# megvii-research/AAAI2023-PVD

Measured on AMD Instinct MI355X. Metric: train rays/s (hash->vm chair distillation step), higher is better.
Workload: dtype f16 tables+MLP (AMP, as the reference forces) / f32 marcher+compositor; 1 GPU; distill hash->vm, synthetic chair, synthetic cameras, stage 3 (rgb + feature/sigma/colour losses), 4096 rays/GPU/step, occupancy 128^3 5.0% occupied, max_steps 1024, teacher pre-trained 300 steps; rays_per_gpu=4096, parallelism=ray-dp1, update=AdamW in one launch, capture_fallback=False

## Files before the change

aaai2023-pvd_amd/csrc/raymarching.hip:

```cpp
#include "dda.h"
#include "rays.h"
#include "../../include/pvd_hip_march.h"

#include <float.h>

namespace pvd {

constexpr uint32_t kBlock = 256;
constexpr float kRPi = 0.3183098861837907f;


__global__ void __launch_bounds__(kBlock) k_near_far(const float *__restrict__ rays_o, const float *__restrict__ rays_d,
                                                     const float *__restrict__ aabb, uint32_t N, float min_near,
                                                     float *__restrict__ nears, float *__restrict__ fars) {
    const uint32_t n = blockIdx.x * kBlock + threadIdx.x;
    if (n >= N) return;
    const float o[3] = {rays_o[3 * (size_t)n], rays_o[3 * (size_t)n + 1], rays_o[3 * (size_t)n + 2]};
    const float d[3] = {rays_d[3 * (size_t)n], rays_d[3 * (size_t)n + 1], rays_d[3 * (size_t)n + 2]};
    near_far_of(o, d, aabb, min_near, nears[n], fars[n]);
}

__global__ void __launch_bounds__(kBlock) k_polar(const float *__restrict__ rays_o, const float *__restrict__ rays_d,
                                                  float radius, uint32_t N, float *__restrict__ coords) {
    const uint32_t n = blockIdx.x * kBlock + threadIdx.x;
    if (n >= N) return;
    const float ox = rays_o[3 * (size_t)n], oy = rays_o[3 * (size_t)n + 1], oz = rays_o[3 * (size_t)n + 2];
    const float dx = rays_d[3 * (size_t)n], dy = rays_d[3 * (size_t)n + 1], dz = rays_d[3 * (size_t)n + 2];
    const float A = dx * dx + dy * dy + dz * dz;
    const float Bh = ox * dx + oy * dy + oz * dz;
    const float Cc = ox * ox + oy * oy + oz * oz - radius * radius;
    const float t = (-Bh + sqrtf(Bh * Bh - A * Cc)) / A;
    const float x = ox + t * dx, y = oy + t * dy, z = oz + t * dz;
    const float theta = atan2f(sqrtf(x * x + z * z), y);
    const float phi = atan2f(z, x);
    coords[2 * (size_t)n] = 2 * theta * kRPi - 1;
    coords[2 * (size_t)n + 1] = phi * kRPi;
}

__global__ void __launch_bounds__(kBlock) k_get_rays(const float *__restrict__ pose, float fx, float fy, float cx, float cy,
                                                     const int64_t *__restrict__ inds, uint32_t W, uint32_t N,
                                                     float *__restrict__ rays_o, float *__restrict__ rays_d) {
    const uint32_t n = blockIdx.x * kBlock + threadIdx.x;
    if (n >= N) return;
    float o[3], d[3];
    ray_of_pixel(pose, fx, fy, cx, cy, inds ? inds[n] : (int64_t)n, W, o, d);
#pragma unroll
    for (int r = 0; r < 3; r++) { rays_o[3 * (size_t)n + r] = o[r]; rays_d[3 * (size_t)n + r] = d[r]; }
}

__global__ void __launch_bounds__(kBlock) k_make_ray_batch(const float *__restrict__ poses, uint32_t P, long long *__restrict__ state,
                                                           uint64_t seed, float fx, float fy, float cx, float cy, uint32_t H, uint32_t W,
                                                           uint32_t N, const float *__restrict__ aabb, float min_near,
                                                           int64_t *__restrict__ inds, float *__restrict__ rays_o,
                                                           float *__restrict__ rays_d, float *__restrict__ bg, float *__restrict__ nears,
                                                           float *__restrict__ fars) {
    const uint32_t n = blockIdx.x * kBlock + threadIdx.x;
    const long long pose_idx = state[0], batch = state[1];
    if (n < N) {
        Pcg32 g;
        g.seed(seed + 0x9E3779B97F4A7C15ull * (uint64_t)(batch + 1));
        g.advance(4ull * n);
        const int64_t k = (int64_t)(((uint64_t)g.next() * (uint64_t)(H * W)) >> 32);
        float o[3], d[3];
        ray_of_pixel(poses + 16 * (size_t)pose_idx, fx, fy, cx, cy, k, W, o, d);
        if (inds) inds[n] = k;
#pragma unroll
        for (int r = 0; r < 3; r++) { rays_o[3 * (size_t)n + r] = o[r]; rays_d[3 * (size_t)n + r] = d[r]; }
        if (bg) {
#pragma unroll
            for (int r = 0; r < 3; r++) bg[3 * (size_t)n + r] = g.next_float();
        }
        near_far_of(o, d, aabb, min_near, nears[n], fars[n]);
    }
    __syncthreads();
    if (threadIdx.x == 0) {
        __threadfence();
        const unsigned long long done = atomicAdd(reinterpret_cast<unsigned long long *>(state + 2), 1ull);
        if (done == gridDim.x - 1) {
            state[0] = (pose_idx + 1) % (long long)P;
            state[1] = batch + 1;
            state[2] = 0;
        }
    }
}

__global__ void __launch_bounds__(kBlock) k_morton3D(const int32_t *__restrict__ coords, uint32_t N, int32_t *__restrict__ indices) {
    const uint32_t n = blockIdx.x * kBlock + threadIdx.x;
    if (n >= N) return;
    indices[n] = (int32_t)morton3((uint32_t)coords[3 * (size_t)n], (uint32_t)coords[3 * (size_t)n + 1], (uint32_t)coords[3 * (size_t)n + 2]);
}

__global__ void __launch_bounds__(kBlock) k_morton3D_invert(const int32_t *__restrict__ indices, uint32_t N, int32_t *__restrict__ coords) {
    const uint32_t n = blockIdx.x * kBlock + threadIdx.x;
    if (n >= N) return;
    const int32_t ind = indices[n];
    coords[3 * (size_t)n] = (int32_t)gather3((uint32_t)(ind >> 0));
    coords[3 * (size_t)n + 1] = (int32_t)gather3((uint32_t)(ind >> 1));
    coords[3 * (size_t)n + 2] = (int32_t)gather3((uint32_t)(ind >> 2));
}

__global__ void __launch_bounds__(kBlock) k_packbits(const float *__restrict__ grid, uint32_t N, float thresh, uint8_t *__restrict__ bitfield) {
    const uint32_t n = blockIdx.x * kBlock + threadIdx.x;
    if (n >= N) return;
    const float4 a = reinterpret_cast<const float4 *>(grid)[2 * (size_t)n];
    const float4 b = reinterpret_cast<const float4 *>(grid)[2 * (size_t)n + 1];
    uint32_t bits = 0;
    bits |= (a.x > thresh) ? 1u : 0u;   bits |= (a.y > thresh) ? 2u : 0u;
    bits |= (a.z > thresh) ? 4u : 0u;   bits |= (a.w > thresh) ? 8u : 0u;
    bits |= (b.x > thresh) ? 16u : 0u;  bits |= (b.y > thresh) ? 32u : 0u;
    bits |= (b.z > thresh) ? 64u : 0u;  bits |= (b.w > thresh) ? 128u : 0u;
    bitfield[n] = (uint8_t)bits;
}


constexpr uint32_t kScanBlock = 1024;
__global__ void __launch_bounds__(kScanBlock) k_march_scan(int32_t *__restrict__ rays, uint32_t N, int32_t *__restrict__ counter) {
    __shared__ uint32_t wave_sums[kScanBlock / kWave];
    __shared__ uint32_t carry_s;
    const uint32_t tid = threadIdx.x, lane = tid & 63u, wid = tid >> 6;
    if (tid == 0) carry_s = (uint32_t)counter[0];
    __syncthreads();
    for (uint32_t base = 0; base < N; base += kScanBlock) {
        const uint32_t n = base + tid;
        const uint32_t v = (n < N) ? (uint32_t)rays[3 * (size_t)n + 2] : 0u;
        uint32_t s = v;
#pragma unroll
        for (int off = 1; off < kWave; off <<= 1) {
            const uint32_t up = __shfl_up(s, off, kWave);
            if ((int)lane >= off) s += up;
        }
        if (lane == 63) wave_sums[wid] = s;
        __syncthreads();
        uint32_t wave_prefix = 0, total = 0;
#pragma unroll
        for (uint32_t w = 0; w < kScanBlock / kWave; w++) {
            const uint32_t ws = wave_sums[w];
            if (w < wid) wave_prefix += ws;
            total += ws;
        }
        const uint32_t carry = carry_s;
        if (n < N) {
            rays[3 * (size_t)n] = (int32_t)n;
            rays[3 * (size_t)n + 1] = (int32_t)(carry + wave_prefix + s - v);
        }
        __syncthreads();
        if (tid == 0) carry_s = carry + total;
        __syncthreads();
    }
    if (tid == 0) {
        counter[0] = (int32_t)carry_s;
        counter[1] += (int32_t)N;
    }
}

__device__ __forceinline__ uint32_t logical_budget(uint32_t M, const int32_t *__restrict__ budget) {
    return budget ? min(M, (uint32_t)max(*budget, 0)) : M;
}


__device__ __forceinline__ float lattice_advance(float t, float dt, uint32_t n) {
    while (n > 0) {
        const float t1 = t + dt;
        n--;
        if (n == 0) return t1;
        const float t2 = t1 + dt;
        const uint32_t b1 = __float_as_uint(t1), b2 = __float_as_uint(t2);
        if ((b1 >> 23) != (b2 >> 23)) { t = t1; continue; }
        n--;
        if (n == 0) return t2;
        const float t3 = t2 + dt;
        const uint32_t b3 = __float_as_uint(t3);
        if ((b2 >> 23) != (b3 >> 23)) { t = t2; continue; }
        const uint32_t c = b3 - b2;
        if (c == 0) return t2;
        const uint32_t last = ((b2 >> 23) + 1u) << 23;
        const uint32_t kmax = (last - 1u - b2) / c;
        const uint32_t k = n < kmax ? n : kmax;
        t = __uint_as_float(b2 + k * c);
        n -= k;
    }
    return t;
}

__device__ __forceinline__ float lattice_points_gamma(float t_base, uint32_t lane, float dt_gamma, float dt_min, float dt_max, float far) {
    float cur = t_base, mine = t_base;
    for (uint32_t i = 1; i < 64; i++) {
        cur = cur + clampf(cur * dt_gamma, dt_min, dt_max);
        mine = lane >= i ? cur : mine;
        if (!(cur < far)) break;
    }
    return mine;
}

__device__ __forceinline__ uint64_t lanes_from(uint32_t lane) { return lane >= 64 ? 0ull : (~0ull << lane); }
__device__ __forceinline__ float readlane_f(float v, uint32_t lane) {
    return __uint_as_float((uint32_t)__builtin_amdgcn_readlane((int)__float_as_uint(v), (int)lane));
}

constexpr uint32_t kMarchMaxRecords = 15;
struct MarchChunk { uint64_t mask; float t_base; uint32_t pad; };
struct MarchRayRecords {
    uint32_t n, overflow, pad[2];
    MarchChunk chunk[kMarchMaxRecords];
};
struct MarchRecord {
    MarchChunk *chunk;
    uint32_t n;
    bool overflow;
};
static_assert(sizeof(MarchRayRecords) == 256, "workspace stride");

template <bool WRITE>
__device__ __forceinline__ uint32_t march_ray_wave(const Dda &r, float t0, float far, uint32_t limit, uint32_t lane,
                                                  float *__restrict__ xyzs, float *__restrict__ dirs, float *__restrict__ deltas,
                                                  uint32_t *n_chunks = nullptr, MarchRecord *__restrict__ rec = nullptr) {
    const bool grows = r.dt_gamma != 0.0f;
    float t_base = t0;
    bool pending = false;
    float pending_tt = 0.f;
    uint32_t emitted = 0;
    float last_t = t0;
    if (limit == 0) return 0;
    uint32_t lat_c = 0;
    for (;;) {
        if (n_chunks) (*n_chunks)++;
        const uint32_t bb = __float_as_uint(t_base);
        const bool fast = !grows && lat_c != 0 && bb + 64u * lat_c < (((bb >> 23) + 1u) << 23);
        const float t = grows ? lattice_points_gamma(t_base, lane, r.dt_gamma, r.dt_min, r.dt_max, far)
                              : (fast ? __uint_as_float(bb + lane * lat_c) : lattice_advance(t_base, r.dt_const, lane));
        const float t_after = t + clampf(t * r.dt_gamma, r.dt_min, r.dt_max);
        const bool valid = t < far;
        float x = 0, y = 0, z = 0, dtp = 0, tt = 0;
        bool occ = false;
// ... 1 lines not shown
        const uint64_t valid_mask = __ballot(valid);
        const uint64_t occ_mask = __ballot(valid && occ);
        uint32_t jump = 64;
        {
            uint32_t lo = lane + 1, hi = 64;
#pragma unroll
            for (int s = 0; s < 6; s++) {
                const uint32_t mid = (lo + hi) >> 1;
                const float tm = __shfl(t, (int)(mid & 63u), 64);
                const bool go_right = lo < hi && tm < tt;
                const bool go_left = lo < hi && !(tm < tt);
                lo = go_right ? mid + 1 : lo;
                hi = go_left ? mid : hi;
            }
            jump = lo;
        }

        uint32_t cur = 0;
        bool done = false;
        uint64_t emit_mask = 0;
        if (pending) {
            const uint64_t ge = __ballot(!(t < pending_tt));
            if (ge == 0) {
                cur = 64;
                if (!((valid_mask >> 63) & 1ull)) done = true;
            } else {
                cur = (uint32_t)__ffsll((long long)ge) - 1u;
                pending = false;
            }
        }
        while (cur < 64 && !done) {
            if (!((valid_mask >> cur) & 1ull)) { done = true; break; }
            if ((occ_mask >> cur) & 1ull) {
                const uint64_t stop = ~occ_mask & lanes_from(cur);
                const uint32_t e = stop ? (uint32_t)__ffsll((long long)stop) - 1u : 64u;
                uint32_t run = e - cur;
                const uint32_t room = limit - emitted;
                if (run >= room) { run = room; done = true; }
                emit_mask |= lanes_from(cur) & ~lanes_from(cur + run);
                emitted += run;
                cur = e;
            } else {
                const uint32_t j = (uint32_t)__builtin_amdgcn_readlane((int)jump, (int)cur);
                if (j >= 64) {
                    pending = true;
                    pending_tt = readlane_f(tt, cur);
                    cur = 64;
                    if (!((valid_mask >> 63) & 1ull)) done = true;
                } else {
                    cur = j;
                }
            }
        }
        if (WRITE && emit_mask) {
            const uint64_t below = emit_mask & ((1ull << lane) - 1ull);
            const uint32_t n_before = emitted - (uint32_t)__popcll(emit_mask);
            const int prev_lane = below ? 63 - __clzll((long long)below) : 0;
            const float prev_after = __shfl(t_after, prev_lane, 64);
            if ((emit_mask >> lane) & 1ull) {
                const size_t k = n_before + (uint32_t)__popcll(below);
                xyzs[3 * k] = x; xyzs[3 * k + 1] = y; xyzs[3 * k + 2] = z;
                dirs[3 * k] = r.dx; dirs[3 * k + 1] = r.dy; dirs[3 * k + 2] = r.dz;
                deltas[2 * k] = dtp;
                deltas[2 * k + 1] = t_after - (below ? prev_after : last_t);
            }
            last_t = readlane_f(t_after, 63u - (uint32_t)__clzll((long long)emit_mask));
        }
        if (rec && emit_mask) {
            if (rec->n < kMarchMaxRecords) {
                if (lane == 0) { rec->chunk[rec->n].mask = emit_mask; rec->chunk[rec->n].t_base = t_base; }
                rec->n++;
            } else {
                rec->overflow = true;
            }
        }
        if (done) break;
        t_base = readlane_f(t_after, 63);
        if (!fast && !grows) {
            const uint32_t b61 = __float_as_uint(readlane_f(t_after, 61)), b62 = __float_as_uint(readlane_f(t_after, 62));
            const uint32_t b63 = __float_as_uint(t_base);
            lat_c = ((b61 >> 23) == (b63 >> 23) && (b62 >> 23) == (b63 >> 23)) ? b63 - b62 : 0u;
        }
    }
    return emitted;
}

constexpr uint32_t kRaysPerBlock = kBlock / kWave;

constexpr uint32_t kCoarseShift = 3;
static_assert((1u << kCoarseShift) == PVD_COARSE_BLOCK, "coarse block edge");

__global__ void __launch_bounds__(kBlock) k_occ_coarse_mask(const uint8_t *__restrict__ bitfield, uint32_t C, uint32_t H,
                                                            uint8_t *__restrict__ mask) {
    const uint32_t G = H >> kCoarseShift, G3 = G * G * G;
    const uint32_t i = blockIdx.x * kBlock + threadIdx.x;
    if (i >= C * G3) return;
    const uint32_t c = i / G3, b = i - c * G3;
    const uint32_t bx = b / (G * G), by = (b / G) % G, bz = b % G;
    const uint8_t *cascade = bitfield + (size_t)c * ((size_t)H * H * H / 8);
    uint32_t any = 0;
    for (uint32_t x = max(bx, 1u) - 1u; x <= min(bx + 1u, G - 1u); x++)
        for (uint32_t y = max(by, 1u) - 1u; y <= min(by + 1u, G - 1u); y++)
            for (uint32_t z = max(bz, 1u) - 1u; z <= min(bz + 1u, G - 1u); z++) {
                const uint4 *p = reinterpret_cast<const uint4 *>(cascade + (size_t)morton3(x, y, z) * 64u);
#pragma unroll
                for (int q = 0; q < 4; q++) { const uint4 v = p[q]; any |= v.x | v.y | v.z | v.w; }
            }
    mask[i] = any ? (uint8_t)1 : (uint8_t)0;
}

__device__ __forceinline__ bool coarse_confine(const Dda &r, const uint8_t *__restrict__ mask, float t0, float &far, uint32_t lane,
                                               bool &empty) {
    empty = false;
    if (!mask || r.dt_gamma != 0.0f) return false;
    const float span = far - t0;
    if (!(span >= far * (1.0f / 1024.0f)) || !(span > 1e-6f)) return false;
    const float step = span * (1.0f / 63.0f);
    const float dmax = fmaxf(fabsf(r.dx), fmaxf(fabsf(r.dy), fabsf(r.dz)));
    const float delta = 1.25f * (0.5f * step * dmax) + r.bound * (1.0f / 1048576.0f);
    const float edge0 = (float)(2u << kCoarseShift) * r.mip_bound0 * r.rH;
    if (!(delta <= 0.9f * edge0)) return false;

    const float s = fmaf((float)lane, step, t0);
    const float x = clampf(fmaf(s, r.dx, r.ox), -r.bound, r.bound);
    const float y = clampf(fmaf(s, r.dy, r.oy), -r.bound, r.bound);
    const float z = clampf(fmaf(s, r.dz, r.oz), -r.bound, r.bound);
    int lo = 0, hi = 0;
    if (!r.one_cascade) {
        const float mx = fmaxf(fabsf(x), fmaxf(fabsf(y), fabsf(z)));
        int e_lo, e_hi, e_dt;
        (void)frexpf(fmaxf(mx - delta, 0.0f), &e_lo);
        (void)frexpf(mx + delta, &e_hi);
        (void)frexpf((float)((double)(r.dt_const * r.Hf) * 0.5), &e_dt);
        const int lvl_dt = (int)fminf(r.Cf - 1, fmaxf(0.0f, (float)e_dt));
        lo = max((int)fminf(r.Cf - 1, fmaxf(0.0f, (float)e_lo)), lvl_dt);
        hi = max((int)fminf(r.Cf - 1, fmaxf(0.0f, (float)e_hi)), lvl_dt);
    }
    const uint32_t G = r.H >> kCoarseShift;
    bool hit = false;
    for (int level = lo; level <= hi; level++) {
        const float mip_rbound = 1.0f / fminf((float)(1 << level), r.bound);
        const uint32_t bx = (uint32_t)(int)clampf(fmaf(x, mip_rbound, 1.0f) * r.half_h, 0.0f, r.cell_hi) >> kCoarseShift;
        const uint32_t by = (uint32_t)(int)clampf(fmaf(y, mip_rbound, 1.0f) * r.half_h, 0.0f, r.cell_hi) >> kCoarseShift;
        const uint32_t bz = (uint32_t)(int)clampf(fmaf(z, mip_rbound, 1.0f) * r.half_h, 0.0f, r.cell_hi) >> kCoarseShift;
        hit = hit || mask[(size_t)level * G * G * G + (bx * G + by) * G + bz] != 0;
    }
    const uint64_t hits = __ballot(hit);
    if (hits == 0) { empty = true; return true; }
    const uint32_t last = 63u - (uint32_t)__clzll((long long)hits);
    if (last < 63u) far = fminf(far, fmaf((float)(last + 1u), step, t0));
    return true;
}

__global__ void __launch_bounds__(kBlock) k_march_count_wave(const float *__restrict__ rays_o, const float *__restrict__ rays_d,
                                                             const uint8_t *__restrict__ grid, float bound, float dt_gamma, uint32_t max_steps,
                                                             uint32_t N, uint32_t C, uint32_t H, const float *__restrict__ nears,
                                                             const float *__restrict__ fars, int32_t *__restrict__ rays, uint32_t perturb,
                                                             MarchRayRecords *__restrict__ records, const int32_t *__restrict__ counter,
                                                             uint32_t fresh, const uint8_t *__restrict__ coarse_mask) {
    if (records && blockIdx.x == 0 && threadIdx.x == 0) records[N].n = fresh ? 0u : (uint32_t)counter[0];
    const uint32_t n = blockIdx.x * kRaysPerBlock + (threadIdx.x >> 6);
    const uint32_t lane = threadIdx.x & 63u;
    if (n >= N) return;
#ifdef PVD_MARCH_PROFILE
    const long long prof_t0 = __builtin_readcyclecounter();
    uint32_t prof_chunks = 0;
#endif
    Dda r;
    r.init(rays_o + 3 * (size_t)n, rays_d + 3 * (size_t)n, bound, dt_gamma, max_steps, C, H, grid);
    const float t0 = ray_t0(nears[n], r.dt_min, perturb, 42u, n);
    float far = fars[n];
    uint32_t num;
    bool empty = false;
    if (t0 >= 0.0f && t0 < far && coarse_confine(r, coarse_mask, t0, far, lane, empty) && empty) {
        num = 0;
        if (records && lane == 0) { records[n].n = 0; records[n].overflow = 0u; }
    } else if (t0 >= 0.0f && t0 < far) {
        MarchRecord rec = {records ? records[n].chunk : nullptr, 0u, false};
#ifdef PVD_MARCH_PROFILE
        num = march_ray_wave<false>(r, t0, far, max_steps, lane, nullptr, nullptr, nullptr, &prof_chunks, records ? &rec : nullptr);
#else
        num = march_ray_wave<false>(r, t0, far, max_steps, lane, nullptr, nullptr, nullptr, nullptr, records ? &rec : nullptr);
#endif
        if (records && lane == 0) { records[n].n = rec.n; records[n].overflow = rec.overflow ? 1u : 0u; }
    } else {
        float t = t0;
        num = 0;
        while (t < far && num < max_steps) {
            float x, y, z, dt, tn;
            if (r.probe(t, x, y, z, dt, tn)) { num++; t += dt; }
            else t = tn;
        }
        if (records && lane == 0) { records[n].n = 0; records[n].overflow = num ? 1u : 0u; }
    }
    if (lane == 0) rays[3 * (size_t)n + 2] = (int32_t)num;
#ifdef PVD_MARCH_PROFILE
    if (lane == 0) { rays[3 * (size_t)n] = (int32_t)(__builtin_readcyclecounter() - prof_t0); rays[3 * (size_t)n + 1] = (int32_t)prof_chunks; }
#endif
}

__global__ void __launch_bounds__(kBlock) k_march_write_wave(const float *__restrict__ rays_o, const float *__restrict__ rays_d,
                                                             const uint8_t *__restrict__ grid, float bound, float dt_gamma, uint32_t max_steps,
                                                             uint32_t N, uint32_t C, uint32_t H, uint32_t M,
                                                             const float *__restrict__ nears, const float *__restrict__ fars,
                                                             float *__restrict__ xyzs, float *__restrict__ dirs, float *__restrict__ deltas,
                                                             const int32_t *__restrict__ rays, uint32_t perturb,
                                                             const int32_t *__restrict__ budget) {
    const uint32_t n = blockIdx.x * kRaysPerBlock + (threadIdx.x >> 6);
    const uint32_t lane = threadIdx.x & 63u;
    if (n >= N) return;
    const uint32_t off = (uint32_t)rays[3 * (size_t)n + 1];
    const uint32_t num = (uint32_t)rays[3 * (size_t)n + 2];
    if (num == 0) return;
    if (off + num >= logical_budget(M, budget)) return;
    Dda r;
    r.init(rays_o + 3 * (size_t)n, rays_d + 3 * (size_t)n, bound, dt_gamma, max_steps, C, H, grid);
    const float t0 = ray_t0(nears[n], r.dt_min, perturb, 42u, n);
    const float far = fars[n];
    float *px = xyzs + 3 * (size_t)off, *pd = dirs + 3 * (size_t)off, *pl = deltas + 2 * (size_t)off;
    if (t0 >= 0.0f) {
        march_ray_wave<true>(r, t0, far, num, lane, px, pd, pl);
    } else if (lane == 0) {
        float t = t0, last_t = t0;
        uint32_t step = 0;
        while (t < far && step < num) {
            float x, y, z, dt, tn;
            if (r.probe(t, x, y, z, dt, tn)) {
                px[0] = x; px[1] = y; px[2] = z;
                pd[0] = r.dx; pd[1] = r.dy; pd[2] = r.dz;
                t += dt;
                pl[0] = dt; pl[1] = t - last_t; last_t = t;
                px += 3; pd += 3; pl += 2; step++;
            } else {
                t = tn;
            }
        }
    }
}


__global__ void __launch_bounds__(kBlock) k_march_write_records(const float *__restrict__ rays_o, const float *__restrict__ rays_d,
                                                               const uint8_t *__restrict__ grid, float bound, float dt_gamma, uint32_t max_steps,
                                                               uint32_t N, uint32_t C, uint32_t H, uint32_t M,
                                                               const float *__restrict__ nears, const float *__restrict__ fars,
                                                               float *__restrict__ xyzs, float *__restrict__ dirs, float *__restrict__ deltas,
                                                               int32_t *__restrict__ rays, uint32_t perturb,
                                                               const MarchRayRecords *__restrict__ records, int32_t *__restrict__ counter,
                                                               uint32_t fresh, const int32_t *__restrict__ budget) {
    __shared__ uint32_t part[kBlock / kWave], part_all[kBlock / kWave];
    const uint32_t Mlog = logical_budget(M, budget);
    const uint32_t n0 = blockIdx.x * kRaysPerBlock;
    const uint32_t wid = threadIdx.x >> 6, lane = threadIdx.x & 63u;
    uint32_t acc = 0, all = 0;
    const uint32_t n_sum = fresh ? N : n0;
    for (uint32_t i = threadIdx.x; i < n_sum; i += kBlock) {
        const uint32_t c = (uint32_t)rays[3 * (size_t)i + 2];
        all += c;
        acc += i < n0 ? c : 0u;
    }
#pragma unroll
    for (int off = 32; off >= 1; off >>= 1) { acc += __shfl_xor(acc, off, kWave); all += __shfl_xor(all, off, kWave); }
    if (lane == 0) { part[wid] = acc; part_all[wid] = all; }
    __syncthreads();
    uint32_t prefix = records[N].n;
    uint32_t grand = prefix;
#pragma unroll
    for (uint32_t w = 0; w < kBlock / kWave; w++) { prefix += part[w]; grand += part_all[w]; }
    if (fresh && grand < Mlog) {
        const size_t stride = (size_t)gridDim.x * kBlock, first = (size_t)blockIdx.x * kBlock + threadIdx.x;
        for (size_t i = 3 * (size_t)grand + first; i < 3 * (size_t)M; i += stride) { xyzs[i] = 0.f; dirs[i] = 0.f; }
        for (size_t i = 2 * (size_t)grand + first; i < 2 * (size_t)M; i += stride) deltas[i] = 0.f;
    }
    const uint32_t n = n0 + wid;
    uint32_t cnt[kRaysPerBlock];
#pragma unroll
    for (uint32_t w = 0; w < kRaysPerBlock; w++) cnt[w] = (n0 + w < N) ? (uint32_t)rays[3 * (size_t)(n0 + w) + 2] : 0u;
    uint32_t off = prefix;
#pragma unroll
    for (uint32_t w = 0; w < kRaysPerBlock; w++) off += (w < wid) ? cnt[w] : 0u;
    if (n0 + kRaysPerBlock >= N && threadIdx.x == 0) {
        uint32_t total = prefix;
#pragma unroll
        for (uint32_t w = 0; w < kRaysPerBlock; w++) total += cnt[w];
        counter[0] = (int32_t)total;
        counter[1] = fresh ? (int32_t)N : counter[1] + (int32_t)N;
    }
    if (n >= N) return;
    const uint32_t num = cnt[wid];
    if (lane == 0) { rays[3 * (size_t)n] = (int32_t)n; rays[3 * (size_t)n + 1] = (int32_t)off; }
    if (num == 0) return;
    if (off + num >= Mlog) {
        if (fresh && off < Mlog) {
            for (size_t i = 3 * (size_t)off + lane; i < 3 * (size_t)M; i += kWave) { xyzs[i] = 0.f; dirs[i] = 0.f; }
            for (size_t i = 2 * (size_t)off + lane; i < 2 * (size_t)M; i += kWave) deltas[i] = 0.f;
        }
        return;
    }
    Dda r;
    r.init(rays_o + 3 * (size_t)n, rays_d + 3 * (size_t)n, bound, dt_gamma, max_steps, C, H, grid);
    const float t0 = ray_t0(nears[n], r.dt_min, perturb, 42u, n);
    float *px = xyzs + 3 * (size_t)off, *pd = dirs + 3 * (size_t)off, *pl = deltas + 2 * (size_t)off;
    const MarchRayRecords &rr = records[n];
    if (rr.overflow) {
        const float far = fars[n];
        if (t0 >= 0.0f) {
            march_ray_wave<true>(r, t0, far, num, lane, px, pd, pl);
        } else if (lane == 0) {
            float t = t0, last_t = t0;
            uint32_t step = 0;
            while (t < far && step < num) {
                float x, y, z, dt, tn;
                if (r.probe(t, x, y, z, dt, tn)) {
                    px[0] = x; px[1] = y; px[2] = z;
                    pd[0] = r.dx; pd[1] = r.dy; pd[2] = r.dz;
                    t += dt;
                    pl[0] = dt; pl[1] = t - last_t; last_t = t;
                    px += 3; pd += 3; pl += 2; step++;
                } else {
                    t = tn;
                }
            }
        }
        return;
    }
    float last_t = t0;
    uint32_t emitted = 0;
    for (uint32_t c = 0; c < rr.n; c++) {
        const uint64_t emit_mask = rr.chunk[c].mask;
        const float t = r.dt_gamma != 0.0f ? lattice_points_gamma(rr.chunk[c].t_base, lane, r.dt_gamma, r.dt_min, r.dt_max, 3.0e38f)
                                           : lattice_advance(rr.chunk[c].t_base, r.dt_const, lane);
        const float t_after = t + clampf(t * r.dt_gamma, r.dt_min, r.dt_max);
        const uint64_t below = emit_mask & ((1ull << lane) - 1ull);
        const int prev_lane = below ? 63 - __clzll((long long)below) : 0;
        const float prev_after = __shfl(t_after, prev_lane, 64);
        if ((emit_mask >> lane) & 1ull) {
            const size_t k = emitted + (uint32_t)__popcll(below);
            xyzs[3 * (size_t)off + 3 * k] = clampf(fmaf(t, r.dx, r.ox), -bound, bound);
            xyzs[3 * (size_t)off + 3 * k + 1] = clampf(fmaf(t, r.dy, r.oy), -bound, bound);
            xyzs[3 * (size_t)off + 3 * k + 2] = clampf(fmaf(t, r.dz, r.oz), -bound, bound);
            pd[3 * k] = r.dx; pd[3 * k + 1] = r.dy; pd[3 * k + 2] = r.dz;
            pl[2 * k] = clampf(t * r.dt_gamma, r.dt_min, r.dt_max);
            pl[2 * k + 1] = t_after - (below ? prev_after : last_t);
        }
        emitted += (uint32_t)__popcll(emit_mask);
        last_t = readlane_f(t_after, 63u - (uint32_t)__clzll((long long)emit_mask));
    }
}



__device__ __forceinline__ float wave_incl_scan_add(float v, uint32_t lane) {
#pragma unroll
    for (int off = 1; off < 64; off <<= 1) {
        const float up = __shfl_up(v, off, 64);
        if ((int)lane >= off) v += up;
    }
    return v;
}
__device__ __forceinline__ float wave_incl_scan_mul(float v, uint32_t lane) {
#pragma unroll
    for (int off = 1; off < 64; off <<= 1) {
        const float up = __shfl_up(v, off, 64);
        if ((int)lane >= off) v *= up;
    }
    return v;
}
__device__ __forceinline__ float wave_sum(float v) {
#pragma unroll
    for (int off = 32; off >= 1; off >>= 1) v += __shfl_xor(v, off, 64);
    return v;
}

struct CompositeEpilogue {
    const float *bg;
    float bg_scalar;
    const float *nears, *fars;
    float depth_eps;
    uint32_t fresh;
    const int32_t *budget;
};

struct CompositeObjective {
    const float *img_t;
    const float *fea_s, *fea_t;
    const float *col_s, *col_t;
    uint32_t rows;
    uint32_t ray_blocks;
    float *partials;
    const float *coef, *upstream;
    float *g_fea, *g_col;
    float *rates_decay;
    float fea_decay;
    const float *rates;
    const float *extra;
    uint32_t n_extra, nparts;
    float *sums, *loss, *coef_out, *norms;
};

__device__ __forceinline__ float objective_block_sum(float v, float *__restrict__ sh) {
#pragma unroll
    for (int off = 32; off >= 1; off >>= 1) v += __shfl_xor(v, off, 64);
    __syncthreads();
    if ((threadIdx.x & 63u) == 0) sh[threadIdx.x >> 6] = v;
    __syncthreads();
    float r = 0.f;
#pragma unroll
    for (uint32_t w = 0; w < kBlock / kWave; w++) r += sh[w];
    return r;
}

__device__ __forceinline__ void objective_finish(const CompositeObjective &ob, float (&c4)[4], float *__restrict__ sh) {
    float a = 0.f, b = 0.f, c = 0.f, d = 0.f;
    for (uint32_t i = threadIdx.x; i < ob.nparts; i += kBlock) {
        const float4 v = reinterpret_cast<const float4 *>(ob.partials)[i];
        a += v.x; b += v.y; c += v.z; d += v.w;
    }
    float s4[4] = {objective_block_sum(a, sh), objective_block_sum(b, sh), objective_block_sum(c, sh), objective_block_sum(d, sh)};
    float nrm[4];
#pragma unroll
    for (int i = 0; i < 4; i++) {
        nrm[i] = sqrtf(s4[i]);
        c4[i] = nrm[i] > 0.f ? ob.rates[i] / nrm[i] : 0.f;
    }
    if (blockIdx.x == 0) {
        float e = 0.f;
        for (uint32_t i = threadIdx.x; i < ob.n_extra; i += kBlock) e += ob.extra[i];
        e = objective_block_sum(e, sh);
        if (threadIdx.x == 0) {
            float t = e;
#pragma unroll
            for (int i = 0; i < 4; i++) { t += ob.rates[i] * nrm[i]; ob.sums[i] = s4[i]; ob.norms[i] = nrm[i]; ob.coef_out[i] = c4[i]; }
            ob.loss[0] = t;
        }
    }
}

__device__ __forceinline__ void objective_row_sums(const CompositeObjective &ob, uint32_t blk, uint32_t nblk, float *__restrict__ sh) {
    const uint32_t tid = blk * kBlock + threadIdx.x, stride = nblk * kBlock;
    float s_fea = 0.f, s_sig = 0.f, s_col = 0.f;
    for (uint32_t i = tid; i < ob.rows * 4u; i += stride) {
        const float4 a = reinterpret_cast<const float4 *>(ob.fea_s)[i], b = reinterpret_cast<const float4 *>(ob.fea_t)[i];
        const float dx = a.x - b.x, dy = a.y - b.y, dz = a.z - b.z, dw = a.w - b.w;
        s_fea += dx * dx + dy * dy + dz * dz + dw * dw;
        if ((i & 3u) == 0) s_sig += dx * dx;
    }
    for (uint32_t i = tid; i < ob.rows * 3u; i += stride) { const float d = ob.col_s[i] - ob.col_t[i]; s_col += d * d; }
    s_fea = objective_block_sum(s_fea, sh); s_sig = objective_block_sum(s_sig, sh); s_col = objective_block_sum(s_col, sh);
    if (threadIdx.x == 0) reinterpret_cast<float4 *>(ob.partials)[ob.ray_blocks + blk] = make_float4(0.f, s_fea, s_sig, s_col);
}

__device__ __forceinline__ void objective_row_grads(const CompositeObjective &ob, const float (&c4)[4], uint32_t blk, uint32_t nblk) {
    const uint32_t tid = blk * kBlock + threadIdx.x, stride = nblk * kBlock;
    const float up = ob.upstream[0];
    const float c_fea = c4[1] * up, c_sig = c4[2] * up, c_col = c4[3] * up;
    for (uint32_t i = tid; i < ob.rows * 4u; i += stride) {
        const float4 a = reinterpret_cast<const float4 *>(ob.fea_s)[i], b = reinterpret_cast<const float4 *>(ob.fea_t)[i];
        float4 g = make_float4(c_fea * (a.x - b.x), c_fea * (a.y - b.y), c_fea * (a.z - b.z), c_fea * (a.w - b.w));
        if ((i & 3u) == 0) g.x += c_sig * (a.x - b.x);
        reinterpret_cast<float4 *>(ob.g_fea)[i] = g;
    }
    for (uint32_t i = tid; i < ob.rows * 3u; i += stride) ob.g_col[i] = c_col * (ob.col_s[i] - ob.col_t[i]);
}

template <bool EPI, bool OBJ = false>
__global__ void __launch_bounds__(kBlock) k_composite_fwd_wave(const float *__restrict__ sigmas, const float *__restrict__ rgbs,
                                                               const float *__restrict__ deltas, const int32_t *__restrict__ rays,
                                                               uint32_t M, uint32_t N, float *__restrict__ weights_sum,
                                                               float *__restrict__ depth, float *__restrict__ image, CompositeEpilogue ep,
                                                               CompositeObjective ob = CompositeObjective{}) {
    __shared__ float obj_sh[kBlock / kWave];
    if (OBJ && blockIdx.x >= ob.ray_blocks) {
        if (ob.rates_decay && blockIdx.x == ob.ray_blocks && threadIdx.x == 0) ob.rates_decay[1] *= ob.fea_decay;
        objective_row_sums(ob, blockIdx.x - ob.ray_blocks, gridDim.x - ob.ray_blocks, obj_sh);
        return;
    }
    const uint32_t n = blockIdx.x * (kBlock / kWave) + (threadIdx.x >> 6);
    const uint32_t lane = threadIdx.x & 63u;
    if (!OBJ && n >= N) return;
    const bool live = n < N;
    const uint32_t index = live ? (uint32_t)rays[3 * (size_t)n] : 0u;
    const uint32_t offset = live ? (uint32_t)rays[3 * (size_t)n + 1] : 0u;
    const uint32_t num = live ? (uint32_t)rays[3 * (size_t)n + 2] : 0u;
    float r = 0, g = 0, b = 0, ws = 0, d = 0;
    if (!(num == 0 || offset + num >= logical_budget(M, EPI ? ep.budget : nullptr))) {
        float T_carry = 1.0f, t_carry = 0.0f;
        for (uint32_t base = 0; base < num; base += 64) {
            const uint32_t s = base + lane;
            const bool in = s < num;
            const size_t i = (size_t)offset + s;
            float alpha = 0.f, dl1 = 0.f, c0 = 0.f, c1 = 0.f, c2 = 0.f;
            if (in) {
                const float2 dl = reinterpret_cast<const float2 *>(deltas)[i];
                alpha = 1.0f - __expf(-sigmas[i] * dl.x);
                dl1 = dl.y;
                c0 = rgbs[3 * i]; c1 = rgbs[3 * i + 1]; c2 = rgbs[3 * i + 2];
            }
            const float incl = wave_incl_scan_mul(1.0f - alpha, lane);
            float excl = __shfl_up(incl, 1, 64);
            if (lane == 0) excl = 1.0f;
            const float w = alpha * (T_carry * excl);
            const float t = t_carry + wave_incl_scan_add(dl1, lane);
            r += w * c0; g += w * c1; b += w * c2;
            d += w * t;
            ws += w;
            T_carry *= __shfl(incl, 63, 64);
            t_carry = __shfl(t, 63, 64);
        }
        r = wave_sum(r); g = wave_sum(g); b = wave_sum(b); ws = wave_sum(ws); d = wave_sum(d);
    }
    float d2 = 0.f;
    if (lane == 0 && live) {
        if (EPI) {
            const float t = 1.0f - ws;
            const float b0 = ep.bg ? ep.bg[3 * (size_t)index] : ep.bg_scalar, b1 = ep.bg ? ep.bg[3 * (size_t)index + 1] : ep.bg_scalar,
                        b2 = ep.bg ? ep.bg[3 * (size_t)index + 2] : ep.bg_scalar;
            r = r + t * b0; g = g + t * b1; b = b + t * b2;
            const float near = ep.nears[index], far = ep.fars[index];
            d = fmaxf(d - near, 0.0f) / (far - near + ep.depth_eps);
        }
        weights_sum[index] = ws;
        depth[index] = d;
        image[3 * (size_t)index] = r; image[3 * (size_t)index + 1] = g; image[3 * (size_t)index + 2] = b;
        if (OBJ) {
            const float e0 = ob.img_t[3 * (size_t)index] - r, e1 = ob.img_t[3 * (size_t)index + 1] - g, e2 = ob.img_t[3 * (size_t)index + 2] - b;
            d2 = e0 * e0 + e1 * e1 + e2 * e2;
        }
    }
    if (OBJ) {
        const float s_img = objective_block_sum(d2, obj_sh);
        if (threadIdx.x == 0) reinterpret_cast<float4 *>(ob.partials)[blockIdx.x] = make_float4(s_img, 0.f, 0.f, 0.f);
    }
}

template <bool EPI, bool OBJ = false>
__global__ void __launch_bounds__(kBlock) k_composite_bwd_wave(const float *__restrict__ grad_ws, const float *__restrict__ grad_image,
                                                               const float *__restrict__ sigmas, const float *__restrict__ rgbs,
                                                               const float *__restrict__ deltas, const int32_t *__restrict__ rays,
                                                               const float *__restrict__ weights_sum, const float *__restrict__ image,
                                                               uint32_t M, uint32_t N, float *__restrict__ grad_sigmas,
                                                               float *__restrict__ grad_rgbs, CompositeEpilogue ep,
                                                               CompositeObjective ob = CompositeObjective{}) {
    float c4[4] = {0.f, 0.f, 0.f, 0.f};
    if (OBJ) {
        __shared__ float fin_sh[kBlock / kWave];
        if (ob.rates) objective_finish(ob, c4, fin_sh);
        else { c4[0] = ob.coef[0]; c4[1] = ob.coef[1]; c4[2] = ob.coef[2]; c4[3] = ob.coef[3]; }
    }
    if (OBJ && blockIdx.x >= ob.ray_blocks) {
        objective_row_grads(ob, c4, blockIdx.x - ob.ray_blocks, gridDim.x - ob.ray_blocks);
        return;
    }
    const uint32_t n = blockIdx.x * (kBlock / kWave) + (threadIdx.x >> 6);
    const uint32_t lane = threadIdx.x & 63u;
    if (n >= N) return;
    const uint32_t index = (uint32_t)rays[3 * (size_t)n];
    const uint32_t offset = (uint32_t)rays[3 * (size_t)n + 1];
    const uint32_t num = (uint32_t)rays[3 * (size_t)n + 2];
    if (EPI && ep.fresh) {
        const uint32_t end = (uint32_t)rays[3 * (size_t)(N - 1) + 1] + (uint32_t)rays[3 * (size_t)(N - 1) + 2];
        for (size_t i = (size_t)end + (size_t)n * kWave + lane; i < M; i += (size_t)N * kWave) {
            grad_sigmas[i] = 0.f; grad_rgbs[3 * i] = 0.f; grad_rgbs[3 * i + 1] = 0.f; grad_rgbs[3 * i + 2] = 0.f;
        }
        if (num != 0 && offset + num >= logical_budget(M, ep.budget))
            for (size_t i = (size_t)offset + lane; i < M; i += kWave) {
                grad_sigmas[i] = 0.f; grad_rgbs[3 * i] = 0.f; grad_rgbs[3 * i + 1] = 0.f; grad_rgbs[3 * i + 2] = 0.f;
            }
    }
    if (num == 0 || offset + num >= logical_budget(M, EPI ? ep.budget : nullptr)) return;
    float gws = grad_ws ? grad_ws[index] : 0.0f;
    float rF = image[3 * (size_t)index], gF = image[3 * (size_t)index + 1], bF = image[3 * (size_t)index + 2];
    float g0, g1, g2;
    if (OBJ) {
        const float c_img = c4[0] * ob.upstream[0];
        g0 = c_img * (rF - ob.img_t[3 * (size_t)index]); g1 = c_img * (gF - ob.img_t[3 * (size_t)index + 1]);
        g2 = c_img * (bF - ob.img_t[3 * (size_t)index + 2]);
    } else {
        g0 = grad_image[3 * (size_t)index]; g1 = grad_image[3 * (size_t)index + 1]; g2 = grad_image[3 * (size_t)index + 2];
    }
    const float wsF = weights_sum[index];
    if (EPI) {
        const float b0 = ep.bg ? ep.bg[3 * (size_t)index] : ep.bg_scalar, b1 = ep.bg ? ep.bg[3 * (size_t)index + 1] : ep.bg_scalar,
                    b2 = ep.bg ? ep.bg[3 * (size_t)index + 2] : ep.bg_scalar;
        const float t = 1.0f - wsF;
        rF -= t * b0; gF -= t * b1; bF -= t * b2;
        gws -= g0 * b0 + g1 * b1 + g2 * b2;
    }
    float T_carry = 1.0f, r_carry = 0.f, g_carry = 0.f, b_carry = 0.f, ws_carry = 0.f;
    for (uint32_t base = 0; base < num; base += 64) {
        const uint32_t s = base + lane;
        const bool in = s < num;
        const size_t i = (size_t)offset + s;
        float alpha = 0.f, dl0 = 0.f, c0 = 0.f, c1 = 0.f, c2 = 0.f;
        if (in) {
            dl0 = deltas[2 * i];
            alpha = 1.0f - __expf(-sigmas[i] * dl0);
            c0 = rgbs[3 * i]; c1 = rgbs[3 * i + 1]; c2 = rgbs[3 * i + 2];
        }
        const float incl = wave_incl_scan_mul(1.0f - alpha, lane);
        float excl = __shfl_up(incl, 1, 64);
        if (lane == 0) excl = 1.0f;
        const float w = alpha * (T_carry * excl);
        const float T = T_carry * incl;
        const float r = r_carry + wave_incl_scan_add(w * c0, lane);
        const float g = g_carry + wave_incl_scan_add(w * c1, lane);
        const float b = b_carry + wave_incl_scan_add(w * c2, lane);
        const float ws = ws_carry + wave_incl_scan_add(w, lane);
        if (in) {
            grad_rgbs[3 * i] = g0 * w; grad_rgbs[3 * i + 1] = g1 * w; grad_rgbs[3 * i + 2] = g2 * w;
            grad_sigmas[i] = dl0 * (g0 * (T * c0 - (rF - r)) + g1 * (T * c1 - (gF - g)) + g2 * (T * c2 - (bF - b)) + gws * (T - (wsF - ws)));
        }
        T_carry = __shfl(T, 63, 64);
        r_carry = __shfl(r, 63, 64); g_carry = __shfl(g, 63, 64); b_carry = __shfl(b, 63, 64); ws_carry = __shfl(ws, 63, 64);
    }
}


__global__ void __launch_bounds__(kBlock) k_march_rays(uint32_t n_alive, uint32_t n_step, const int32_t *__restrict__ rays_alive,
                                                       const float *__restrict__ rays_t, const float *__restrict__ rays_o,
                                                       const float *__restrict__ rays_d, float bound, float dt_gamma,
                                                       uint32_t max_steps, uint32_t C, uint32_t H, const uint8_t *__restrict__ grid,
                                                       const float *__restrict__ fars, float *__restrict__ xyzs,
                                                       float *__restrict__ dirs, float *__restrict__ deltas, uint32_t perturb) {
    const uint32_t n = blockIdx.x * kBlock + threadIdx.x;
    if (n >= n_alive) return;
    const int32_t index = rays_alive[n];
    Dda r;
    r.init(rays_o + 3 * (size_t)index, rays_d + 3 * (size_t)index, bound, dt_gamma, max_steps, C, H, grid);
    const float far = fars[index];
    float t = ray_t0(rays_t[n], r.dt_min, perturb, (uint64_t)perturb, n);
    float last_t = t;
    float *px = xyzs + 3 * (size_t)n * n_step, *pd = dirs + 3 * (size_t)n * n_step, *pl = deltas + 2 * (size_t)n * n_step;
    uint32_t step = 0;
    while (t < far && step < n_step) {
        float x, y, z, dt, tn;
        if (r.probe(t, x, y, z, dt, tn)) {
            px[0] = x; px[1] = y; px[2] = z;
            pd[0] = r.dx; pd[1] = r.dy; pd[2] = r.dz;
            t += dt;
            pl[0] = dt; pl[1] = t - last_t; last_t = t;
            px += 3; pd += 3; pl += 2; step++;
        } else {
            t = tn;
        }
    }
}

__global__ void __launch_bounds__(kBlock) k_composite_rays(uint32_t n_alive, uint32_t n_step, const int32_t *__restrict__ rays_alive,
                                                           float *__restrict__ rays_t, const float *__restrict__ sigmas,
                                                           const float *__restrict__ rgbs, const float *__restrict__ deltas,
                                                           float *__restrict__ weights_sum, float *__restrict__ depth,
                                                           float *__restrict__ image) {
    const uint32_t n = blockIdx.x * kBlock + threadIdx.x;
    if (n >= n_alive) return;
    const int32_t index = rays_alive[n];
    float t = rays_t[n];
    float ws = weights_sum[index], d = depth[index];
    float r = image[3 * (size_t)index], g = image[3 * (size_t)index + 1], b = image[3 * (size_t)index + 2];
    uint32_t step = 0;
    while (step < n_step) {
        const size_t i = (size_t)n * n_step + step;
        const float dl0 = deltas[2 * i];
        if (dl0 == 0) break;
        const float alpha = 1.0f - __expf(-sigmas[i] * dl0);
        const float T = 1 - ws;
        const float w = alpha * T;
        ws += w;
        t += deltas[2 * i + 1];
        d += w * t;
        r += w * rgbs[3 * i]; g += w * rgbs[3 * i + 1]; b += w * rgbs[3 * i + 2];
        if ((double)T < 1e-4) break;
        step++;
    }
    rays_t[n] = (step < n_step) ? -1.0f : t;
    weights_sum[index] = ws;
    depth[index] = d;
    image[3 * (size_t)index] = r; image[3 * (size_t)index + 1] = g; image[3 * (size_t)index + 2] = b;
}

__global__ void __launch_bounds__(kBlock) k_compact_rays(uint32_t n_alive, int32_t *__restrict__ rays_alive,
                                                         const int32_t *__restrict__ rays_alive_old, float *__restrict__ rays_t,
                                                         const float *__restrict__ rays_t_old, int32_t *__restrict__ alive_counter) {
    __shared__ uint32_t wave_cnt[kBlock / kWave];
    __shared__ uint32_t block_base;
    const uint32_t n = blockIdx.x * kBlock + threadIdx.x;
    const uint32_t lane = threadIdx.x & 63u, wid = threadIdx.x >> 6;
    float t = -1.0f;
    int32_t id = 0;
// ... 128 lines not shown
            if (dl0 == 0) break;
            const float alpha = 1.0f - __expf(-(sigma_scale * sigmas[i]) * dl0);
            const float T = 1 - ws;
            const float w = alpha * T;
            ws += w;
            t += deltas[2 * i + 1];
            d += w * t;
            r += w * rgbs[3 * i]; g += w * rgbs[3 * i + 1]; b += w * rgbs[3 * i + 2];
            if ((double)T < 1e-4) break;
            step++;
        }
        rays_t[n] = (step < n_step) ? -1.0f : t;
        weights_sum[index] = ws;
        depth[index] = d;
        image[3 * (size_t)index] = r; image[3 * (size_t)index + 1] = g; image[3 * (size_t)index + 2] = b;
    }
}

}

using namespace pvd;

#define PVD_REQUIRE(cond) \
    do { if (!(cond)) return PVD_ERR_INVALID; } while (0)

extern "C" {

int pvd_near_far_from_aabb(const float *rays_o, const float *rays_d, const float *aabb, uint32_t N, float min_near,
                           float *nears, float *fars, pvd_stream_t stream) {
    if (N == 0) return PVD_OK;
    PVD_REQUIRE(rays_o && rays_d && aabb && nears && fars);
    hipLaunchKernelGGL(k_near_far, dim3(div_up(N, kBlock)), dim3(kBlock), 0, (hipStream_t)stream, rays_o, rays_d, aabb, N, min_near, nears, fars);
    return check_launch();
}

int pvd_get_rays(const float *pose, float fx, float fy, float cx, float cy, const int64_t *inds, uint32_t W, uint32_t N,
                 float *rays_o, float *rays_d, pvd_stream_t stream) {
    if (N == 0) return PVD_OK;
    PVD_REQUIRE(pose && rays_o && rays_d && W > 0);
    hipLaunchKernelGGL(k_get_rays, dim3(div_up(N, kBlock)), dim3(kBlock), 0, (hipStream_t)stream, pose, fx, fy, cx, cy, inds, W, N, rays_o, rays_d);
    return check_launch();
}

int pvd_make_ray_batch(const float *poses, uint32_t P, int64_t *state, uint64_t seed, float fx, float fy, float cx, float cy, uint32_t H,
                       uint32_t W, uint32_t N, const float *aabb, float min_near, int64_t *inds, float *rays_o, float *rays_d, float *bg,
                       float *nears, float *fars, pvd_stream_t stream) {
    if (N == 0) return PVD_OK;
    PVD_REQUIRE(poses && P > 0 && state && aabb && rays_o && rays_d && nears && fars && H > 0 && W > 0);
    PVD_REQUIRE((uint64_t)H * W < (1ull << 32));
    hipLaunchKernelGGL(k_make_ray_batch, dim3(div_up(N, kBlock)), dim3(kBlock), 0, (hipStream_t)stream, poses, P, (long long *)state, seed, fx,
                       fy, cx, cy, H, W, N, aabb, min_near, inds, rays_o, rays_d, bg, nears, fars);
    return check_launch();
}

int pvd_polar_from_ray(const float *rays_o, const float *rays_d, float radius, uint32_t N, float *coords, pvd_stream_t stream) {
    if (N == 0) return PVD_OK;
    PVD_REQUIRE(rays_o && rays_d && coords);
    hipLaunchKernelGGL(k_polar, dim3(div_up(N, kBlock)), dim3(kBlock), 0, (hipStream_t)stream, rays_o, rays_d, radius, N, coords);
    return check_launch();
}

int pvd_morton3D(const int32_t *coords, uint32_t N, int32_t *indices, pvd_stream_t stream) {
    if (N == 0) return PVD_OK;
    PVD_REQUIRE(coords && indices);
    hipLaunchKernelGGL(k_morton3D, dim3(div_up(N, kBlock)), dim3(kBlock), 0, (hipStream_t)stream, coords, N, indices);
    return check_launch();
}

int pvd_morton3D_invert(const int32_t *indices, uint32_t N, int32_t *coords, pvd_stream_t stream) {
    if (N == 0) return PVD_OK;
    PVD_REQUIRE(coords && indices);
    hipLaunchKernelGGL(k_morton3D_invert, dim3(div_up(N, kBlock)), dim3(kBlock), 0, (hipStream_t)stream, indices, N, coords);
    return check_launch();
}

int pvd_packbits(const float *grid, uint32_t N, float density_thresh, uint8_t *bitfield, pvd_stream_t stream) {
    if (N == 0) return PVD_OK;
    PVD_REQUIRE(grid && bitfield);
    PVD_REQUIRE((reinterpret_cast<uintptr_t>(grid) & 15u) == 0);
    hipLaunchKernelGGL(k_packbits, dim3(div_up(N, kBlock)), dim3(kBlock), 0, (hipStream_t)stream, grid, N, density_thresh, bitfield);
    return check_launch();
}

constexpr uint32_t kMarchFusedScanMaxRays = 16384;

size_t pvd_march_workspace_bytes(uint32_t N) { return ((size_t)N + 1) * sizeof(MarchRayRecords); }

int pvd_march_rays_train(const float *rays_o, const float *rays_d, const uint8_t *grid, float bound, float dt_gamma,
                         uint32_t max_steps, uint32_t N, uint32_t C, uint32_t H, uint32_t M, const float *nears,
                         const float *fars, float *xyzs, float *dirs, float *deltas, int32_t *rays, int32_t *counter,
                         uint32_t perturb, pvd_stream_t stream) {
    return pvd_march_rays_train_ws(rays_o, rays_d, grid, bound, dt_gamma, max_steps, N, C, H, M, nears, fars, xyzs, dirs, deltas, rays,
                                   counter, perturb, nullptr, 0, 0u, nullptr, stream);
}

int pvd_march_rays_train_ws(const float *rays_o, const float *rays_d, const uint8_t *grid, float bound, float dt_gamma,
                            uint32_t max_steps, uint32_t N, uint32_t C, uint32_t H, uint32_t M, const float *nears,
                            const float *fars, float *xyzs, float *dirs, float *deltas, int32_t *rays, int32_t *counter,
                            uint32_t perturb, void *workspace, size_t workspace_bytes, uint32_t flags, const int32_t *budget_dev,
                            pvd_stream_t stream) {
    return pvd_march_rays_train_mask(rays_o, rays_d, grid, bound, dt_gamma, max_steps, N, C, H, M, nears, fars, xyzs, dirs, deltas, rays,
                                     counter, perturb, workspace, workspace_bytes, flags, budget_dev, nullptr, stream);
}

int pvd_occ_coarse_mask(const uint8_t *bitfield, uint32_t C, uint32_t H, uint8_t *mask, pvd_stream_t stream) {
    PVD_REQUIRE(bitfield && mask && C >= 1 && C <= 16 && H >= 1 && H <= 1024);
    if ((H & (H - 1u)) || H < PVD_COARSE_BLOCK) return PVD_ERR_UNSUPPORTED;
    PVD_REQUIRE((reinterpret_cast<uintptr_t>(bitfield) & 15u) == 0);
    const uint32_t G = H >> kCoarseShift;
    hipLaunchKernelGGL(k_occ_coarse_mask, dim3(div_up(C * G * G * G, kBlock)), dim3(kBlock), 0, (hipStream_t)stream, bitfield, C, H, mask);
    return check_launch();
}

int pvd_march_rays_train_mask(const float *rays_o, const float *rays_d, const uint8_t *grid, float bound, float dt_gamma,
                              uint32_t max_steps, uint32_t N, uint32_t C, uint32_t H, uint32_t M, const float *nears,
                              const float *fars, float *xyzs, float *dirs, float *deltas, int32_t *rays, int32_t *counter,
                              uint32_t perturb, void *workspace, size_t workspace_bytes, uint32_t flags,
                              const int32_t *budget_dev, const uint8_t *coarse_mask, pvd_stream_t stream) {
    hipStream_t s = (hipStream_t)stream;
    const bool fresh = (flags & PVD_MARCH_FRESH) != 0;
    if (N == 0) {
        if (fresh && M && xyzs && dirs && deltas && counter) {
            (void)hipMemsetAsync(xyzs, 0, 3 * (size_t)M * sizeof(float), s); (void)hipMemsetAsync(dirs, 0, 3 * (size_t)M * sizeof(float), s);
            (void)hipMemsetAsync(deltas, 0, 2 * (size_t)M * sizeof(float), s); (void)hipMemsetAsync(counter, 0, 2 * sizeof(int32_t), s);
        }
        return PVD_OK;
    }
    PVD_REQUIRE(rays_o && rays_d && grid && nears && fars && xyzs && dirs && deltas && rays && counter);
    PVD_REQUIRE(C >= 1 && C <= 16 && H >= 1 && H <= 1024 && max_steps >= 1);
    MarchRayRecords *records = (workspace && workspace_bytes >= pvd_march_workspace_bytes(N) && N <= kMarchFusedScanMaxRays)
                                   ? (MarchRayRecords *)workspace : nullptr;
    if (fresh && !records) {
        (void)hipMemsetAsync(xyzs, 0, 3 * (size_t)M * sizeof(float), s); (void)hipMemsetAsync(dirs, 0, 3 * (size_t)M * sizeof(float), s);
        (void)hipMemsetAsync(deltas, 0, 2 * (size_t)M * sizeof(float), s); (void)hipMemsetAsync(counter, 0, 2 * sizeof(int32_t), s);
    }
    const dim3 g(div_up(N, kRaysPerBlock)), b(kBlock);
    if ((H & (H - 1u)) || H < PVD_COARSE_BLOCK) coarse_mask = nullptr;
    hipLaunchKernelGGL(k_march_count_wave, g, b, 0, s, rays_o, rays_d, grid, bound, dt_gamma, max_steps, N, C, H, nears, fars, rays, perturb,
                       records, counter, records && fresh ? 1u : 0u, coarse_mask);
    if (records) {
        hipLaunchKernelGGL(k_march_write_records, g, b, 0, s, rays_o, rays_d, grid, bound, dt_gamma, max_steps, N, C, H, M, nears, fars, xyzs,
                           dirs, deltas, rays, perturb, records, counter, fresh ? 1u : 0u, budget_dev);
        return check_launch();
    }
#ifdef PVD_MARCH_PROFILE
    return check_launch();
#endif
    hipLaunchKernelGGL(k_march_scan, dim3(1), dim3(kScanBlock), 0, s, rays, N, counter);
    hipLaunchKernelGGL(k_march_write_wave, g, b, 0, s, rays_o, rays_d, grid, bound, dt_gamma, max_steps, N, C, H, M, nears, fars, xyzs, dirs,
                       deltas, rays, perturb, budget_dev);
    return check_launch();
}

int pvd_composite_rays_train_forward(const float *sigmas, const float *rgbs, const float *deltas, const int32_t *rays,
                                     uint32_t M, uint32_t N, float *weights_sum, float *depth, float *image,
                                     pvd_stream_t stream) {
    if (N == 0) return PVD_OK;
    PVD_REQUIRE(sigmas && rgbs && deltas && rays && weights_sum && depth && image);
    hipLaunchKernelGGL(k_composite_fwd_wave<false>, dim3(div_up(N, kBlock / kWave)), dim3(kBlock), 0, (hipStream_t)stream, sigmas, rgbs, deltas,
                       rays, M, N, weights_sum, depth, image, CompositeEpilogue{});
    return check_launch();
}

int pvd_composite_rays_train_backward(const float *grad_weights_sum, const float *grad_image, const float *sigmas,
                                      const float *rgbs, const float *deltas, const int32_t *rays, const float *weights_sum,
                                      const float *image, uint32_t M, uint32_t N, float *grad_sigmas, float *grad_rgbs,
                                      pvd_stream_t stream) {
    if (N == 0) return PVD_OK;
    PVD_REQUIRE(grad_weights_sum && grad_image && sigmas && rgbs && deltas && rays && weights_sum && image && grad_sigmas && grad_rgbs);
    hipLaunchKernelGGL(k_composite_bwd_wave<false>, dim3(div_up(N, kBlock / kWave)), dim3(kBlock), 0, (hipStream_t)stream, grad_weights_sum,
                       grad_image, sigmas, rgbs, deltas, rays, weights_sum, image, M, N, grad_sigmas, grad_rgbs, CompositeEpilogue{});
    return check_launch();
}

int pvd_composite_rays_train_bg_forward(const float *sigmas, const float *rgbs, const float *deltas, const int32_t *rays, uint32_t M,
                                        uint32_t N, const float *bg, float bg_scalar, const float *nears, const float *fars,
                                        float depth_eps, float *weights_sum, float *depth, float *image, const int32_t *budget_dev,
                                        pvd_stream_t stream) {
    if (N == 0) return PVD_OK;
    PVD_REQUIRE(sigmas && rgbs && deltas && rays && nears && fars && weights_sum && depth && image);
    const CompositeEpilogue ep{bg, bg_scalar, nears, fars, depth_eps, 0u, budget_dev};
    hipLaunchKernelGGL(k_composite_fwd_wave<true>, dim3(div_up(N, kBlock / kWave)), dim3(kBlock), 0, (hipStream_t)stream, sigmas, rgbs, deltas,
                       rays, M, N, weights_sum, depth, image, ep);
    return check_launch();
}

int pvd_composite_rays_train_bg_backward(const float *grad_weights_sum, const float *grad_image, const float *sigmas, const float *rgbs,
                                         const float *deltas, const int32_t *rays, const float *weights_sum, const float *image,
                                         uint32_t M, uint32_t N, const float *bg, float bg_scalar, float *grad_sigmas, float *grad_rgbs,
                                         uint32_t flags, const int32_t *budget_dev, pvd_stream_t stream) {
    const bool fresh = (flags & PVD_MARCH_FRESH) != 0;
    if (N == 0) {
        if (fresh && M && grad_sigmas && grad_rgbs) {
            (void)hipMemsetAsync(grad_sigmas, 0, (size_t)M * sizeof(float), (hipStream_t)stream);
            (void)hipMemsetAsync(grad_rgbs, 0, 3 * (size_t)M * sizeof(float), (hipStream_t)stream);
        }
        return PVD_OK;
    }
    PVD_REQUIRE(grad_image && sigmas && rgbs && deltas && rays && weights_sum && image && grad_sigmas && grad_rgbs);
    const CompositeEpilogue ep{bg, bg_scalar, nullptr, nullptr, 0.f, fresh ? 1u : 0u, budget_dev};
    hipLaunchKernelGGL(k_composite_bwd_wave<true>, dim3(div_up(N, kBlock / kWave)), dim3(kBlock), 0, (hipStream_t)stream, grad_weights_sum,
                       grad_image, sigmas, rgbs, deltas, rays, weights_sum, image, M, N, grad_sigmas, grad_rgbs, ep);
    return check_launch();
}

static uint32_t objective_row_blocks(uint32_t rows, uint32_t cap) {
    uint32_t b = div_up(rows * 4u, kBlock);
    if (b > cap) b = cap;
    return b < 1 ? 1 : b;
}

uint32_t pvd_composite_objective_blocks(uint32_t N, uint32_t rows) { return div_up(N, kBlock / kWave) + objective_row_blocks(rows, 256u); }
uint32_t pvd_composite_objective_blocks_fixed(uint32_t N) { return div_up(N, kBlock / kWave) + 256u; }

int pvd_composite_objective_forward(const float *sigmas, const float *rgbs, const float *deltas, const int32_t *rays, uint32_t M, uint32_t N,
                                    const float *bg, float bg_scalar, const float *nears, const float *fars, float depth_eps,
                                    float *weights_sum, float *depth, float *image, const int32_t *budget_dev, const float *img_tea,
                                    const float *fea_stu, const float *fea_tea, const float *col_stu, const float *col_tea, uint32_t rows,
                                    float *S4, float *rates4_decay, float fea_decay, uint32_t flags, pvd_stream_t stream) {
    PVD_REQUIRE(N > 0 && rows > 0);
    PVD_REQUIRE(sigmas && rgbs && deltas && rays && nears && fars && weights_sum && depth && image);
    PVD_REQUIRE(img_tea && fea_stu && fea_tea && col_stu && col_tea && S4);
    const CompositeEpilogue ep{bg, bg_scalar, nears, fars, depth_eps, 0u, budget_dev};
    CompositeObjective ob{};
    ob.img_t = img_tea; ob.fea_s = fea_stu; ob.fea_t = fea_tea; ob.col_s = col_stu; ob.col_t = col_tea; ob.rows = rows;
    ob.ray_blocks = div_up(N, kBlock / kWave);
    ob.partials = S4 + 4;
    ob.rates_decay = rates4_decay; ob.fea_decay = fea_decay;
    const uint32_t blocks = ob.ray_blocks + ((flags & PVD_OBJECTIVE_FIXED_PARTS) ? 256u : objective_row_blocks(rows, 256u));
    hipLaunchKernelGGL((k_composite_fwd_wave<true, true>), dim3(blocks), dim3(kBlock), 0, (hipStream_t)stream, sigmas, rgbs, deltas, rays, M, N,
                       weights_sum, depth, image, ep, ob);
    return check_launch();
}

int pvd_composite_objective_backward(const float *grad_weights_sum, const float *sigmas, const float *rgbs, const float *deltas,
                                     const int32_t *rays, const float *weights_sum, const float *image, uint32_t M, uint32_t N,
                                     const float *bg, float bg_scalar, float *grad_sigmas, float *grad_rgbs, uint32_t flags,
                                     const int32_t *budget_dev, const float *img_tea, const float *fea_stu, const float *fea_tea,
                                     const float *col_stu, const float *col_tea, uint32_t rows, float *coef4, const float *upstream,
                                     float *g_fea, float *g_col, const float *rates4, const float *extra, uint32_t n_extra, float *S4,
                                     float *loss, float *norms4, pvd_stream_t stream) {
    PVD_REQUIRE(N > 0 && rows > 0);
    PVD_REQUIRE(sigmas && rgbs && deltas && rays && weights_sum && image && grad_sigmas && grad_rgbs);
    PVD_REQUIRE(img_tea && fea_stu && fea_tea && col_stu && col_tea && coef4 && upstream && g_fea && g_col);
    PVD_REQUIRE(!rates4 || (S4 && loss && norms4 && (!n_extra || extra)));
    const bool fresh = (flags & PVD_MARCH_FRESH) != 0;
    const CompositeEpilogue ep{bg, bg_scalar, nullptr, nullptr, 0.f, fresh ? 1u : 0u, budget_dev};
    CompositeObjective ob{};
    ob.img_t = img_tea; ob.fea_s = fea_stu; ob.fea_t = fea_tea; ob.col_s = col_stu; ob.col_t = col_tea; ob.rows = rows;
    ob.ray_blocks = div_up(N, kBlock / kWave);
    ob.coef = coef4; ob.upstream = upstream; ob.g_fea = g_fea; ob.g_col = g_col;
    if (rates4) {
        ob.rates = rates4; ob.extra = extra; ob.n_extra = n_extra;
        ob.nparts = (flags & PVD_OBJECTIVE_FIXED_PARTS) ? pvd_composite_objective_blocks_fixed(N) : pvd_composite_objective_blocks(N, rows);
        ob.partials = S4 + 4; ob.sums = S4; ob.loss = loss; ob.coef_out = coef4; ob.norms = norms4;
    }
    const uint32_t blocks = ob.ray_blocks + objective_row_blocks(rows, 2048u);
    hipLaunchKernelGGL((k_composite_bwd_wave<true, true>), dim3(blocks), dim3(kBlock), 0, (hipStream_t)stream, grad_weights_sum,
                       (const float *)nullptr, sigmas, rgbs, deltas, rays, weights_sum, image, M, N, grad_sigmas, grad_rgbs, ep, ob);
    return check_launch();
}

int pvd_march_rays(uint32_t n_alive, uint32_t n_step, const int32_t *rays_alive, const float *rays_t, const float *rays_o,
                   const float *rays_d, float bound, float dt_gamma, uint32_t max_steps, uint32_t C, uint32_t H,
                   const uint8_t *grid, const float *nears, const float *fars, float *xyzs, float *dirs, float *deltas,
                   uint32_t perturb, pvd_stream_t stream) {
    (void)nears;
    if (n_alive == 0) return PVD_OK;
    PVD_REQUIRE(rays_alive && rays_t && rays_o && rays_d && grid && fars && xyzs && dirs && deltas);
    PVD_REQUIRE(C >= 1 && C <= 16 && H >= 1 && H <= 1024 && max_steps >= 1);
    hipLaunchKernelGGL(k_march_rays, dim3(div_up(n_alive, kBlock)), dim3(kBlock), 0, (hipStream_t)stream, n_alive, n_step, rays_alive, rays_t,
                       rays_o, rays_d, bound, dt_gamma, max_steps, C, H, grid, fars, xyzs, dirs, deltas, perturb);
    return check_launch();
}

int pvd_composite_rays(uint32_t n_alive, uint32_t n_step, const int32_t *rays_alive, float *rays_t, const float *sigmas,
                       const float *rgbs, const float *deltas, float *weights_sum, float *depth, float *image,
                       pvd_stream_t stream) {
    if (n_alive == 0) return PVD_OK;
    PVD_REQUIRE(rays_alive && rays_t && sigmas && rgbs && deltas && weights_sum && depth && image);
    hipLaunchKernelGGL(k_composite_rays, dim3(div_up(n_alive, kBlock)), dim3(kBlock), 0, (hipStream_t)stream, n_alive, n_step, rays_alive,
                       rays_t, sigmas, rgbs, deltas, weights_sum, depth, image);
    return check_launch();
}

int pvd_compact_rays(uint32_t n_alive, int32_t *rays_alive, const int32_t *rays_alive_old, float *rays_t,
                     const float *rays_t_old, int32_t *alive_counter, pvd_stream_t stream) {
    if (n_alive == 0) return PVD_OK;
    PVD_REQUIRE(rays_alive && rays_alive_old && rays_t && rays_t_old && alive_counter);
    hipLaunchKernelGGL(k_compact_rays, dim3(div_up(n_alive, kBlock)), dim3(kBlock), 0, (hipStream_t)stream, n_alive, rays_alive,
                       rays_alive_old, rays_t, rays_t_old, alive_counter);
    return check_launch();
}

static uint32_t infer_blocks(uint32_t upper) {
    uint32_t b = div_up(upper ? upper : 1u, kBlock);
    return b < kInferBlocks ? b : kInferBlocks;
}

int pvd_infer_round_begin(int32_t *state, uint32_t parity, uint32_t N, uint32_t max_steps, pvd_stream_t stream) {
    PVD_REQUIRE(state && parity < 2 && N > 0);
    hipLaunchKernelGGL(k_infer_begin, dim3(1), dim3(64), 0, (hipStream_t)stream, (InferState *)state, parity, N, max_steps);
    return check_launch();
}

int pvd_infer_compact(int32_t *state, uint32_t parity, uint32_t n_upper, int32_t *rays_alive, const int32_t *rays_alive_old, float *rays_t,
// ... 28 lines not shown
```

aaai2023-pvd_amd/pvd/knobs.py:

```python

PRODUCTION = {
    "PVD_HIP_LIB": ("<package>/libpvd_hip.so", "path of an A/B build of the same C ABI (pvd_hip/__init__.py)"),
    "PVD_DIST_BACKEND": ("nccl", "nccl (= RCCL, one GPU per rank) | gloo (ranks may share a GPU: how the GPU tests run two ranks on a one-GPU box)"),
    "PVD_DP_EXCHANGE": ("allreduce", "ray-DP gradient exchange: allreduce (gather that zeroes / checks -> all-reduce -> the update reads the buffer) | "
                                     "sharded (reduce_scatter -> AdamW on the rank's rows -> all_gather) | classic (rounds 1-5's sequence, incl. the objective's "
                                     "four separate launches): pvd/trainer.py, pvd/ray_dp.py"),
    "PVD_DP_HASH_WIRE": ("f16", "f16 | f32: a hash student's table gradient under ray-DP crosses the links as the half-precision table the scatter wrote "
                                "(the reference's arithmetic for this gradient; 21 MB) or widened into the fp32 bucket first (42 MB; rounds 1-5)"),
    "PVD_DP_WIRE": ("f32", "f32 | f16 | bf16: width of the gradient on the wire (classic form only; measured -0.3 dB PSNR: opt-in)"),
    "PVD_STEPS_PER_GRAPH": ("", "bench.py: steps recorded per hipGraph launch (default: the largest of 20/10/5/4/2 dividing --steps)"),
    "PVD_HW_QUEUES": ("", "keep = do not set GPU_MAX_HW_QUEUES=2 at import (an integrator who owns that variable); the forked schedule is then refused "
                          "unless the caller exported 2 itself"),
}

TEST = {
    "PVD_DP_FORCE": ("0", "1 = run the ray-DP code path (collectives, exchange forms) in a world of ONE rank: RCCL next to graph capture on a one-GPU box"),
    "PVD_DP_PIPELINE": ("1", "0 | 1 (fork the next step's prefix when there is more than one rank) | 2 (always: the one-rank tests)"),
    "PVD_DP_INGRAPH": ("1", "0 = keep RCCL's collectives out of the graphs (graphs cut at the collectives: the gloo form, and the fall-back of a failed capture)"),
    "PVD_DP_OVERLAP": ("1", "segmented form only: 0 = do not replay the next step's prefix under the eager exchange"),
    "PVD_DP_SHARDED_MIN": ("65536", "elements below which a sharded sum stays a plain all-reduce (tests lower it for toy models)"),
    "PVD_ADAMW_SPLIT": ("late", "late | 0: AdamW in two parts (L1-only rows one step later on the branch) or one launch -- bit-identical (tests/test_hip_graph.py)"),
    "PVD_ADAMW_LAZY": ("1", "0 = decay the cold parameter groups every step instead of logging and replaying the decays -- bit-identical"),
    "PVD_TOUCHED_SET": ("1", "0 = zero / check the whole gradient buffer instead of the rows the occupancy grid lets a sample touch -- same training"),
    "PVD_INF_CHECK_RIDE": ("1", "0 = GradScaler's inf check as a launch of its own instead of riding on the table scatter / the exchange"),
    "PVD_HEAD_DW_RIDE": ("1", "0 = the VM head's riders on the lookup's launches as launches of their own: the weight-gradient reduction (extra workgroups of the table scatter) and the f16 weight image (extra workgroups of the lookup's forward)"),
    "PVD_MLP_FUSED": ("1", "0 = the frozen NeRF-MLP teacher layer by layer instead of pvd_mlp_head_forward_fused"),
    "PVD_INFER_PERSISTENT": ("1", "0 = inference as rounds (march / forward / composite / compact launches) instead of one persistent launch -- bit-identical images"),
    "PVD_INFER_DEVICE_ROUNDS": ("1", "0 = the reference-shaped host loop with a read-back per round"),
    "PVD_INFER_SHUFFLE": ("", "C side: slot-assignment stride of the persistent renders (a permutation of the work order; images bit-identical)"),
    "PVD_FUSED_DMA": ("", "C side: 0 / 1 = the fused lookup's weight image by register copies / LDS-DMA -- bit-identical"),
    "PVD_FORKED_GRAPHS": ("", "0 | 1 overrides whether two-chain hipGraphs may be recorded (default: only with GPU_MAX_HW_QUEUES=2)"),
    "PVD_CAPTURE_GC": ("1", "0 = leave the cyclic garbage collector on while recording (the round-2 SIGABRT's regression test)"),
    "PVD_TEST_FAIL_IN_CAPTURE": ("", "1 | forked = raise inside a recording: exercises every fall-back"),
}

ALL = {**PRODUCTION, **TEST}
```

aaai2023-pvd_amd/pvd/ops.py:

```python
import os
import types

import torch


def _mse_loss():
    from .losses import mse_fused
    return mse_fused


def _distill_loss():
    from .losses import distill_loss_normL2
    return distill_loss_normL2


def _flat_adamw():
    from .flat_adamw import FlatAdamW
    return FlatAdamW


def hip_ops():
    import gridencoder
    import raymarching
    import fusedhead
    import pvd_hip
    import shencoder
    import vmencoder
    import plenoxel

    def get_rays_fused(pose, intrinsics, H, W, N, error_map=None, generator=None):
        dev = pose.device
        coarse = None
        if error_map is not None:
            from .scene import sample_pixels_by_error
            inds2, coarse = sample_pixels_by_error(error_map.reshape(1, -1).to(dev), N, H, W, generator)
            inds = inds2[0].contiguous()
        else:
            inds = torch.randint(0, H * W, size=[N], device=dev, generator=generator)
        rays_o = torch.empty(1, N, 3, device=dev)
        rays_d = torch.empty(1, N, 3, device=dev)
        fx, fy, cx, cy = intrinsics
        pvd_hip.get_rays(pose.reshape(4, 4).contiguous(), fx, fy, cx, cy, inds, W, N, rays_o, rays_d)
        out = {"rays_o": rays_o, "rays_d": rays_d, "inds": inds[None]}
        if coarse is not None:
            out["inds_coarse"] = coarse
        return out

    def make_batch(poses, state, seed, intrinsics, H, W, N, aabb, min_near):
        dev = poses.device
        f = lambda *s: torch.empty(*s, dtype=torch.float32, device=dev)
        rays_o, rays_d, bg, nears, fars = f(1, N, 3), f(1, N, 3), f(1, N, 3), f(N), f(N)
        fx, fy, cx, cy = intrinsics
        pvd_hip.make_ray_batch(poses, state, seed, fx, fy, cx, cy, H, W, N, aabb, min_near, None, rays_o, rays_d, bg, nears, fars)
        return rays_o, rays_d, bg, (nears, fars)

    def freq_encode(x, bands, include_input=True, out_dtype=torch.float32, row_stride=None):
        return pvd_hip.freq_encode(x, bands, include_input, out_dtype, row_stride)

    return types.SimpleNamespace(freq_encode=freq_encode, make_batch=make_batch, occupancy=pvd_hip.occupancy_backend, raymarching=raymarching, GridEncoder=gridencoder.GridEncoder, SHEncoder=shencoder.SHEncoder,
                                 vm_encode=vmencoder.vm_encode, vm_encode_infer=vmencoder.vm_encode_infer, plenoxel=plenoxel, get_rays=get_rays_fused, fused_head=fusedhead, distill_loss=_distill_loss(), mse_loss=_mse_loss(), flat_adamw=_flat_adamw(), device_type="cuda", name="hip")
```

aaai2023-pvd_amd/pvd/renderer.py:

```python
import math

import numpy as np
import torch
import torch.nn as nn


def near_far_from_aabb_torch(rays_o, rays_d, aabb, min_near):
    rd = 1.0 / rays_d
    lo = (aabb[:3] - rays_o) * rd
    hi = (aabb[3:] - rays_o) * rd
    t_lo, t_hi = torch.minimum(lo, hi), torch.maximum(lo, hi)
    near, far = t_lo[:, 0], t_hi[:, 0]
    miss = torch.zeros_like(near, dtype=torch.bool)
    for a in (1, 2):
        miss = miss | (near > t_hi[:, a]) | (t_lo[:, a] > far)
        near, far = torch.maximum(near, t_lo[:, a]), torch.minimum(far, t_hi[:, a])
    big = torch.finfo(near.dtype).max
    near = torch.where(miss, torch.full_like(near, big), near.clamp_min(min_near))
    far = torch.where(miss, torch.full_like(far, big), far)
    return near, far


def sample_pdf(bins, weights, n_samples, det=False):
    pdf = weights + 1e-5
# ... 175 lines not shown
                i_march = True
            premarched = kwargs.get("premarched", False)
            if premarched:
                i_march = False
            else:
                counter = self.step_counter[self.local_step % 16]
                self.local_step += 1
            budget = self._budget() if not force_all_rays else None
            own = i_march or bool(kwargs.get("own_march", False))
            if i_march:
                xyzs, dirs, deltas, rays = self._march_train(rays_o, rays_d, nears, fars, counter, perturb, force_all_rays, dt_gamma,
                                                             max_steps, budget)
                inherited_params = [xyzs, dirs, deltas, rays]
            else:
                xyzs, dirs, deltas, rays = inherited_params

            sigmas, rgbs = self(xyzs, dirs)

            if not self.teacher_variant:
                gs, st = self.args.global_step, self.args.stage_iters
                if gs < st["stage1"]:
                    return {"stage1": gs, "depth": None, "image": None, "inherited_params": inherited_params, "sigmas": sigmas, "rays": rays}
                if gs < st["stage2"]:
                    return {"stage2": gs, "depth": None, "image": None, "inherited_params": inherited_params, "sigmas": sigmas, "rays": rays}

            if self.density_scale != 1:
                sigmas = self.density_scale * sigmas
            eps = 0.0 if self.teacher_variant else 1e-6
            ride = kwargs.get("objective")
            if ride is not None and not (torch.is_grad_enabled() and ride.with_student(getattr(self, "feature_sigma_color", None), getattr(self, "color_l", None))):
                ride = None
            okw = {} if ride is None else {"objective": ride}
            if budget is not None and own:
                weights_sum, depth, image = rm.composite_rays_train_bg(sigmas, rgbs, deltas, rays, bg_color, nears, fars, eps, True, budget[1], **okw)
            else:
                weights_sum, depth, image = rm.composite_rays_train_bg(sigmas, rgbs, deltas, rays, bg_color, nears, fars, eps, True, **okw)
            image = image.view(*prefix, 3)
            depth = depth.view(*prefix)
            return {"depth": depth, "image": image, "inherited_params": inherited_params, "sigmas": sigmas, "rays": rays,
                    "nears_fars": (nears, fars)}

        if self._persistent_render(rays_o, perturb):
            if self.model_type == "tensors":
                run = self.ops.plenoxel.infer_image
            else:
                fh = self.ops.fused_head
                run = {"hash": fh.hash_infer_image, "vm": fh.vm_infer_image}.get(self.model_type) or fh.mlp_infer_image
            weights_sum, depth, image = run(self, rays_o, rays_d, nears, fars, dt_gamma, max_steps)
            image = image + (1 - weights_sum).unsqueeze(-1) * bg_color
            depth = torch.clamp(depth - nears, min=0) / (fars - nears)
            return {"depth": depth.view(*prefix), "image": image.view(*prefix, 3), "inherited_params": inherited_params}
        if self._rounds_on_device(rays_o, perturb):
            return self._run_rounds_device(rays_o, rays_d, nears, fars, bg_color, dt_gamma, max_steps, prefix, inherited_params)
        dtype = torch.float32
        weights_sum = torch.zeros(N, dtype=dtype, device=device)
        depth = torch.zeros(N, dtype=dtype, device=device)
        image = torch.zeros(N, 3, dtype=dtype, device=device)
        n_alive = N
        alive_counter = torch.zeros([1], dtype=torch.int32, device=device)
        rays_alive = torch.zeros(2, n_alive, dtype=torch.int32, device=device)
        rays_t = torch.zeros(2, n_alive, dtype=dtype, device=device)
        step, i = 0, 0
        while step < max_steps:
            if step == 0:
                rays_alive[0] = torch.arange(n_alive, dtype=torch.int32, device=device)
                rays_t[0] = nears
            else:
                alive_counter.zero_()
                rm.compact_rays(n_alive, rays_alive[i % 2], rays_alive[(i + 1) % 2], rays_t[i % 2], rays_t[(i + 1) % 2], alive_counter)
                n_alive = alive_counter.item()
            if n_alive <= 0:
                break
            n_step = max(min(N // n_alive, 8), 1)
            xyzs, dirs, deltas = rm.march_rays(n_alive, n_step, rays_alive[i % 2], rays_t[i % 2], rays_o, rays_d, self.bound,
                                               self.density_bitfield, self.cascade, self.grid_size, nears, fars, 128, perturb,
                                               dt_gamma, max_steps)
            sigmas, rgbs = self(xyzs, dirs)
            sigmas = self.density_scale * sigmas
            rm.composite_rays(n_alive, n_step, rays_alive[i % 2], rays_t[i % 2], sigmas, rgbs, deltas, weights_sum, depth, image)
            step += n_step
            i += 1
        image = image + (1 - weights_sum).unsqueeze(-1) * bg_color
        depth = torch.clamp(depth - nears, min=0) / (fars - nears)
        return {"depth": depth.view(*prefix), "image": image.view(*prefix, 3), "inherited_params": inherited_params}

    def _persistent_render(self, rays_o, perturb):
        import os
        fh = getattr(getattr(self, "ops", None), "fused_head", None)
        mt = getattr(self, "model_type", None)
        if os.environ.get("PVD_INFER_PERSISTENT", "1") == "0":
            return False
        if mt == "tensors":
            px = getattr(getattr(self, "ops", None), "plenoxel", None)
            return (rays_o.is_cuda and not perturb and hasattr(px, "infer_image") and getattr(self, "bg_net", None) is None
                    and not self.args.enable_edit_plenoxel)
        return self._rounds_on_device(rays_o, perturb) and ((mt == "hash" and hasattr(fh, "hash_infer_image")) or
                                                            (mt == "vm" and hasattr(fh, "vm_infer_image")) or
                                                            (mt == "mlp" and hasattr(fh, "mlp_infer_image")))

    def _rounds_on_device(self, rays_o, perturb):
        import os
        return (rays_o.is_cuda and not perturb and hasattr(self.rm, "infer_march") and torch.is_autocast_enabled("cuda")
                and getattr(self, "supports_device_rows", lambda: False)() and os.environ.get("PVD_INFER_DEVICE_ROUNDS", "1") != "0")

    @torch.no_grad()
    def _run_rounds_device(self, rays_o, rays_d, nears, fars, bg_color, dt_gamma, max_steps, prefix, inherited_params, check_every=8):
        rm = self.rm
        N, device = rays_o.shape[0], rays_o.device
        f32 = dict(dtype=torch.float32, device=device)
        weights_sum, depth, image = torch.zeros(N, **f32), torch.zeros(N, **f32), torch.zeros(N, 3, **f32)
        state = torch.zeros(rm.INFER_STATE_INTS, dtype=torch.int32, device=device)
        state[0] = N
        rays_alive = torch.empty(2, N, dtype=torch.int32, device=device)
        rays_t = torch.empty(2, N, **f32)
        rays_alive[0] = torch.arange(N, dtype=torch.int32, device=device)
        rays_t[0] = nears
        rows = N + (128 - N % 128) % 128
        xyzs, dirs, deltas = torch.empty(rows, 3, **f32), torch.empty(rows, 3, **f32), torch.empty(rows, 2, **f32)
        rows_dev = state[4:5]
        n_upper, i = N, 0
        while True:
            for _ in range(check_every):
                cur, old = i & 1, (i & 1) ^ 1
                if i > 0:
                    rm.infer_compact(state, cur, n_upper, rays_alive[cur], rays_alive[old], rays_t[cur], rays_t[old])
                rm.infer_round_begin(state, cur, N, max_steps)
                rm.infer_march(state, n_upper, rays_alive[cur], rays_t[cur], rays_o, rays_d, self.bound, dt_gamma, max_steps, self.cascade,
                               self.grid_size, self.density_bitfield, fars, xyzs, dirs, deltas, False)
                m_upper = min(rows, 8 * n_upper + (128 - (8 * n_upper) % 128) % 128)
                sigmas, rgbs = self.forward_rows(xyzs[:m_upper], dirs[:m_upper], rows_dev)
                rm.infer_composite(state, n_upper, rays_alive[cur], rays_t[cur], sigmas, rgbs.float(), deltas, float(self.density_scale),
                                   weights_sum, depth, image)
                i += 1
            n_alive, steps_done = state[2:6:3].tolist()
            if n_alive <= 0 or steps_done >= max_steps:
                break
            n_upper = min(n_upper, n_alive)
        self._last_rounds = int(state[6])
        image = image + (1 - weights_sum).unsqueeze(-1) * bg_color
        depth = torch.clamp(depth - nears, min=0) / (fars - nears)
        return {"depth": depth.view(*prefix), "image": image.view(*prefix, 3), "inherited_params": inherited_params}

    def march(self, rays_o, rays_d, dt_gamma=0, perturb=False, force_all_rays=False, max_steps=1024, nears_fars=None):
        rm = self.rm
        rays_o = rays_o.contiguous().view(-1, 3)
        rays_d = rays_d.contiguous().view(-1, 3)
        nears, fars = nears_fars if nears_fars is not None else rm.near_far_from_aabb(rays_o, rays_d, self.aabb_train, self.min_near)
        counter = self.step_counter[self.local_step % 16]
        self.local_step += 1
        budget = self._budget() if not force_all_rays else None
        xyzs, dirs, deltas, rays = self._march_train(rays_o, rays_d, nears, fars, counter, perturb, force_all_rays, dt_gamma, max_steps, budget)
        return [xyzs, dirs, deltas, rays], (nears, fars)

    def _march_train(self, rays_o, rays_d, nears, fars, counter, perturb, force_all_rays, dt_gamma, max_steps, budget):
        coarse = self.coarse_mask()
        extra = () if budget is None and coarse is None else (budget,) if coarse is None else (budget, coarse)
        return self.rm.march_rays_train(rays_o, rays_d, self.bound, self.density_bitfield, self.cascade, self.grid_size, nears, fars,
                                        counter, self.mean_count, perturb, 128, force_all_rays, dt_gamma, max_steps, True, *extra)

    def _cell_centres(self, coords, cas, jitter):
        H = self.grid_size
        xyzs = 2 * coords.float() / (H - 1) - 1
        bound = min(2 ** cas, self.bound)
        hgs = bound / H
        p = xyzs * (bound - hgs)
        if jitter:
            p = p + (torch.rand_like(p) * 2 - 1) * hgs
        return p, hgs

    @torch.no_grad()
    def mark_untrained_grid(self, poses, intrinsic, S=64):
        if not self.cuda_ray:
            return
        if isinstance(poses, np.ndarray):
            poses = torch.from_numpy(poses)
        dev = self.density_grid.device
        poses = poses.to(dev)
        B = poses.shape[0]
        fx, fy, cx, cy = intrinsic
        H = self.grid_size
        axis = torch.arange(H, dtype=torch.int32, device=dev)
        count = torch.zeros_like(self.density_grid)
        for xs in axis.split(S):
            for ys in axis.split(S):
                for zs in axis.split(S):
                    xx, yy, zz = torch.meshgrid(xs, ys, zs, indexing="ij")
                    coords = torch.stack([xx.reshape(-1), yy.reshape(-1), zz.reshape(-1)], dim=-1)
                    indices = self.rm.morton3D(coords).long()
                    for cas in range(self.cascade):
                        world, hgs = self._cell_centres(coords, cas, jitter=False)
                        for head in range(0, B, S):
                            P = poses[head:head + S]
                            cam = (world.unsqueeze(0) - P[:, :3, 3].unsqueeze(1)) @ P[:, :3, :3]
                            seen = (cam[..., 2] > 0) \
                                & (cam[..., 0].abs() < cx / fx * cam[..., 2] + hgs * 2) \
                                & (cam[..., 1].abs() < cy / fy * cam[..., 2] + hgs * 2)
                            count[cas, indices] += seen.sum(0).reshape(-1)
        self.density_grid[count == 0] = -1
        self.note_occupancy_changed()

    @torch.no_grad()
    def update_extra_state(self, decay=0.95, S=128):
        if not self.cuda_ray:
            return
        self._flush_deferred_updates()
        occ = getattr(self.ops, "occupancy", None)
        if occ is not None and self.density_grid.is_cuda:
            return self._update_extra_state_device(occ, decay)
        rm = self.rm
        dev = self.density_grid.device
        H = self.grid_size
        tmp_grid = -torch.ones_like(self.density_grid)

        def query(coords, indices, cas):
            p, _ = self._cell_centres(coords, cas, jitter=True)
            sig = self.density(p)["sigma"].reshape(-1).detach().float() * self.density_scale
            tmp_grid[cas, indices] = sig

        if self.iter_density < 16:
            axis = torch.arange(H, dtype=torch.int32, device=dev)
            for xs in axis.split(S):
                for ys in axis.split(S):
                    for zs in axis.split(S):
                        xx, yy, zz = torch.meshgrid(xs, ys, zs, indexing="ij")
                        coords = torch.stack([xx.reshape(-1), yy.reshape(-1), zz.reshape(-1)], dim=-1)
                        indices = rm.morton3D(coords).long()
                        for cas in range(self.cascade):
                            query(coords, indices, cas)
        else:
            n = H ** 3 // 4
            for cas in range(self.cascade):
                coords = torch.randint(0, H, (n, 3), device=dev)
                indices = rm.morton3D(coords).long()
                occ = torch.nonzero(self.density_grid[cas] > 0).squeeze(-1)
                if occ.shape[0] > 0:
                    occ = occ[torch.randint(0, occ.shape[0], [n], dtype=torch.long, device=dev)]
                    occ_coords = rm.morton3D_invert(occ)
                    indices = torch.cat([indices, occ], dim=0)
                    coords = torch.cat([coords, occ_coords], dim=0)
                query(coords, indices, cas)

        valid = (self.density_grid >= 0) & (tmp_grid >= 0)
        self.density_grid[valid] = torch.maximum(self.density_grid[valid] * decay, tmp_grid[valid])
        self.mean_density = torch.mean(self.density_grid.clamp(min=0)).item()
        self.iter_density += 1

        thresh = min(self.mean_density, self.density_thresh)
        self.density_bitfield = rm.packbits(self.density_grid, thresh, self.density_bitfield)
        self.note_occupancy_changed()

        total_step = min(16, self.local_step)
        if total_step > 0:
            self.mean_count = int(self.step_counter[:total_step, 0].sum().item() / total_step)
        self.local_step = 0

    def _update_extra_state_device(self, occ, decay):
        dev = self.density_grid.device
        H, C = self.grid_size, self.cascade
        H3 = H ** 3
        st = getattr(self, "_occ_state", None)
        if st is None:
            st = self._occ_state = dict(list=torch.empty(H3, dtype=torch.int32, device=dev), count=torch.zeros(1, dtype=torch.int32, device=dev),
                                        tmp=torch.empty(H3, dtype=torch.float32, device=dev), scratch=torch.empty(1024, device=dev),
                                        mean_thresh=torch.zeros(2, device=dev), calls=0)
        full = self.iter_density < 16
        n_u, n_o = (H3, 0) if full else (H3 // 4, H3 // 4)
        n = n_u + n_o
        indices = torch.empty(n, dtype=torch.int32, device=dev)
        xyz = torch.empty(n, 3, dtype=torch.float32, device=dev)
        for cas in range(C):
            st["calls"] += 1
            if self.occ_replay:
                self._occ_cascade_replay(occ, st, cas, full, n_u, indices, xyz, decay)
                continue
            occ.occ_sample(self.density_grid[cas], H, n_u, n_o, full, float(min(2 ** cas, self.bound)), 0x0cc0 + 7919 * st["calls"], st["list"],
                           st["count"], indices, xyz)
            sig = self.density(xyz)["sigma"].reshape(-1).detach().float().contiguous()
            occ.occ_update(self.density_grid[cas], st["tmp"], indices, sig, H, float(self.density_scale), float(decay))
        occ.occ_finish(self.density_grid.view(-1), float(self.density_thresh), st["mean_thresh"], st["scratch"], self.density_bitfield)
        self.note_occupancy_changed()
        self.mean_density = st["mean_thresh"][0]
        self.iter_density += 1
        total_step = min(16, self.local_step)
        if total_step > 0:
            self.mean_count = int(self.step_counter[:total_step, 0].sum().item() / total_step)
            self._publish_budget()
        self.local_step = 0

    occ_replay = False

    def _occ_cascade_replay(self, occ, st, cas, full, n_u, indices, xyz, decay):
        dev = self.density_grid.device
        H = self.grid_size
        bound_c = float(min(2 ** cas, self.bound))
        if full:
            assert H <= 128, "the reference sweeps in 128^3 blocks: replay covers the single-block case"
            jitter = torch.rand(H ** 3, 3).to(dev)
            occ.occ_sample_replay(H, 0, 0, True, bound_c, None, None, None, jitter, indices, xyz)
            n = H ** 3
        else:
            cells = torch.randint(0, H, (n_u, 3))
            lst = torch.nonzero(self.density_grid[cas] > 0).squeeze(-1)
            n_o = 0
            picks = None
            if lst.shape[0] > 0:
                picks = torch.randint(0, lst.shape[0], [n_u], dtype=torch.long).to(torch.int32).to(dev)
# ... 55 lines not shown
```

aaai2023-pvd_amd/pvd/trainer.py:

```python
import os

import torch
import torch.distributed as dist

from .capture import CarriedPrefix, SegmentedCapture
from .ray_dp import FlatGrads, RayDP, _FlatOptGrads, _make_loss


def pvd_forked_graphs_ok():
    import pvd_hip
    return pvd_hip.forked_graphs_ok()


def psnr(pred, truth):
    mse = torch.mean((pred.float() - truth.float()) ** 2)
    return -10.0 * torch.log10(mse)


class _TrainerBase:
    def __init__(self, opt, model, lr, device, fp16=True, dp=None, eta_min=None, exp_decay=False):
        self.opt = opt
        self.device = torch.device(device)
        self.device_type = self.device.type
        self.fp16 = bool(fp16)
# ... 74 lines not shown
        if c is None:
            from .dp_compact import GradCompactor
            offs = self.optimizer.offsets if self.flat_opt else None
            if offs is None:
                offs, acc = [], 0
                for p in self.flat.params:
                    offs.append(acc)
                    acc += p.numel()
            c = GradCompactor(m, self.flat.params, offs, self.device, marcher=marcher)
            c.agreed = True
            if self.dp.enabled and self.dp.capture is None and c.idx is not None:
                sig = torch.tensor([c.idx.numel(), float(c.idx.sum())], dtype=torch.float64, device=self.device)
                sig = torch.cat([sig, -sig])
                dist.all_reduce(sig, op=dist.ReduceOp.MAX, group=self.dp.group)
                c.agreed = bool(sig[0] == -sig[2]) and bool(sig[1] == -sig[3])
            self._compactor = c
        return c if (c.fraction < 0.7 and c.agreed) else None

    def _zero_grads(self, first_in_recording=False):
        if self.flat_opt:
            c = self._grad_compactor() if os.environ.get("PVD_TOUCHED_SET", "1") != "0" else None
            if c is not self.optimizer.touched:
                self.optimizer.set_touched(c)
        self.flat.zero_(full=first_in_recording)

    _xlayouts = None
    _v2_off = False
    _sharded_stale = False

    def _exchange_mode(self, c):
        mode = os.environ.get("PVD_DP_EXCHANGE", "allreduce")
        if (mode == "classic" or c is None or self._v2_off or not self.flat_opt or self.device_type != "cuda" or c is not self.optimizer.touched
                or not self.optimizer._outside_is_zero or os.environ.get("PVD_DP_WIRE", "f32") != "f32"
                or getattr(self, "_overlap_with_exchange", None) is not None or not self.optimizer.compact_ready()):
            return None
        return "sharded" if (mode == "sharded" and (self.dp.world_size > 1 or os.environ.get("PVD_DP_FORCE") == "1")) else "allreduce"

    def _xlayout(self, c, chunks, with_params):
        from .dp_compact import ExchangeLayout
        key = (id(c), chunks, with_params)
        if self._xlayouts is None or self._xlayouts[0] != key:
            assert not torch.cuda.is_current_stream_capturing(), "the exchange layout is built by the eager warm-up steps"
            self._xlayouts = (key, ExchangeLayout(c, self.optimizer._warm_B, chunks, self.device, with_params=with_params))
        return self._xlayouts[1]

    def prepare_exchange(self):
        if not self.dp.enabled or not self.flat_opt:
            return
        c = self._grad_compactor()
        mode = self._exchange_mode(c)
        if mode is not None:
            try:
                self._xlayout(c, self.dp.world_size if mode == "sharded" else 1, mode == "sharded")
            except AssertionError:
                self._v2_off = True

    def _exchange_v2(self, c, mode):
        import pvd_hip
        o, dp = self.optimizer, self.dp
        sharded = mode == "sharded"
        L = self._xlayout(c, dp.world_size if sharded else 1, sharded)
        pvd_hip.segments_gather_zero_check(self.flat.flat, L.segs, L.xbuf, L.xbuf[L.slot:], L.chunk, L.chunks)
        clear = (L.xbuf[L.slot:], L.chunk, L.chunks)
        if not sharded:
            dp.all_reduce_sum_(L.xbuf)
            o.take_compact(L.xbuf, L.xbuf[L.slot:L.slot + 1], clear, (0, L.n_groups))
            return
        mine = L.chunk_of(L.xbuf, dp.rank)
        dp.reduce_scatter_sum_(mine, L.xbuf)
        pmine = L.chunk_of(L.pbuf, dp.rank)
        o.take_compact(mine, mine[L.slot:L.slot + 1], clear, L.rows_of(dp.rank), param_out=pmine)

        def after_update():
            dp.all_gather_(L.pbuf, pmine)
            pvd_hip.segments_op(pvd_hip.SEG_SCATTER, o.flat_p, L.segs, buf=L.pbuf)
            pvd_hip.note_weights_changed(o.params)
        self._after_update = after_update
        self._sharded_stale = True

    def sync_sharded_state(self):
        if not self._sharded_stale:
            return
        import pvd_hip
        assert not torch.cuda.is_current_stream_capturing()
        L, o, dp = self._xlayouts[1], self.optimizer, self.dp
        o.flush()
        for buf in (o.flat_m, o.flat_v):
            pvd_hip.segments_op(pvd_hip.SEG_GATHER, buf, L.segs, buf=L.pbuf)
            dp.all_gather_(L.pbuf, L.chunk_of(L.pbuf, dp.rank).clone())
            pvd_hip.segments_op(pvd_hip.SEG_SCATTER, buf, L.segs, buf=L.pbuf)
        self._sharded_stale = False

    def _exchange(self):
        if self.dp.enabled:
            c = self._grad_compactor()
            mode = self._exchange_mode(c)
            if mode is not None:
                return self._exchange_v2(c, mode)
            if self._sharded_stale and not torch.cuda.is_current_stream_capturing():
                self.sync_sharded_state()
            ov = getattr(self, "_overlap_with_exchange", None)
            wire = {"f16": torch.float16, "bf16": torch.bfloat16}.get(os.environ.get("PVD_DP_WIRE", "f32"))
            hg = getattr(self.optimizer, "_half_grad", None) if self.flat_opt else None
            if c is None and hg is not None:
                lo, hi, g16 = hg
                self.dp.all_reduce_sum_(g16, overlap=ov)
                flat = self.flat.flat
                if self.optimizer._half_range_dirty:
                    self.dp.all_reduce_sum_(flat)
                else:
                    if lo > 0:
                        self.dp.all_reduce_sum_(flat[:lo])
                    if hi < flat.numel():
                        self.dp.all_reduce_sum_(flat[hi:])
            elif c is None:
                if wire is None:
                    self.dp.all_reduce_sum_(self.flat.flat, overlap=ov)
                else:
                    w16 = self.flat.flat.to(wire)
                    self.dp.all_reduce_sum_(w16, overlap=ov)
                    self.flat.flat.copy_(w16)
            else:
                buf = c.gather(self.flat.flat)
                if wire is None:
                    self.dp.all_reduce_sum_(buf, overlap=ov)
                else:
                    w16 = buf.to(wire)
                    self.dp.all_reduce_sum_(w16, overlap=ov)
                    buf = w16.to(torch.float32)
                checked = (self.flat_opt and c is self.optimizer.touched and self.optimizer._outside_is_zero
                           and bool(getattr(self.scaler, "_enabled", False)) and os.environ.get("PVD_INF_CHECK_RIDE", "1") != "0")
                c.scatter(self.flat.flat, buf, found_inf=self.optimizer.inf_flag() if checked else None)
                if checked:
                    self.optimizer.note_checked_by_backward()

    _after_update = None

    def _optimize(self):
        self.scaler.step(self.optimizer)
        self.scaler.update()
        after, self._after_update = self._after_update, None
        if after is not None:
            after()

    def _backward_and_step(self, loss):
        self._backward(loss)
        self._exchange()
        self._optimize()
        self.scheduler.step()
        self.global_step += 1

    steps_per_replay = 1

    def capture(self, body, warmup=3, steps_per_graph=1):
        assert self.device_type == "cuda"
        side = torch.cuda.Stream()
        side.wait_stream(torch.cuda.current_stream())
        with torch.cuda.stream(side):
            for _ in range(warmup):
                self._zero_grads()
                out = body()
                self._backward(out[0])
                self._exchange()
                self._optimize()
                self.scheduler.step()
                self.global_step += 1
                del out
        torch.cuda.current_stream().wait_stream(side)
        torch.cuda.synchronize()
        cap = SegmentedCapture(self.device)
        self.dp.capture = cap
        if self.dp.enabled and not self.dp.ingraph:
            steps_per_graph = 1
        self._graph_zeroes = False
        if max(1, int(steps_per_graph)) >= 2 and not self.dp.enabled:
            self._fold_launches(True)
        try:
            with cap:
                for k_rec in range(max(1, int(steps_per_graph))):
                    self._zero_grads(first_in_recording=k_rec == 0)
                    self._static_out = body()
                    if os.environ.get("PVD_TEST_FAIL_IN_CAPTURE") == "1":
                        raise RuntimeError("forced failure inside the capture (PVD_TEST_FAIL_IN_CAPTURE)")
                    self._backward(self._static_out[0])
                    self._exchange()
                    self._optimize()
        finally:
            self.dp.capture = None
            self._fold_launches(False)
        self._cap = cap
        self.steps_per_replay = max(1, int(steps_per_graph))
        self._captured_occ_epoch = self._marching_model().occ_epoch if (self.flat_opt and self.optimizer.touched is not None) else None
        return self._static_out

    def _fold_launches(self, on):
        if self.flat_opt:
            self.optimizer.zero_in_step = bool(on)
            if on:
                self._graph_zeroes = False
                self.optimizer._zeroed_by_step = False
            else:
                self._graph_zeroes = bool(self.optimizer._zeroed_by_step)
                self.optimizer._zeroed_by_step = False

    def _after_failed_capture(self):
        import traceback
        traceback.print_exc()
        torch.cuda.synchronize()
        self.dp.capture = None
        self._fold_launches(False)
        self._graph_zeroes = False
        self._after_update = None
        if self.flat_opt:
            self.optimizer._compact = None
            self.optimizer._half_grad = None
            self.optimizer._part_a_owed = None
            self.optimizer.end_two_part(failed=True)

    def replay(self):
        assert getattr(self, "_captured_occ_epoch", None) in (None, self._marching_model().occ_epoch), \
            "the occupancy grid changed since the step was captured (touched-row set is stale): capture again"
        if self.flat_opt:
            import pvd_hip
            pvd_hip.note_weights_changed(self.optimizer.params)
        if self.flat_opt:
            self.optimizer.before_replay()
        self._cap.replay()
        if self.flat_opt:
            if getattr(self, "_replay_owes_part_a", None) is not None:
                self.optimizer.note_carried_part_a(self._replay_owes_part_a)
            self.optimizer.note_device_steps(self.steps_per_replay)
            if getattr(self, "_graph_zeroes", False):
                self.optimizer._zeroed_by_step = True
        for _ in range(self.steps_per_replay):
            self.scheduler.step()
        self.global_step += self.steps_per_replay
        return self._static_out


class DistillTrainer(_TrainerBase):

    compact_exchange = True

    def __init__(self, opt, model_tea, model_stu, device, fp16=True, dp=None):
        for p in model_tea.parameters():
            p.requires_grad = False
        lr = opt.lr * (0.1 if opt.model_type == "mlp" else 1.0)
        super().__init__(opt, model_stu, lr, device, fp16, dp, eta_min=5e-5)
        self.model_tea = model_tea.train()
        self.model_stu = model_stu.train()
        self.loss = _make_loss(opt.loss_type, self.dp)
        self.loss_rate_fea_sc = opt.loss_rate_fea_sc
        self.rates = torch.tensor([opt.loss_rate_rgb, opt.loss_rate_fea_sc, opt.loss_rate_sigma, opt.loss_rate_color],
                                  dtype=torch.float32, device=self.device)
        self.fea_rate = self.rates[1:2]
        self.fused_loss = getattr(model_stu.ops, "distill_loss", None)

    def render_kwargs(self):
        o = self.opt
        return dict(dt_gamma=o.dt_gamma, max_steps=o.max_steps)

    def _marching_model(self):
        return self.model_stu if bool(getattr(self.opt, "render_stu_first", True)) else self.model_tea

    def prefetch(self, batch_fn):
        return self.prefetch_teacher(self.prefetch_march(batch_fn))

    def prefetch_march(self, batch_fn):
        rays_o, rays_d, bg, *rest = batch_fn()
        with torch.autocast(self.device_type, dtype=torch.float16, enabled=self.fp16 and self.device_type == "cuda"):
            inh, nf = self.model_stu.march(rays_o, rays_d, perturb=True, force_all_rays=False, nears_fars=rest[0] if rest else None,
                                           **self.render_kwargs())
        return dict(rays_o=rays_o, rays_d=rays_d, bg=bg, inh=inh, nf=nf)

    def prefetch_teacher(self, part):
        with torch.autocast(self.device_type, dtype=torch.float16, enabled=self.fp16 and self.device_type == "cuda"), torch.no_grad():
            out_tea = self.model_tea.render(part["rays_o"], part["rays_d"], staged=False, bg_color=part["bg"], perturb=True,
                                            force_all_rays=False, inherited_params=part["inh"], nears_fars=part["nf"], premarched=True,
                                            **self.render_kwargs())
        tea = self.model_tea
        attrs = {k: getattr(tea, k, None) for k in ("feature_sigma_color", "sigma_l", "color_l")}
        return dict(part, out_tea=out_tea, tea_attrs={k: v for k, v in attrs.items() if torch.is_tensor(v)})

    def compute_loss(self, rays_o, rays_d, bg_color, nears_fars=None, pre=None):
        o, stu, tea = self.opt, self.model_stu, self.model_tea
        o.global_step = self.global_step
        self.__dict__.pop("_ride", None)
        kw = self.render_kwargs()
        kw_stu = dict(kw, nears_fars=nears_fars) if nears_fars is not None else kw
        if pre is not None:
            for k, v in pre.get("tea_attrs", {}).items():
                setattr(tea, k, v)
            out_tea = dict(pre["out_tea"])
            if out_tea.get("image") is not None and pre.get("replayed_ahead", False):
                out_tea["image"] = out_tea["image"].clone()
            ride = None
            l1_on_host = o.l1_reg_weight > 0.0 and o.model_type == "vm" and not self.flat_opt
            dp_ride = self.dp.enabled and not l1_on_host and os.environ.get("PVD_DP_EXCHANGE", "allreduce") != "classic"
            if (self.fused_loss is not None and o.loss_type == "normL2" and (not self.dp.enabled or dp_ride) and torch.is_grad_enabled()
                    and self._stage_of(self.global_step) == 3 and out_tea.get("image") is not None
                    and min(o.loss_rate_color, o.loss_rate_sigma, self.loss_rate_fea_sc * 0.995, o.loss_rate_rgb) > 0.0
                    and torch.is_tensor(getattr(tea, "feature_sigma_color", None)) and torch.is_tensor(getattr(tea, "color_l", None))
                    and tea.feature_sigma_color.dim() == 2 and tea.feature_sigma_color.shape[-1] == 16
                    and tea.feature_sigma_color.dtype == torch.float32 and pre["rays_o"].is_cuda):
                from .losses import ObjectiveRide
                fin = not l1_on_host
                ride = ObjectiveRide(out_tea["image"], tea.feature_sigma_color, tea.color_l, rates_decay=self.rates if fin else None, fea_decay=0.995,
                                     fixed_parts=self.dp.enabled)
                self.dp_objective_rides = bool(self.dp.enabled)
            out_stu = stu.render(pre["rays_o"], pre["rays_d"], staged=False, bg_color=pre["bg"], perturb=True, force_all_rays=False,
                                 inherited_params=pre["inh"], nears_fars=pre["nf"], premarched=True, objective=ride, **kw)
            self._ride = ride if (ride is not None and ride.S is not None) else None
        else:
            out_tea = None
            if not bool(getattr(o, "render_stu_first", True)) and stu.cuda_ray:
                with torch.no_grad():
                    out_tea = tea.render(rays_o, rays_d, staged=False, bg_color=bg_color, perturb=True, force_all_rays=False, **kw_stu)
                out_stu = stu.render(rays_o, rays_d, staged=False, bg_color=bg_color, perturb=True, force_all_rays=False,
                                     inherited_params=out_tea["inherited_params"], nears_fars=out_tea.get("nears_fars"), **kw)
            else:
                out_stu = stu.render(rays_o, rays_d, staged=False, bg_color=bg_color, perturb=True, force_all_rays=False, **kw_stu)
            if out_tea is None:
                with torch.no_grad():
                    out_tea = tea.render(rays_o, rays_d, staged=False, bg_color=bg_color, perturb=True, force_all_rays=False,
                                         inherited_params=out_stu["inherited_params"], nears_fars=out_stu.get("nears_fars"), **kw)
        self.loss_rate_fea_sc *= 0.995
        have_fea = stu.feature_sigma_color is not None and tea.feature_sigma_color is not None
        pred_stu, pred_tea = out_stu.get("image"), out_tea.get("image")
        fused = (self.fused_loss is not None and o.loss_type == "normL2" and have_fea and pred_stu is not None and pred_stu.is_cuda
                 and "stage1" not in out_stu and "stage2" not in out_stu
                 and min(o.loss_rate_color, o.loss_rate_sigma, self.loss_rate_fea_sc, o.loss_rate_rgb) > 0.0
                 and stu.feature_sigma_color.dtype == torch.float32 and tea.feature_sigma_color.dtype == torch.float32
                 and stu.feature_sigma_color.dim() == 2 and stu.feature_sigma_color.shape[-1] == 16
                 and tea.feature_sigma_color.shape == stu.feature_sigma_color.shape)
        fused_nofea = (not fused and not have_fea and self.fused_loss is not None and o.loss_type == "normL2" and pred_stu is not None
                       and pred_stu.is_cuda and "stage1" not in out_stu and "stage2" not in out_stu
                       and min(o.loss_rate_color, o.loss_rate_sigma, o.loss_rate_rgb) > 0.0
                       and getattr(stu, "sigma_l", None) is not None and getattr(tea, "sigma_l", None) is not None
                       and stu.sigma_l.dim() == 1 and tea.sigma_l.shape == stu.sigma_l.shape
                       and not (o.l1_reg_weight > 0.0 and o.model_type == "vm"))
        assert fused or not getattr(getattr(self, "_ride", None), "decayed", False), \
            "the compositing launch applied the feature rate's decay for a fused objective that is not being formed"
        if not fused:
            self.fea_rate.mul_(0.995) if not fused_nofea else None
        info = {}
        loss = 0.0
        if "stage1" in out_stu and self.loss_rate_fea_sc > 0.0 and have_fea:
            l_fea = self.loss(stu.feature_sigma_color, tea.feature_sigma_color)
            info["fea"] = l_fea.detach()
            return loss + self.fea_rate * l_fea, info, None, None
        if "stage2" in out_stu:
            l_col = self.loss(stu.color_l, tea.color_l)
            l_sig = self.loss(stu.sigma_l, tea.sigma_l)
            if o.loss_rate_color > 0.0:
                loss = loss + o.loss_rate_color * l_col
            if o.loss_rate_sigma > 0.0:
                loss = loss + o.loss_rate_sigma * l_sig
            if self.loss_rate_fea_sc > 0.0 and have_fea:
                loss = loss + self.fea_rate * self.loss(stu.feature_sigma_color, tea.feature_sigma_color)
            info.update(color=l_col.detach(), sigma=l_sig.detach())
            return loss, info, None, None

        if fused_nofea:
            l3, norms = self.fused_loss(pred_stu, pred_tea, stu.sigma_l.float().unsqueeze(-1), tea.sigma_l.float().unsqueeze(-1),
                                        stu.color_l.float(), tea.color_l.float(), self.rates, self.dp, fea_decay=0.995)
            info["rgb"] = norms[0]
            return l3, info, pred_stu, pred_tea
        if fused:
            extra = None
            if o.l1_reg_weight > 0.0 and o.model_type == "vm":
                if self.flat_opt:
                    self._l1_term(partials_only=True)
                    extra = self.optimizer.l1_partials(1.0 / self.dp.world_size)
            add_l1 = o.l1_reg_weight > 0.0 and o.model_type == "vm" and extra is None
            ride = self.__dict__.pop("_ride", None)
            rkw = {} if ride is None else {"ride": ride}
            l4, norms = self.fused_loss(pred_stu, pred_tea, stu.feature_sigma_color, tea.feature_sigma_color, stu.color_l.float(),
                                        tea.color_l.float(), self.rates, self.dp, fea_decay=0.995, extra=extra, **rkw)
            loss = l4
            if add_l1:
                loss = loss + self._l1_term()
            info["rgb"] = norms[0]
            return loss, info, pred_stu, pred_tea
        if o.loss_type == "normL2":
            l_rgb = self.dp.global_norm_l2(pred_tea - pred_stu)
        elif o.loss_type == "normL1":
            l_rgb = self.dp.global_norm_l1(pred_tea - pred_stu)
        else:
            l_rgb = self.dp.global_mean((pred_tea.float() - pred_stu.float()) ** 2)
        loss = loss + l_rgb * o.loss_rate_rgb
        if o.l1_reg_weight > 0.0 and o.model_type == "vm":
            loss = loss + self._l1_term()
        if self.loss_rate_fea_sc > 0.0 and have_fea:
            loss = loss + self.fea_rate * self.loss(stu.feature_sigma_color, tea.feature_sigma_color)
        if o.loss_rate_color > 0.0:
            loss = loss + o.loss_rate_color * self.loss(stu.color_l, tea.color_l)
        if o.loss_rate_sigma > 0.0:
            loss = loss + o.loss_rate_sigma * self.loss(stu.sigma_l, tea.sigma_l)
        info["rgb"] = l_rgb.detach()
        return loss, info, pred_stu, pred_tea

    def train_step(self, rays_o, rays_d, bg_color, nears_fars=None):
        o, stu = self.opt, self.model_stu
        if getattr(o, "update_stu_extra", False) and stu.cuda_ray and self.global_step % o.update_extra_interval == 0:
            with torch.autocast(self.device_type, dtype=torch.float16, enabled=self.fp16 and self.device_type == "cuda"):
                stu.update_extra_state()
        self._zero_grads()
        with torch.autocast(self.device_type, dtype=torch.float16, enabled=self.fp16 and self.device_type == "cuda"):
            loss, info, pred_stu, pred_tea = self.compute_loss(rays_o, rays_d, bg_color, nears_fars)
        self._backward_and_step(loss)
        return loss.detach(), info, pred_stu, pred_tea

    def capture_step(self, batch_fn, steps_per_graph=1):
        def body():
            rays_o, rays_d, bg, *rest = batch_fn()
            with torch.autocast(self.device_type, dtype=torch.float16, enabled=self.fp16):
                return self.compute_loss(rays_o, rays_d, bg, *rest)
        warm = 3
        if self.flat_opt:
            self.optimizer.flush()
            self.sync_sharded_state()
        self._replay_owes_part_a = None
        self.fused_spans = None
        stage = self._stage_of(self.global_step)
        assert self._stage_of(self.global_step + warm) == stage, \
            "capture_step: the %d warm-up steps cross a stage boundary (global_step %d); step eagerly past it first" % (warm, self.global_step)
        stu_marches = bool(getattr(self.opt, "render_stu_first", True))
        if self.dp.enabled and self.dp.ingraph:
            try:
                pipe = os.environ.get("PVD_DP_PIPELINE", "1")
                if stu_marches and stage == 3 and steps_per_graph > 1 and (pipe == "2" or (pipe == "1" and self.dp.world_size > 1)):
                    out = self._capture_ingraph_pipelined(batch_fn, body, steps_per_graph)
                else:
                    out = self.capture(body, steps_per_graph=steps_per_graph)
            except Exception:
                self._after_failed_capture()
                self.dp.ingraph = False
                out = self.capture(body, warmup=0, steps_per_graph=1)
                self.capture_fallback = "segmented"
        elif self.dp.enabled and stu_marches and stage == 3 and os.environ.get("PVD_DP_OVERLAP", "1") != "0":
            out = self._capture_pipelined(batch_fn, body)
        elif not self.dp.enabled and stage == 3 and steps_per_graph > 1 and stu_marches and pvd_forked_graphs_ok():
            try:
                out = self._capture_ingraph_pipelined(batch_fn, body, steps_per_graph)
            except Exception:
                self._after_failed_capture()
                self.pipelined_ingraph = False
                self.capture_fallback = "back-to-back"
                out = self.capture(body, warmup=0, steps_per_graph=steps_per_graph)
        else:
            out = self.capture(body, steps_per_graph=steps_per_graph)
        self._captured_stage = self._stage_of(self.global_step)
        return out

    def _capture_ingraph_pipelined(self, batch_fn, body, steps_per_graph):
        assert self.device_type == "cuda" and (not self.dp.enabled or self.dp.ingraph)
        K = int(steps_per_graph)
        assert K >= 2, "with one step per graph the step's own scatter would still read the samples the carried prefix overwrites"
        side = torch.cuda.Stream()
        side.wait_stream(torch.cuda.current_stream())
        with torch.cuda.stream(side):
            for _ in range(3):
                self._zero_grads()
                out = body()
                self._backward(out[0])
                self._exchange()
                self._optimize()
                self.scheduler.step()
                self.global_step += 1
                del out
        torch.cuda.current_stream().wait_stream(side)
        torch.cuda.synchronize()
        self._graph_zeroes = False
        if not self.dp.enabled:
            self._fold_launches(True)
        with torch.cuda.stream(side):
            carried = CarriedPrefix(self.prefetch(batch_fn))
        torch.cuda.current_stream().wait_stream(side)
        torch.cuda.synchronize()
        late = (self.flat_opt and os.environ.get("PVD_ADAMW_SPLIT", "late") == "late" and (not self.dp.enabled or self.dp.ingraph))
        scaled = bool(getattr(self.scaler, "_enabled", False))
        self._replay_owes_part_a = None
        fh = getattr(getattr(self.model_stu, "ops", None), "fused_head", None)
        pack_ahead = getattr(fh, "prepack_train_image", None)
        self.fused_spans = None
        if getattr(self, "record_fused_spans", False) and getattr(self.model_tea, "model_type", "") == "hash":
            import pvd_hip
            self.fused_spans = torch.tensor([list(pvd_hip.FUSED_SPAN_INIT)] * K, dtype=torch.int64, device=self.device)
        if late and not self.optimizer.begin_two_part(defer=True):
            late = False
        if late:
            self.optimizer.carry_last = True
        if self.dp.enabled and self.flat_opt:
            self.prepare_exchange()
            if self._exchange_mode(self._grad_compactor()) is not None:
                self._fold_launches(True)
        cap = SegmentedCapture(self.device)
        self.dp.capture = cap
        branch = torch.cuda.Stream(self.device)
        try:
            with cap:
                main = torch.cuda.current_stream()
                pre = carried.pre
                try:
                    for k in range(K):
                        branch.wait_stream(main)
                        if self.fused_spans is not None:
                            self.model_tea._fused_span = self.fused_spans[k]
                        with torch.cuda.stream(branch):
                            if pack_ahead is not None and pack_ahead(self.model_stu):
                                packed = torch.cuda.Event()
                                packed.record(branch)
                                self.model_stu._before_head = lambda packed=packed: main.wait_event(packed)
                            marched = self.prefetch_march(batch_fn)
                            if late:
                                self.optimizer.run_part_a()
                                if k == 0:
                                    self.optimizer.run_carried_part_a(scaled)
                            pre_next = self.prefetch_teacher(marched)
                            if k + 1 == K:
                                carried.store(pre_next)
                        self._zero_grads(first_in_recording=k == 0)
                        with torch.autocast(self.device_type, dtype=torch.float16, enabled=self.fp16):
                            self._static_out = self.compute_loss(None, None, None, pre=pre)
                        self._backward(self._static_out[0])
                        if os.environ.get("PVD_TEST_FAIL_IN_CAPTURE") in ("1", "forked") and k == 1:
                            raise RuntimeError("forced failure inside the forked capture (PVD_TEST_FAIL_IN_CAPTURE)")
                        self._exchange()
                        if late and k + 1 == K:
                            self.optimizer._next_step_is_last = True
                        self._optimize()
                        main.wait_stream(branch)
                        pre = pre_next
                    if late:
                        self.optimizer._part_a_owed = None
                        self._replay_owes_part_a = scaled
                except Exception:
                    self.model_stu.__dict__.pop("_before_head", None)
                    self.model_stu.__dict__.pop("_train_image_ready", None)
                    main.wait_stream(branch)
                    raise
        finally:
            self.dp.capture = None
            self._fold_launches(False)
            if late:
                self.optimizer.end_two_part()
        self._cap = cap
        self.steps_per_replay = K
        self._captured_occ_epoch = self._marching_model().occ_epoch if (self.flat_opt and self.optimizer.touched is not None) else None
        self.pipelined_ingraph = True
        self.pipeline_fork = "start"
        self.adamw_split = "late" if (late and getattr(self.optimizer, "_graph_is_two_part", False)) else "0"
        return self._static_out

    def _capture_pipelined(self, batch_fn, body):
        side = torch.cuda.Stream()
        side.wait_stream(torch.cuda.current_stream())
        with torch.cuda.stream(side):
            for _ in range(3):
                self._zero_grads()
                out = body()
                self._backward(out[0])
                self._exchange()
                self._optimize()
                self.scheduler.step()
                self.global_step += 1
                del out
        torch.cuda.current_stream().wait_stream(side)
        torch.cuda.synchronize()
        self._g_prefix = torch.cuda.CUDAGraph()
        with torch.cuda.graph(self._g_prefix, capture_error_mode="thread_local"):
            self._pre = dict(self.prefetch(batch_fn), replayed_ahead=True)

        def body_pre():
            with torch.autocast(self.device_type, dtype=torch.float16, enabled=self.fp16):
                return self.compute_loss(None, None, None, pre=self._pre)
        self._overlap_with_exchange = self._g_prefix.replay
        try:
            out = self.capture(body_pre, warmup=0)
        finally:
            self._overlap_with_exchange = None
        self._g_prefix.replay()
        return out

    def _stage_of(self, step):
        st = self.opt.stage_iters
        return 1 if step < st["stage1"] else (2 if step < st["stage2"] else 3)

    def replay_step(self):
        assert self._stage_of(self.global_step) == self._captured_stage, "stage changed: capture_step() again"
        assert self._stage_of(self.global_step + self.steps_per_replay - 1) == self._captured_stage, "the replay would cross a stage boundary"
        loss, info, pred_stu, pred_tea = self.replay()
        return loss.detach(), info, pred_stu, pred_tea


class TeacherTrainer(_TrainerBase):

    def __init__(self, opt, model, device, fp16=True, dp=None):
        lr = opt.lr * (0.1 if opt.model_type == "mlp" else 1.0)
        super().__init__(opt, model, lr, device, fp16, dp, exp_decay=True)
        self.model.train()

# ... 141 lines not shown
```

aaai2023-pvd_amd/pvd/workload.py:

```python
import numpy as np
import torch

from .config import PVDConfig
from .network import NeRFNetwork
from .scene import BLENDER_INTRINSICS, ChairScene, forward_facing_train_poses, get_rays, packbits_torch, rand_poses, synthetic_poses
from .trainer import DistillTrainer, RayDP, TeacherTrainer


def renderer_kwargs(opt):
    return dict(bound=opt.bound, cuda_ray=opt.cuda_ray, density_scale=1, min_near=opt.min_near, density_thresh=opt.density_thresh,
                bg_radius=opt.bg_radius, grid_size=opt.grid_size)


def make_model(ops, opt, model_type, is_teacher, device, teacher_variant=False):
    m = NeRFNetwork(ops, model_type=model_type, args=opt, is_teacher=is_teacher, teacher_variant=teacher_variant,
                    **renderer_kwargs(opt))
    return m.to(device)


def install_occupancy(model, scene, opt):
    dev = model.density_grid.device
    grid = scene.density_grid(opt.grid_size, opt.bound, model.cascade, device=dev)
    model.density_grid.copy_(grid)
    model.density_bitfield.copy_(packbits_torch(grid, min(float(grid.clamp(min=0).mean()), opt.density_thresh)))
    model.mean_density = float(grid.clamp(min=0).mean())
    model.note_occupancy_changed()
    return grid


class AnalyticTarget:

    def __init__(self, ops, scene, proxy):
        self.rm, self.scene, self.proxy = ops.raymarching, scene, proxy

    @torch.no_grad()
    def __call__(self, rays_o, rays_d, bg_color, max_steps=1024):
        p, rm = self.proxy, self.rm
        o, d = rays_o.contiguous().view(-1, 3), rays_d.contiguous().view(-1, 3)
        nears, fars = rm.near_far_from_aabb(o, d, p.aabb_train, p.min_near)
        xyzs, dirs, deltas, rays = rm.march_rays_train(o, d, p.bound, p.density_bitfield, p.cascade, p.grid_size, nears, fars,
                                                       None, -1, False, 128, True, 0, max_steps)
        sig, col = self.scene.sigma(xyzs), self.scene.color(xyzs, dirs)
        ws, _, img = rm.composite_rays_train(sig, col, deltas, rays)
        return (img + (1 - ws).unsqueeze(-1) * bg_color).view(*rays_o.shape[:-1], 3)


def measure_mean_count(model, poses, opt, n_poses=8, generator=None):
    rm = model.rm
    tot = 0
    for k in range(n_poses):
        r = get_rays(poses[k:k + 1], BLENDER_INTRINSICS, 800, 800, opt.num_rays, generator=generator)
        o, d = r["rays_o"].contiguous().view(-1, 3), r["rays_d"].contiguous().view(-1, 3)
        nears, fars = rm.near_far_from_aabb(o, d, model.aabb_train, model.min_near)
        counter = torch.zeros(2, dtype=torch.int32, device=o.device)
        rm.march_rays_train(o, d, model.bound, model.density_bitfield, model.cascade, model.grid_size, nears, fars, counter, -1,
                            True, 128, True, opt.dt_gamma, opt.max_steps)
        tot += int(counter[0].item())
    return tot // n_poses


class DistillWorkload:

    def __init__(self, ops, device, opt=None, teacher_pretrain_steps=0, seed=0, dp=None, start_stage="stage3", thicken=0.08, scene_scale=1.0):
        self.ops, self.device = ops, torch.device(device)
        self.opt = opt or PVDConfig()
        opt = self.opt
        torch.manual_seed(seed)
        self.rng = np.random.RandomState(seed)
        self.gen = torch.Generator(device=self.device)
        self.dp_rank = dp.rank if dp else 0
        self.gen.manual_seed(seed + 1000 * self.dp_rank)
        self.scene = ChairScene(thicken=thicken, scale=scene_scale)
        orig = forward_facing_train_poses(self.rng) if opt.data_type == "llff" else None
        self.poses = torch.from_numpy(rand_poses(opt.data_type, self.rng, original_poses=orig, scale=opt.scale)).to(self.device)

        self.tea = make_model(ops, opt, opt.teacher_type, True, self.device)
        install_occupancy(self.tea, self.scene, opt)
        self.target = AnalyticTarget(ops, self.scene, self.tea)
        self.teacher_psnr = None
        if teacher_pretrain_steps > 0:
            self.pretrain_teacher(teacher_pretrain_steps)

        self.stu = make_model(ops, opt, opt.model_type, False, self.device)
        src = self.tea.state_dict()
        dst = self.stu.state_dict()
        self.stu.load_state_dict({k: v for k, v in src.items() if k in dst and dst[k].shape == v.shape}, strict=False)
        mc = measure_mean_count(self.tea, self.poses, opt, generator=self.gen)
        self.tea.mean_count = self.stu.mean_count = mc
        self.trainer = DistillTrainer(opt, self.tea, self.stu, self.device, fp16=opt.fp16, dp=dp)
        if start_stage == "stage3":
            self.trainer.global_step = opt.stage_iters["stage2"]
        elif start_stage == "stage2":
            self.trainer.global_step = max(opt.stage_iters["stage1"], 0)
        self.step_idx = 0

    def pretrain_teacher(self, steps):
        opt = self.opt
        topt = PVDConfig(**{**opt.__dict__, "model_type": opt.teacher_type, "iters": max(steps, 1), "update_extra_interval": 10 ** 9,
                            "stage_iters": {"stage1": -1, "stage2": -1}})
        self.tea.teacher_variant = True
        self.tea.args = self.tea.opt = topt
        tr = TeacherTrainer(topt, self.tea, self.device, fp16=opt.fp16)
        self.tea.mean_count = measure_mean_count(self.tea, self.poses, opt, generator=self.gen)
        last = None
        for it in range(steps):
            r = get_rays(self.poses[it % len(self.poses)][None], BLENDER_INTRINSICS, 800, 800, opt.num_rays, generator=self.gen)
            bg = torch.rand(1, opt.num_rays, 3, device=self.device, generator=self.gen)
            gt = self.target(r["rays_o"], r["rays_d"], bg)
            _, pred = tr.train_step(r["rays_o"], r["rays_d"], gt, bg)
            last = (pred, gt)
        from .trainer import psnr
        self.teacher_psnr = float(psnr(last[0].detach(), last[1]))
        self.tea.teacher_variant = False
        self.tea.args = self.tea.opt = opt
        for p in self.tea.parameters():
            p.grad = None

    def next_batch(self):
        opt = self.opt
        pose = self.poses[self.step_idx % len(self.poses)][None]
        self.step_idx += 1
        r = get_rays(pose, BLENDER_INTRINSICS, 800, 800, opt.num_rays, generator=self.gen)
        bg = torch.rand(1, opt.num_rays, 3, device=self.device, generator=self.gen)
        return r["rays_o"], r["rays_d"], bg

    def device_batch(self):
        opt = self.opt
        mk = getattr(self.ops, "make_batch", None)
        if mk is not None:
            if not hasattr(self, "_batch_state"):
                self._batch_state = torch.zeros(3, dtype=torch.int64, device=self.device)
                self._poses_c = self.poses.float().contiguous()
                self._batch_seed = 0x5eed + 1000003 * int(torch.cuda.initial_seed() % (2 ** 31)) + 0x9E3779B1 * self.dp_rank
            return mk(self._poses_c, self._batch_state, self._batch_seed, BLENDER_INTRINSICS, 800, 800, opt.num_rays,
                      self.stu.aabb_train, self.stu.min_near)
        if not hasattr(self, "_pose_idx"):
            self._pose_idx = torch.zeros(1, dtype=torch.long, device=self.device)
        pose = self.poses.index_select(0, self._pose_idx)
        self._pose_idx.add_(1).remainder_(len(self.poses))
        fused = getattr(self.ops, "get_rays", None)
        r = fused(pose, BLENDER_INTRINSICS, 800, 800, opt.num_rays) if fused else get_rays(pose, BLENDER_INTRINSICS, 800, 800, opt.num_rays)
        bg = torch.rand(1, opt.num_rays, 3, device=self.device)
        return r["rays_o"], r["rays_d"], bg

    def enable_graph(self, steps_per_graph=1):
        assert not self.opt.update_stu_extra, "update_stu_extra rewrites the occupancy grid between steps: run eagerly"
        self.trainer.capture_step(self.device_batch, steps_per_graph=steps_per_graph)
        self._graph = True

    @property
    def steps_per_call(self):
        return self.trainer.steps_per_replay if getattr(self, "_graph", False) else 1

    def step(self):
        if getattr(self, "_graph", False):
            return self.trainer.replay_step()
        if getattr(self, "_eager_device_batches", False):
            return self.trainer.train_step(*self.device_batch())
        return self.trainer.train_step(*self.next_batch())
```

aaai2023-pvd_amd/pvd_hip/__init__.py:

```python
import ctypes
import os
import sys
import types

_HWQ = "GPU_MAX_HW_QUEUES"
_torch_loaded = sys.modules.get("torch")
if _HWQ in os.environ:
    HW_QUEUES, HW_QUEUES_SOURCE = os.environ[_HWQ], "caller"
elif os.environ.get("PVD_HW_QUEUES", "") == "keep":
    HW_QUEUES, HW_QUEUES_SOURCE = None, "left to the runtime (PVD_HW_QUEUES=keep)"
elif _torch_loaded is not None and _torch_loaded.cuda.is_initialized():
    HW_QUEUES, HW_QUEUES_SOURCE = None, "runtime started before pvd_hip was imported"
else:
    os.environ[_HWQ] = "2"
    HW_QUEUES, HW_QUEUES_SOURCE = "2", "package default"

import torch


def forked_graphs_ok():
    force = os.environ.get("PVD_FORKED_GRAPHS")
    if force in ("0", "1"):
        return force == "1"
    try:
        return HW_QUEUES is not None and int(HW_QUEUES) == 2
    except ValueError:
        return False


_PKG_ROOT = os.path.dirname(os.path.dirname(os.path.abspath(__file__)))
LIB_PATH = os.environ.get("PVD_HIP_LIB") or os.path.join(_PKG_ROOT, "libpvd_hip.so")

if not os.path.exists(LIB_PATH):
    raise ImportError(
        "libpvd_hip.so not found at %s -- build it with `python -c 'import __graft_entry__ as g; g.build()'` "
        "or `make -C aaai2023-pvd_amd/csrc` (there is no CPU fallback)" % LIB_PATH
    )

_lib = ctypes.CDLL(LIB_PATH)
_lib.pvd_status_string.restype = ctypes.c_char_p
_lib.pvd_last_hip_error.restype = ctypes.c_char_p
_lib.pvd_abi_version.restype = ctypes.c_int

ABI_VERSION = int(_lib.pvd_abi_version())

_u32, _f32, _int, _vp = ctypes.c_uint32, ctypes.c_float, ctypes.c_int, ctypes.c_void_p
_u64 = ctypes.c_uint64

PVD_F32, PVD_F16 = 0, 1

ENTRY_POINTS = (
    "pvd_abi_version", "pvd_status_string", "pvd_last_hip_error",
    "pvd_near_far_from_aabb", "pvd_polar_from_ray", "pvd_morton3D", "pvd_morton3D_invert", "pvd_packbits",
    "pvd_march_rays_train", "pvd_march_rays_train_ws", "pvd_march_workspace_bytes", "pvd_composite_rays_train_forward", "pvd_composite_rays_train_backward",
    "pvd_march_rays", "pvd_composite_rays", "pvd_compact_rays", "pvd_infer_round_begin", "pvd_infer_compact", "pvd_infer_march", "pvd_infer_composite", "pvd_occ_sample", "pvd_occ_update", "pvd_occ_finish", "pvd_occ_sample_replay", "pvd_occ_update_ordered",
    "pvd_mse_forward", "pvd_grid_encode_forward", "pvd_grid_encode_forward_affine", "pvd_grid_encode_forward_affine_pack", "pvd_grid_encode_backward", "pvd_grid_encode_backward_affine",
    "pvd_sh_encode_forward", "pvd_sh_encode_backward",
    "pvd_vm_forward", "pvd_vm_forward_pack_rider", "pvd_vm_backward", "pvd_infer_image_vm", "pvd_infer_image_plenoxel", "pvd_vm_backward_rider", "pvd_head_backward_defer", "pvd_plenoxel_forward", "pvd_plenoxel_backward", "pvd_get_rays", "pvd_make_ray_batch",
    "pvd_head_forward", "pvd_hash_head_forward_fused", "pvd_hash_head_forward_fused_span", "pvd_infer_image_hash",
    "pvd_head_backward", "pvd_head_backward_workspace_floats", "pvd_head_image_halfs", "pvd_head_pack_weights",
    "pvd_composite_rays_train_bg_forward", "pvd_composite_rays_train_bg_backward",
    "pvd_composite_objective_blocks", "pvd_composite_objective_blocks_fixed", "pvd_composite_objective_forward", "pvd_composite_objective_backward",
    "pvd_distill_sumsq", "pvd_distill_loss_final", "pvd_distill_sumsq_backward", "pvd_distill_loss_backward", "pvd_grid_set_variant", "pvd_grid_set_fwd_kernel",
    "pvd_adamw_step", "pvd_adamw_step_ex", "pvd_adamw_lazy_flush", "pvd_freq_encode", "pvd_mlp_head_forward_fused", "pvd_check_finite", "pvd_check_finite_f16", "pvd_check_finite_mixed", "pvd_l1_ranges", "pvd_segments_op", "pvd_segments_gather_zero_check",
)
ENTRY_POINTS_MLP = ("pvd_mlp_head_forward_fused_rows", "pvd_infer_image_mlp")
ENTRY_POINTS_METRICS = ("pvd_image_metrics_workspace_floats", "pvd_image_metrics")
ENTRY_POINTS_DATA = ("pvd_image_batch", "pvd_error_map_update")
ENTRY_POINTS_MARCH = ("pvd_occ_coarse_mask", "pvd_march_rays_train_mask")
ENTRY_POINTS_MESH = ("pvd_mesh_workspace_bytes", "pvd_mesh_count", "pvd_mesh_emit")
ENTRY_POINTS_COMPONENTS = ("pvd_components_label", "pvd_components_filter", "pvd_components_neighbours")
ENTRY_POINTS_MESH_ATTR = ("pvd_mesh_normals",)
ENTRY_POINTS_MESH_DIST = ("pvd_mesh_dist_workspace_bytes", "pvd_mesh_dist_build", "pvd_mesh_dist_query")
ENTRY_POINTS_MESH_SIMPLIFY = ("pvd_mesh_simplify_workspace_bytes", "pvd_mesh_simplify_count", "pvd_mesh_simplify_emit")
ENTRY_POINTS_MESH_RAY = ("pvd_mesh_ray_workspace_bytes", "pvd_mesh_ray_count", "pvd_mesh_ray_build", "pvd_mesh_ray_cast")
ENTRY_POINTS_MESH_SMOOTH = ("pvd_mesh_smooth_workspace_bytes", "pvd_mesh_smooth_build", "pvd_mesh_smooth_run")
for _name in (ENTRY_POINTS + ENTRY_POINTS_MLP + ENTRY_POINTS_METRICS + ENTRY_POINTS_DATA + ENTRY_POINTS_MARCH + ENTRY_POINTS_MESH
              + ENTRY_POINTS_COMPONENTS + ENTRY_POINTS_MESH_ATTR + ENTRY_POINTS_MESH_DIST + ENTRY_POINTS_MESH_SIMPLIFY + ENTRY_POINTS_MESH_RAY
              + ENTRY_POINTS_MESH_SMOOTH):
    if _name not in ("pvd_status_string", "pvd_last_hip_error"):
        getattr(_lib, _name).restype = ctypes.c_int
_lib.pvd_march_workspace_bytes.restype = ctypes.c_size_t
_lib.pvd_mesh_workspace_bytes.restype = ctypes.c_size_t
_lib.pvd_mesh_dist_workspace_bytes.restype = ctypes.c_size_t
_lib.pvd_mesh_simplify_workspace_bytes.restype = ctypes.c_size_t
_lib.pvd_mesh_ray_workspace_bytes.restype = ctypes.c_size_t
_lib.pvd_mesh_smooth_workspace_bytes.restype = ctypes.c_size_t
_lib.pvd_composite_objective_blocks.restype = ctypes.c_uint32
_lib.pvd_composite_objective_blocks_fixed.restype = ctypes.c_uint32


class PvdHipError(RuntimeError):
    pass


def _check(status, what):
    if status != 0:
        msg = _lib.pvd_status_string(status).decode()
        hip = _lib.pvd_last_hip_error().decode()
        raise PvdHipError("%s: %s%s" % (what, msg, (" [%s]" % hip) if hip else ""))


def _dev(*tensors):
    dev = None
    for t in tensors:
        if t is None:
            continue
        if not t.is_cuda:
            raise PvdHipError("tensor must be a CUDA(HIP) tensor -- libpvd_hip has no CPU path")
        if not t.is_contiguous():
            raise PvdHipError("tensor must be contiguous")
        if dev is None:
            dev = t.device
        elif t.device != dev:
            raise PvdHipError("all tensors must be on the same device")
    return dev


def _want(t, dtype, name):
    if t.dtype != dtype:
        raise PvdHipError("%s must be %s, got %s" % (name, dtype, t.dtype))


def _p(t):
    return _vp(t.data_ptr()) if t is not None else _vp(0)


def _stream(dev):
    return _vp(torch.cuda.current_stream(dev).cuda_stream)


class KernelTimer:

    def __init__(self, names, external=False):
        self.names = set(names)
        self.external = bool(external)
        self.events = {n: [] for n in self.names}
        self.meta = {n: [] for n in self.names}
        self.captured = {n: [] for n in self.names}

    def __enter__(self):
        global _timer
        _timer = self
        return self

    def __exit__(self, *exc):
        global _timer
        _timer = None

    def launches(self, name):
        return len(self.events[name])

    def total_ms(self, name):
        torch.cuda.synchronize()
        return float(sum(a.elapsed_time(b) for a, b in self.events[name]))

    def mean_ms(self, name):
        n = self.launches(name)
        return self.total_ms(name) / n if n else float("nan")

    def captured_ms(self, name):
        torch.cuda.synchronize()
        return [float(a.elapsed_time(b)) for (a, b), c in zip(self.events[name], self.captured[name]) if c]


_timer = None


def _invoke(fn_name, dev, *args, meta=None):
    with torch.cuda.device(dev):
        t = _timer
        if t is not None and fn_name in t.names:
            kw = {"external": True} if t.external else {}
            a, b = torch.cuda.Event(enable_timing=True, **kw), torch.cuda.Event(enable_timing=True, **kw)
            a.record()
            status = getattr(_lib, fn_name)(*args, _stream(dev))
            b.record()
            t.events[fn_name].append((a, b))
            t.meta[fn_name].append(meta)
            t.captured[fn_name].append(bool(torch.cuda.is_current_stream_capturing()))
            return status
        return getattr(_lib, fn_name)(*args, _stream(dev))


def _call(fn_name, dev, *args):
    _check(_invoke(fn_name, dev, *args), fn_name)


def _f32_all(**named):
    for k, v in named.items():
        _want(v, torch.float32, k)


def near_far_from_aabb(rays_o, rays_d, aabb, N, min_near, nears, fars):
    dev = _dev(rays_o, rays_d, aabb, nears, fars)
    _f32_all(rays_o=rays_o, rays_d=rays_d, aabb=aabb, nears=nears, fars=fars)
    _call("pvd_near_far_from_aabb", dev, _p(rays_o), _p(rays_d), _p(aabb), _u32(N), _f32(min_near), _p(nears), _p(fars))


def get_rays(pose, fx, fy, cx, cy, inds, W, N, rays_o, rays_d):
    dev = _dev(pose, inds, rays_o, rays_d)
    _f32_all(pose=pose, rays_o=rays_o, rays_d=rays_d)
    if inds is not None:
        _want(inds, torch.int64, "inds")
    _call("pvd_get_rays", dev, _p(pose), _f32(fx), _f32(fy), _f32(cx), _f32(cy), _p(inds), _u32(W), _u32(N), _p(rays_o), _p(rays_d))


def make_ray_batch(poses, state, seed, fx, fy, cx, cy, H, W, N, aabb, min_near, inds, rays_o, rays_d, bg, nears, fars):
    dev = _dev(poses, state, aabb, inds, rays_o, rays_d, bg, nears, fars)
    _f32_all(poses=poses, aabb=aabb, rays_o=rays_o, rays_d=rays_d, nears=nears, fars=fars)
    _want(state, torch.int64, "state")
    if inds is not None:
        _want(inds, torch.int64, "inds")
    if bg is not None:
        _want(bg, torch.float32, "bg")
    if state.numel() < 3:
        raise PvdHipError("state must hold 3 int64 values")
    _call("pvd_make_ray_batch", dev, _p(poses), _u32(poses.shape[0]), _p(state), ctypes.c_uint64(int(seed) & (2 ** 64 - 1)), _f32(fx),
          _f32(fy), _f32(cx), _f32(cy), _u32(H), _u32(W), _u32(N), _p(aabb), _f32(min_near), _p(inds), _p(rays_o), _p(rays_d), _p(bg),
          _p(nears), _p(fars))


def polar_from_ray(rays_o, rays_d, radius, N, coords):
    dev = _dev(rays_o, rays_d, coords)
    _f32_all(rays_o=rays_o, rays_d=rays_d, coords=coords)
    _call("pvd_polar_from_ray", dev, _p(rays_o), _p(rays_d), _f32(radius), _u32(N), _p(coords))


def morton3D(coords, N, indices):
    dev = _dev(coords, indices)
    _want(coords, torch.int32, "coords"), _want(indices, torch.int32, "indices")
    _call("pvd_morton3D", dev, _p(coords), _u32(N), _p(indices))


# ... 576 lines not shown


def _mlp_stream_halfs(n_before, n_after):
    return 4 * (64 * 72 + 64) + (n_before + n_after) * 4 * (64 * 264 + 64) + 4 * (64 * 328 + 64) + (32 * 264 + 32)


def mlp_head_forward_fused(pts16, wstream, n_before, n_after, dirs, M, Wa1, Wa2, Wc1, Wc2, Wc3, clip_sigma_min, clip_max, sigma, rgb, feat16,
                           image=None, rows_dev=None):
    dev = _dev(pts16, wstream, dirs, Wa1, Wa2, Wc1, Wc2, Wc3, sigma, rgb, feat16, image)
    _want(pts16, torch.float16, "pts16"), _want(wstream, torch.float16, "wstream")
    _f32_all(dirs=dirs, Wa1=Wa1, Wa2=Wa2, Wc1=Wc1, Wc2=Wc2, Wc3=Wc3, sigma=sigma, rgb=rgb, feat16=feat16)
    if pts16.shape != (M, 64) or not pts16.is_contiguous() or not wstream.is_contiguous():
        raise PvdHipError("pts16 must be a contiguous [M, 64] f16 tensor")
    need = _mlp_stream_halfs(n_before, n_after)
    if wstream.numel() != need:
        raise PvdHipError("weight stream has %d halfs, the layer structure needs %d" % (wstream.numel(), need))
    _check_image(KIND_HASH_CONST, image)
    if rows_dev is not None:
        if dirs.shape[0] < M or sigma.numel() < M or rgb.numel() < 3 * M or feat16.numel() < 16 * M:
            raise PvdHipError("buffers shorter than M rows")
        _call("pvd_mlp_head_forward_fused_rows", dev, _p(pts16), _u32(M), _p(wstream), _u32(n_before), _u32(n_after), _p(dirs), _p(Wa1), _p(Wa2),
              _p(Wc1), _p(Wc2), _p(Wc3), _p(image), _f32(clip_sigma_min), _f32(clip_max), _p(sigma), _p(rgb), _p(feat16), _rows_dev(rows_dev, dev))
        return
    _call("pvd_mlp_head_forward_fused", dev, _p(pts16), _u32(M), _p(wstream), _u32(n_before), _u32(n_after), _p(dirs), _p(Wa1), _p(Wa2),
          _p(Wc1), _p(Wc2), _p(Wc3), _p(image), _f32(clip_sigma_min), _f32(clip_max), _p(sigma), _p(rgb), _p(feat16))


def infer_image_mlp(rays_o, rays_d, nears, fars, bitfield, bound, dt_gamma, max_steps, C, H, sigma_scale, freq_bands, wstream, n_before, n_after,
                    Wa1, Wa2, Wc1, Wc2, Wc3, clip_sigma_min, clip_max, workspace, weights_sum, depth, image_out, image=None):
    dev = _dev(rays_o, rays_d, nears, fars, bitfield, wstream, Wa1, Wa2, Wc1, Wc2, Wc3, workspace, weights_sum, depth, image_out, image)
    _want(wstream, torch.float16, "wstream"), _want(workspace, torch.int32, "workspace"), _want(bitfield, torch.uint8, "bitfield")
    _f32_all(rays_o=rays_o, rays_d=rays_d, nears=nears, fars=fars, Wa1=Wa1, Wa2=Wa2, Wc1=Wc1, Wc2=Wc2, Wc3=Wc3, weights_sum=weights_sum,
             depth=depth, image_out=image_out)
    N = rays_o.shape[0]
    if rays_d.shape[0] < N or nears.numel() < N or fars.numel() < N or weights_sum.numel() < N or depth.numel() < N or image_out.numel() < 3 * N \
            or workspace.numel() < 2 * N + 12:
        raise PvdHipError("buffers shorter than N rays")
    need = _mlp_stream_halfs(n_before, n_after)
    if wstream.numel() != need:
        raise PvdHipError("weight stream has %d halfs, the layer structure needs %d" % (wstream.numel(), need))
    _check_image(KIND_HASH_CONST, image)
    bands = (ctypes.c_float * max(1, len(freq_bands)))(*[float(f) for f in freq_bands])
    _call("pvd_infer_image_mlp", dev, _p(rays_o), _p(rays_d), _p(nears), _p(fars), _u32(N), _p(bitfield), _f32(bound), _f32(dt_gamma),
          _u32(max_steps), _u32(C), _u32(H), _f32(sigma_scale), bands, _u32(len(freq_bands)), _p(wstream), _u32(n_before), _u32(n_after),
          _p(Wa1), _p(Wa2), _p(Wc1), _p(Wc2), _p(Wc3), _p(image), _f32(clip_sigma_min), _f32(clip_max), _p(workspace), _p(weights_sum),
          _p(depth), _p(image_out))


KIND_HASH_CONST = 0


def note_weights_changed(params):
    for p in params:
        p._pvd_epoch = getattr(p, "_pvd_epoch", 0) + 1


def weights_key(tensors):
    return tuple((t._version, t.data_ptr(), getattr(t, "_pvd_epoch", 0)) for t in tensors if t is not None)


def head_image_halfs(kind):
    return int(_lib.pvd_head_image_halfs(_int(kind)))


def _check_image(kind, image):
    if image is not None and (image.dtype != torch.float16 or image.numel() < head_image_halfs(kind)):
        raise PvdHipError("weight image must be float16 with pvd_head_image_halfs(kind) elements")


def head_pack_weights(kind, Wa1, Wa2, Wc1, Wc2, Wc3, image=None):
    dev = _dev(Wa1, Wa2, Wc1, Wc2, Wc3, image)
    _f32_all(Wa1=Wa1, Wc1=Wc1, Wc2=Wc2, Wc3=Wc3)
    if image is None:
        image = torch.empty(head_image_halfs(kind), dtype=torch.float16, device=dev)
    _check_image(kind, image)
    _call("pvd_head_pack_weights", dev, _int(kind), _p(Wa1), _p(Wa2), _p(Wc1), _p(Wc2), _p(Wc3), _p(image))
    return image


def head_backward_workspace_floats(kind, M):
    return int(_lib.pvd_head_backward_workspace_floats(_int(kind), _u32(M)))


def head_backward(kind, x0, sigma_raw, dirs, M, Wa1, Wa2, Wc1, Wc2, Wc3, clip_sigma_min, clip_feat_min, clip_max, g_sigma, g_rgb, g_feat16,
                  g_sigma_raw, g_x0, gWa1, gWa2, gWc1, gWc2, gWc3, workspace, image=None, g_rgb2=None, defer_reduce=None):
    dev = _dev(x0, sigma_raw, dirs, Wa1, Wa2, Wc1, Wc2, Wc3, g_sigma, g_rgb, g_feat16, g_sigma_raw, g_x0, workspace)
    _want(x0, torch.float16, "x0"), _want(g_x0, torch.float16, "g_x0")
    _f32_all(dirs=dirs, Wa1=Wa1, Wc1=Wc1, Wc2=Wc2, Wc3=Wc3, g_sigma=g_sigma, g_rgb=g_rgb,
             gWa1=gWa1, gWc1=gWc1, gWc2=gWc2, gWc3=gWc3, workspace=workspace)
    for t in (sigma_raw, Wa2, g_sigma_raw, gWa2, g_feat16):
        if t is not None:
            _want(t, torch.float32, "head_backward argument")
    for t in (gWa1, gWa2, gWc1, gWc2, gWc3):
        if t is not None and not (t.is_cuda and t.is_contiguous()):
            raise PvdHipError("weight gradient buffers must be contiguous HIP tensors")
    if workspace.numel() < head_backward_workspace_floats(kind, M):
        raise PvdHipError("workspace too small")
    _check_image(kind, image)
    if g_rgb2 is not None:
        _dev(g_rgb, g_rgb2)
        _f32_all(g_rgb2=g_rgb2)
        if g_rgb2.shape != g_rgb.shape:
            raise PvdHipError("g_rgb2 must have the shape of g_rgb")
    if defer_reduce is not None:
        rider = _HeadDwRider()
        _call("pvd_head_backward_defer", dev, _int(kind), _p(x0), _p(sigma_raw), _p(dirs), _u32(M), _p(Wa1), _p(Wa2), _p(Wc1), _p(Wc2), _p(Wc3),
              _p(image), _f32(clip_sigma_min), _f32(clip_feat_min), _f32(clip_max), _p(g_sigma), _p(g_rgb), _p(g_rgb2), _p(g_feat16),
              _p(g_sigma_raw), _p(g_x0), _p(gWa1), _p(gWa2), _p(gWc1), _p(gWc2), _p(gWc3), _p(workspace), ctypes.byref(rider))
        defer_reduce["rider"], defer_reduce["keep"] = rider, (workspace, gWa1, gWc1, gWc2, gWc3)
        return
    _call("pvd_head_backward", dev, _int(kind), _p(x0), _p(sigma_raw), _p(dirs), _u32(M), _p(Wa1), _p(Wa2), _p(Wc1), _p(Wc2), _p(Wc3),
          _p(image), _f32(clip_sigma_min), _f32(clip_feat_min), _f32(clip_max), _p(g_sigma), _p(g_rgb), _p(g_rgb2), _p(g_feat16), _p(g_sigma_raw), _p(g_x0),
          _p(gWa1), _p(gWa2), _p(gWc1), _p(gWc2), _p(gWc3), _p(workspace))


class _HeadDwRider(ctypes.Structure):
    _fields_ = [("partials", ctypes.c_void_p), ("nblocks", ctypes.c_uint32), ("gWa1", ctypes.c_void_p), ("gWc1", ctypes.c_void_p),
                ("gWc2", ctypes.c_void_p), ("gWc3", ctypes.c_void_p), ("found_inf", ctypes.c_void_p)]


def freq_encode(x, freq_bands, include_input=True, out_dtype=torch.float32, row_stride=None):
    dev = _dev(x)
    _want(x, torch.float32, "x")
    if x.dim() != 2 or not x.is_contiguous():
        raise PvdHipError("x must be a contiguous [M, D] tensor")
    M, D = x.shape
    width = (D if include_input else 0) + 2 * D * len(freq_bands)
    stride = width if row_stride is None else int(row_stride)
    if stride < width or len(freq_bands) > 16:
        raise PvdHipError("row_stride must cover the encoding; at most 16 frequencies")
    out = torch.empty(M, stride, dtype=out_dtype, device=x.device)
    bands = (ctypes.c_float * max(1, len(freq_bands)))(*[float(f) for f in freq_bands])
    _call("pvd_freq_encode", dev, _p(x), _u32(M), _u32(D), bands, _u32(len(freq_bands)), _int(int(bool(include_input))), _p(out),
          _int(_table_dtype(out, "out")), _u32(stride))
    return out


def composite_rays_train_bg_forward(sigmas, rgbs, deltas, rays, M, N, bg, bg_scalar, nears, fars, depth_eps, weights_sum, depth, image,
                                    budget_dev=None):
    dev = _dev(sigmas, rgbs, deltas, rays, bg, nears, fars, weights_sum, depth, image, budget_dev)
    _f32_all(sigmas=sigmas, rgbs=rgbs, deltas=deltas, nears=nears, fars=fars, weights_sum=weights_sum, depth=depth, image=image)
    _call("pvd_composite_rays_train_bg_forward", dev, _p(sigmas), _p(rgbs), _p(deltas), _p(rays), _u32(M), _u32(N), _p(bg), _f32(bg_scalar),
          _p(nears), _p(fars), _f32(depth_eps), _p(weights_sum), _p(depth), _p(image), _p(budget_dev))


def composite_rays_train_bg_backward(grad_weights_sum, grad_image, sigmas, rgbs, deltas, rays, weights_sum, image, M, N, bg, bg_scalar,
                                     grad_sigmas, grad_rgbs, fresh=False, budget_dev=None):
    dev = _dev(grad_weights_sum, grad_image, sigmas, rgbs, deltas, rays, weights_sum, image, bg, grad_sigmas, grad_rgbs, budget_dev)
    _f32_all(grad_image=grad_image, sigmas=sigmas, rgbs=rgbs, deltas=deltas, weights_sum=weights_sum, image=image)
    _call("pvd_composite_rays_train_bg_backward", dev, _p(grad_weights_sum), _p(grad_image), _p(sigmas), _p(rgbs), _p(deltas), _p(rays),
          _p(weights_sum), _p(image), _u32(M), _u32(N), _p(bg), _f32(bg_scalar), _p(grad_sigmas), _p(grad_rgbs), _u32(1 if fresh else 0),
          _p(budget_dev))



def composite_objective_blocks(N, rows, fixed=False):
    if fixed:
        return int(_lib.pvd_composite_objective_blocks_fixed(_u32(N)))
    return int(_lib.pvd_composite_objective_blocks(_u32(N), _u32(rows)))


def composite_objective_forward(sigmas, rgbs, deltas, rays, M, N, bg, bg_scalar, nears, fars, depth_eps, weights_sum, depth, image,
                                img_t, fea_s, fea_t, col_s, col_t, S4, budget_dev=None, rates_decay=None, fea_decay=1.0, fixed_parts=False):
    dev = _dev(sigmas, rgbs, deltas, rays, bg, nears, fars, weights_sum, depth, image, budget_dev, img_t, fea_s, fea_t, col_s, col_t, S4)
    _f32_all(sigmas=sigmas, rgbs=rgbs, deltas=deltas, nears=nears, fars=fars, weights_sum=weights_sum, depth=depth, image=image,
             img_t=img_t, fea_s=fea_s, fea_t=fea_t, col_s=col_s, col_t=col_t, S4=S4)
    _want(rays, torch.int32, "rays")
    rows = fea_s.shape[0]
    if fea_s.dim() != 2 or fea_s.shape[1] != 16 or fea_t.shape != fea_s.shape or col_s.shape != (rows, 3) or col_t.shape != (rows, 3):
        raise PvdHipError("feature rows must be [rows,16], colour rows [rows,3]")
    if img_t.numel() != 3 * N or S4.numel() < 4 + 4 * composite_objective_blocks(N, rows, fixed_parts):
        raise PvdHipError("teacher image must be [N,3]; S4 must hold 4 + 4 * composite_objective_blocks floats")
    if budget_dev is not None:
        _want(budget_dev, torch.int32, "budget_dev")
    _call("pvd_composite_objective_forward", dev, _p(sigmas), _p(rgbs), _p(deltas), _p(rays), _u32(M), _u32(N), _p(bg), _f32(bg_scalar),
          _p(nears), _p(fars), _f32(depth_eps), _p(weights_sum), _p(depth), _p(image), _p(budget_dev), _p(img_t), _p(fea_s), _p(fea_t),
          _p(col_s), _p(col_t), _u32(rows), _p(S4), _p(rates_decay), _f32(fea_decay), _u32(2 if fixed_parts else 0))


def composite_objective_backward(grad_ws, sigmas, rgbs, deltas, rays, weights_sum, image, M, N, bg, bg_scalar, grad_sigmas, grad_rgbs,
                                 img_t, fea_s, fea_t, col_s, col_t, coef4, upstream, g_fea, g_col, fresh=False, budget_dev=None, finish=None,
                                 fixed_parts=False):
    dev = _dev(grad_ws, sigmas, rgbs, deltas, rays, weights_sum, image, bg, grad_sigmas, grad_rgbs, budget_dev, img_t, fea_s, fea_t, col_s,
               col_t, coef4, upstream, g_fea, g_col)
    _f32_all(sigmas=sigmas, rgbs=rgbs, deltas=deltas, weights_sum=weights_sum, image=image, grad_sigmas=grad_sigmas, grad_rgbs=grad_rgbs,
             img_t=img_t, fea_s=fea_s, fea_t=fea_t, col_s=col_s, col_t=col_t, coef4=coef4, upstream=upstream, g_fea=g_fea, g_col=g_col)
    _want(rays, torch.int32, "rays")
    rows = fea_s.shape[0]
    if g_fea.shape != fea_s.shape or g_col.shape != col_s.shape or fea_s.shape[1] != 16:
        raise PvdHipError("gradient buffers must have the shapes of the student tensors ([rows,16], [rows,3])")
    rates4 = extra = S4 = loss = norms4 = None
    if finish is not None:
        rates4, extra, S4, loss, norms4 = finish
        _dev(rates4, extra, S4, loss, norms4)
        _f32_all(rates4=rates4, S4=S4, loss=loss, norms4=norms4)
        if extra is not None:
            _want(extra, torch.float32, "extra")
        if S4.numel() < 4 + 4 * composite_objective_blocks(N, rows, fixed_parts):
            raise PvdHipError("S4 must be the buffer composite_objective_forward filled")
    _call("pvd_composite_objective_backward", dev, _p(grad_ws), _p(sigmas), _p(rgbs), _p(deltas), _p(rays), _p(weights_sum), _p(image),
          _u32(M), _u32(N), _p(bg), _f32(bg_scalar), _p(grad_sigmas), _p(grad_rgbs), _u32((1 if fresh else 0) | (2 if fixed_parts else 0)),
          _p(budget_dev), _p(img_t),
          _p(fea_s), _p(fea_t), _p(col_s), _p(col_t), _u32(rows), _p(coef4), _p(upstream), _p(g_fea), _p(g_col), _p(rates4), _p(extra),
          _u32(extra.numel() if extra is not None else 0), _p(S4), _p(loss), _p(norms4))

def _distill_shapes(img_s, img_t, fea_s, fea_t, col_s, col_t):
    if fea_s.dim() != 2 or fea_t.shape != fea_s.shape:
        raise PvdHipError("feature tensors must both be [M, W], got %s and %s" % (tuple(fea_s.shape), tuple(fea_t.shape)))
    M = fea_s.shape[0]
    if tuple(col_s.shape) != (M, 3) or tuple(col_t.shape) != (M, 3):
        raise PvdHipError("colour tensors must be [M, 3] with M = %d, got %s and %s" % (M, tuple(col_s.shape), tuple(col_t.shape)))
    if img_s.numel() != img_t.numel():
        raise PvdHipError("student and teacher images differ in size")
    return M, fea_s.shape[1]


def mse_forward(pred, target, loss, dloss):
    dev = _dev(pred, target, loss, dloss)
    _f32_all(pred=pred, target=target, loss=loss, dloss=dloss)
    if pred.numel() != target.numel() or dloss.numel() != pred.numel() or pred.numel() == 0:
        raise PvdHipError("mse_forward: pred, target and dloss of one (non-empty) size expected")
    _call("pvd_mse_forward", dev, _p(pred), _p(target), _u32(pred.numel()), _p(loss), _p(dloss))


def distill_sumsq(img_s, img_t, fea_s, fea_t, col_s, col_t, S4, reduce=True, rates_decay=None, fea_decay=1.0):
    dev = _dev(img_s, img_t, fea_s, fea_t, col_s, col_t, S4, rates_decay)
    if rates_decay is not None:
        _want(rates_decay, torch.float32, "rates_decay")
    _f32_all(img_s=img_s, img_t=img_t, fea_s=fea_s, fea_t=fea_t, col_s=col_s, col_t=col_t, S4=S4)
    M, W = _distill_shapes(img_s, img_t, fea_s, fea_t, col_s, col_t)
    if S4.numel() < 4 + 4 * 1024:
        raise PvdHipError("S4 needs 4 + 4*1024 floats")
    _call("pvd_distill_sumsq", dev, _p(img_s), _p(img_t), _u32(img_s.numel()), _p(fea_s), _p(fea_t), _u32(M), _u32(W), _p(col_s), _p(col_t),
          _p(S4), _int(int(bool(reduce))), _p(rates_decay), _f32(fea_decay))


def distill_loss_backward(img_s, img_t, fea_s, fea_t, col_s, col_t, S4, rates4, upstream, loss, coef4, norms4, g_img, g_fea, g_col,
                          reduce=False, extra=None):
    dev = _dev(img_s, img_t, fea_s, fea_t, col_s, col_t, S4, rates4, upstream, loss, coef4, norms4, g_img, g_fea, g_col, extra)
    _f32_all(img_s=img_s, img_t=img_t, fea_s=fea_s, fea_t=fea_t, col_s=col_s, col_t=col_t, S4=S4, rates4=rates4, upstream=upstream, loss=loss,
             coef4=coef4, norms4=norms4, g_img=g_img, g_fea=g_fea, g_col=g_col)
    if extra is not None:
        _want(extra, torch.float32, "extra")
    M, W = _distill_shapes(img_s, img_t, fea_s, fea_t, col_s, col_t)
    if g_img.numel() != img_s.numel() or g_fea.shape != fea_s.shape or g_col.shape != col_s.shape:
        raise PvdHipError("gradient buffers must have the shapes of the student tensors")
    if S4.numel() < 4 + 4 * 1024:
        raise PvdHipError("S4 needs 4 + 4*1024 floats")
    _call("pvd_distill_loss_backward", dev, _p(img_s), _p(img_t), _u32(img_s.numel()), _p(fea_s), _p(fea_t), _u32(M), _u32(W), _p(col_s),
          _p(col_t), _p(S4), _int(int(bool(reduce))), _p(rates4), _p(extra), _u32(extra.numel() if extra is not None else 0), _p(upstream),
          _p(loss), _p(coef4), _p(norms4), _p(g_img), _p(g_fea), _p(g_col))


def distill_loss_final(S4, rates4, loss, coef4, norms4, n_img=0, M=0, reduce=False, fea_decay=1.0, extra=None):
    dev = _dev(S4, rates4, loss, coef4, norms4, extra)
    _f32_all(S4=S4, rates4=rates4, loss=loss, coef4=coef4, norms4=norms4)
    if extra is not None:
        _want(extra, torch.float32, "extra")
    nred = int(reduce) if (not isinstance(reduce, bool) and int(reduce) >= 2) else int(bool(reduce))
    if nred >= 2 and S4.numel() < 4 + 4 * nred:
        raise PvdHipError("S4 too small for %d partials" % nred)
    _call("pvd_distill_loss_final", dev, _p(S4), _u32(n_img), _u32(M), _int(nred), _p(rates4), _f32(fea_decay), _p(extra),
          _u32(extra.numel() if extra is not None else 0), _p(loss), _p(coef4), _p(norms4))


def distill_sumsq_backward(img_s, img_t, fea_s, fea_t, col_s, col_t, coef4, upstream, g_img, g_fea, g_col):
    dev = _dev(img_s, img_t, fea_s, fea_t, col_s, col_t, coef4, upstream, g_img, g_fea, g_col)
    _f32_all(img_s=img_s, img_t=img_t, fea_s=fea_s, fea_t=fea_t, col_s=col_s, col_t=col_t, coef4=coef4, upstream=upstream, g_img=g_img,
             g_fea=g_fea, g_col=g_col)
    M, W = _distill_shapes(img_s, img_t, fea_s, fea_t, col_s, col_t)
    if g_img.numel() != img_s.numel() or g_fea.shape != fea_s.shape or g_col.shape != col_s.shape:
        raise PvdHipError("gradient buffers must have the shapes of the student tensors")
    _call("pvd_distill_sumsq_backward", dev, _p(img_s), _p(img_t), _u32(img_s.numel()), _p(fea_s), _p(fea_t), _u32(M), _u32(W), _p(col_s),
          _p(col_t), _p(coef4), _p(upstream), _p(g_img), _p(g_fea), _p(g_col))


class _AdamwExtras(ctypes.Structure):
    _fields_ = [("sched_kind", ctypes.c_int32), ("sched_T", ctypes.c_float), ("sched_param", ctypes.c_float),
                ("base_lr", ctypes.c_void_p), ("sched_step", ctypes.c_void_p), ("n_l1", ctypes.c_uint32),
                ("l1_begin_host", ctypes.POINTER(ctypes.c_uint64)), ("l1_end_host", ctypes.POINTER(ctypes.c_uint64)),
                ("l1_coef_host", ctypes.POINTER(ctypes.c_float)), ("amp_scale", ctypes.c_void_p), ("amp_growth_tracker", ctypes.c_void_p),
                ("amp_growth", ctypes.c_double), ("amp_backoff", ctypes.c_double), ("amp_interval", ctypes.c_int32),
                ("g16", ctypes.c_void_p), ("g16_begin", ctypes.c_uint64), ("g16_end", ctypes.c_uint64),
                ("l1_next", ctypes.c_void_p), ("l1_next_scale", ctypes.c_float), ("cold_bits", ctypes.c_void_p),
                ("lazy_log", ctypes.c_void_p), ("lazy_count", ctypes.c_void_p), ("lazy_capacity", ctypes.c_uint32),
                ("warm_groups", ctypes.c_void_p), ("n_warm_groups", ctypes.c_uint32), ("warm_zero_grad_from", ctypes.c_uint32),
                ("snapshot", ctypes.c_void_p), ("replay", ctypes.c_void_p),
                ("zero_grad_after", ctypes.c_uint32), ("arrivals", ctypes.c_void_p),
                ("compact_grad", ctypes.c_void_p), ("compact_param_out", ctypes.c_void_p), ("tail_clear", ctypes.c_void_p),
                ("tail_clear_stride", ctypes.c_uint32), ("tail_clear_n", ctypes.c_uint32)]


def _u64_array(vals):
    return (ctypes.c_uint64 * len(vals))(*[int(v) for v in vals])


def adamw_step(p, g, m, v, segment_ends, lr, beta1, beta2, eps, weight_decay, step, grad_scale=None, found_inf=None, schedule=None,
               l1_ranges=None, amp_update=None, half_grad=None, l1_next=None, cold_bits=None, lazy=None, snapshot=None, replay=None, zero_after=False, arrivals=None,
               compact_grad=None, compact_param_out=None, tail_clear=None):
    dev = _dev(p, g, m, v, lr, step, grad_scale, found_inf)
    _f32_all(p=p, g=g, m=m, v=v, lr=lr, step=step)
    ends = _u64_array(segment_ends)
    ex = None
    if (schedule is not None or l1_ranges or amp_update is not None or half_grad is not None or cold_bits is not None or zero_after
            or arrivals is not None or snapshot is not None):
        ex = _AdamwExtras()
# ... 605 lines not shown
```

Measured before the change: 11.65 million rays/s.

## Batch ray generation, marching and compositing over G steps in grouped launches

Adds grouped variants of ray-batch generation, the march count and write kernels, and forward compositing. They use blockIdx.y to process G independent step segments in one launch, and a shared state counter advances pose and batch by G. The aim is to amortise launch overhead and raise occupancy for the small 4096-ray batches, for example by precomputing several steps' teacher prefix work at once. The cost is G-times larger buffers and workspace, plus extra Python wiring through a batch_group_fn hook whose activation is not fully visible.

```diff
diff --git a/aaai2023-pvd_amd/csrc/raymarching.hip b/aaai2023-pvd_amd/csrc/raymarching.hip
--- a/aaai2023-pvd_amd/csrc/raymarching.hip
+++ b/aaai2023-pvd_amd/csrc/raymarching.hip
@@ -1,6 +1,6 @@
 #include "dda.h"
 #include "rays.h"
-#include "../../include/pvd_hip_march.h"
+#include "../../include/pvd_hip_prefix.h"
 
 #include <float.h>
 
@@ -48,6 +48,27 @@
     for (int r = 0; r < 3; r++) { rays_o[3 * (size_t)n + r] = o[r]; rays_d[3 * (size_t)n + r] = d[r]; }
 }
 
+__device__ __forceinline__ void make_batch_ray(const float *__restrict__ poses, long long pose_idx, long long batch, uint64_t seed, float fx,
+                                               float fy, float cx, float cy, uint32_t H, uint32_t W, uint32_t n,
+                                               const float *__restrict__ aabb, float min_near, int64_t *__restrict__ inds,
+                                               float *__restrict__ rays_o, float *__restrict__ rays_d, float *__restrict__ bg,
+                                               float *__restrict__ nears, float *__restrict__ fars) {
+    Pcg32 g;
+    g.seed(seed + 0x9E3779B97F4A7C15ull * (uint64_t)(batch + 1));
+    g.advance(4ull * n);
+    const int64_t k = (int64_t)(((uint64_t)g.next() * (uint64_t)(H * W)) >> 32);
+    float o[3], d[3];
+    ray_of_pixel(poses + 16 * (size_t)pose_idx, fx, fy, cx, cy, k, W, o, d);
+    if (inds) inds[n] = k;
+#pragma unroll
+    for (int r = 0; r < 3; r++) { rays_o[3 * (size_t)n + r] = o[r]; rays_d[3 * (size_t)n + r] = d[r]; }
+    if (bg) {
+#pragma unroll
+        for (int r = 0; r < 3; r++) bg[3 * (size_t)n + r] = g.next_float();
+    }
+    near_far_of(o, d, aabb, min_near, nears[n], fars[n]);
+}
+
 __global__ void __launch_bounds__(kBlock) k_make_ray_batch(const float *__restrict__ poses, uint32_t P, long long *__restrict__ state,
                                                            uint64_t seed, float fx, float fy, float cx, float cy, uint32_t H, uint32_t W,
                                                            uint32_t N, const float *__restrict__ aabb, float min_near,
@@ -56,22 +77,7 @@
                                                            float *__restrict__ fars) {
     const uint32_t n = blockIdx.x * kBlock + threadIdx.x;
     const long long pose_idx = state[0], batch = state[1];
-    if (n < N) {
-        Pcg32 g;
-        g.seed(seed + 0x9E3779B97F4A7C15ull * (uint64_t)(batch + 1));
-        g.advance(4ull * n);
-        const int64_t k = (int64_t)(((uint64_t)g.next() * (uint64_t)(H * W)) >> 32);
-        float o[3], d[3];
-        ray_of_pixel(poses + 16 * (size_t)pose_idx, fx, fy, cx, cy, k, W, o, d);
-        if (inds) inds[n] = k;
-#pragma unroll
-        for (int r = 0; r < 3; r++) { rays_o[3 * (size_t)n + r] = o[r]; rays_d[3 * (size_t)n + r] = d[r]; }
-        if (bg) {
-#pragma unroll
-            for (int r = 0; r < 3; r++) bg[3 * (size_t)n + r] = g.next_float();
-        }
-        near_far_of(o, d, aabb, min_near, nears[n], fars[n]);
-    }
+    if (n < N) make_batch_ray(poses, pose_idx, batch, seed, fx, fy, cx, cy, H, W, n, aabb, min_near, inds, rays_o, rays_d, bg, nears, fars);
     __syncthreads();
     if (threadIdx.x == 0) {
         __threadfence();
@@ -79,6 +85,30 @@
         if (done == gridDim.x - 1) {
             state[0] = (pose_idx + 1) % (long long)P;
             state[1] = batch + 1;
+            state[2] = 0;
+        }
+    }
+}
+
+__global__ void __launch_bounds__(kBlock) k_make_ray_batch_group(const float *__restrict__ poses, uint32_t P, long long *__restrict__ state,
+                                                                 uint64_t seed, float fx, float fy, float cx, float cy, uint32_t H, uint32_t W,
+                                                                 uint32_t N, const float *__restrict__ aabb, float min_near,
+                                                                 int64_t *__restrict__ inds, float *__restrict__ rays_o,
+                                                                 float *__restrict__ rays_d, float *__restrict__ bg, float *__restrict__ nears,
+                                                                 float *__restrict__ fars) {
+    const uint32_t n = blockIdx.x * kBlock + threadIdx.x, j = blockIdx.y, G = gridDim.y;
+    const long long pose0 = state[0], batch0 = state[1];
+    const size_t base = (size_t)j * N;
+    if (n < N)
+        make_batch_ray(poses, (pose0 + (long long)j) % (long long)P, batch0 + (long long)j, seed, fx, fy, cx, cy, H, W, n, aabb, min_near,
+                       inds ? inds + base : nullptr, rays_o + 3 * base, rays_d + 3 * base, bg ? bg + 3 * base : nullptr, nears + base, fars + base);
+    __syncthreads();
+    if (threadIdx.x == 0) {
+        __threadfence();
+        const unsigned long long done = atomicAdd(reinterpret_cast<unsigned long long *>(state + 2), 1ull);
+        if (done == (unsigned long long)gridDim.x * G - 1ull) {
+            state[0] = (pose0 + (long long)G) % (long long)P;
+            state[1] = batch0 + (long long)G;
             state[2] = 0;
         }
     }
@@ -386,7 +416,7 @@
     return true;
 }
 
-__global__ void __launch_bounds__(kBlock) k_march_count_wave(const float *__restrict__ rays_o, const float *__restrict__ rays_d,
+__device__ __forceinline__ void march_count_wave_body(const float *__restrict__ rays_o, const float *__restrict__ rays_d,
                                                              const uint8_t *__restrict__ grid, float bound, float dt_gamma, uint32_t max_steps,
                                                              uint32_t N, uint32_t C, uint32_t H, const float *__restrict__ nears,
                                                              const float *__restrict__ fars, int32_t *__restrict__ rays, uint32_t perturb,
@@ -433,6 +463,28 @@
 #endif
 }
 
+__global__ void __launch_bounds__(kBlock) k_march_count_wave(const float *__restrict__ rays_o, const float *__restrict__ rays_d,
+                                                             const uint8_t *__restrict__ grid, float bound, float dt_gamma, uint32_t max_steps,
+                                                             uint32_t N, uint32_t C, uint32_t H, const float *__restrict__ nears,
+                                                             const float *__restrict__ fars, int32_t *__restrict__ rays, uint32_t perturb,
+                                                             MarchRayRecords *__restrict__ records, const int32_t *__restrict__ counter,
+                                                             uint32_t fresh, const uint8_t *__restrict__ coarse_mask) {
+    march_count_wave_body(rays_o, rays_d, grid, bound, dt_gamma, max_steps, N, C, H, nears, fars, rays, perturb, records, counter, fresh,
+                          coarse_mask);
+}
+
+__global__ void __launch_bounds__(kBlock) k_march_count_wave_group(const float *__restrict__ rays_o, const float *__restrict__ rays_d,
+                                                                   const uint8_t *__restrict__ grid, float bound, float dt_gamma,
+                                                                   uint32_t max_steps, uint32_t N, uint32_t C, uint32_t H,
+                                                                   const float *__restrict__ nears, const float *__restrict__ fars,
+                                                                   int32_t *__restrict__ rays, uint32_t perturb,
+                                                                   MarchRayRecords *__restrict__ records, const int32_t *__restrict__ counter,
+                                                                   uint32_t fresh, const uint8_t *__restrict__ coarse_mask) {
+    const size_t base = (size_t)blockIdx.y * N;
+    march_count_wave_body(rays_o + 3 * base, rays_d + 3 * base, grid, bound, dt_gamma, max_steps, N, C, H, nears + base, fars + base,
+                          rays + 3 * base, perturb, records + base + blockIdx.y, counter + 2 * (size_t)blockIdx.y, fresh, coarse_mask);
+}
+
 __global__ void __launch_bounds__(kBlock) k_march_write_wave(const float *__restrict__ rays_o, const float *__restrict__ rays_d,
                                                              const uint8_t *__restrict__ grid, float bound, float dt_gamma, uint32_t max_steps,
                                                              uint32_t N, uint32_t C, uint32_t H, uint32_t M,
@@ -473,7 +525,7 @@
 }
 
 
-__global__ void __launch_bounds__(kBlock) k_march_write_records(const float *__restrict__ rays_o, const float *__restrict__ rays_d,
+__device__ __forceinline__ void march_write_records_body(const float *__restrict__ rays_o, const float *__restrict__ rays_d,
                                                                const uint8_t *__restrict__ grid, float bound, float dt_gamma, uint32_t max_steps,
                                                                uint32_t N, uint32_t C, uint32_t H, uint32_t M,
                                                                const float *__restrict__ nears, const float *__restrict__ fars,
@@ -581,6 +633,32 @@
     }
 }
 
+__global__ void __launch_bounds__(kBlock) k_march_write_records(const float *__restrict__ rays_o, const float *__restrict__ rays_d,
+                                                               const uint8_t *__restrict__ grid, float bound, float dt_gamma, uint32_t max_steps,
+                                                               uint32_t N, uint32_t C, uint32_t H, uint32_t M,
+                                                               const float *__restrict__ nears, const float *__restrict__ fars,
+                                                               float *__restrict__ xyzs, float *__restrict__ dirs, float *__restrict__ deltas,
+                                                               int32_t *__restrict__ rays, uint32_t perturb,
+                                                               const MarchRayRecords *__restrict__ records, int32_t *__restrict__ counter,
+                                                               uint32_t fresh, const int32_t *__restrict__ budget) {
+    march_write_records_body(rays_o, rays_d, grid, bound, dt_gamma, max_steps, N, C, H, M, nears, fars, xyzs, dirs, deltas, rays, perturb,
+                             records, counter, fresh, budget);
+}
+
+__global__ void __launch_bounds__(kBlock) k_march_write_records_group(const float *__restrict__ rays_o, const float *__restrict__ rays_d,
+                                                                     const uint8_t *__restrict__ grid, float bound, float dt_gamma,
+                                                                     uint32_t max_steps, uint32_t N, uint32_t C, uint32_t H, uint32_t M,
+                                                                     const float *__restrict__ nears, const float *__restrict__ fars,
+                                                                     float *__restrict__ xyzs, float *__restrict__ dirs, float *__restrict__ deltas,
+                                                                     int32_t *__restrict__ rays, uint32_t perturb,
+                                                                     const MarchRayRecords *__restrict__ records, int32_t *__restrict__ counter,
+                                                                     uint32_t fresh, const int32_t *__restrict__ budget, uint32_t budget_stride) {
+    const size_t base = (size_t)blockIdx.y * N, sbase = (size_t)blockIdx.y * M;
+    march_write_records_body(rays_o + 3 * base, rays_d + 3 * base, grid, bound, dt_gamma, max_steps, N, C, H, M, nears + base, fars + base,
+                             xyzs + 3 * sbase, dirs + 3 * sbase, deltas + 2 * sbase, rays + 3 * base, perturb, records + base + blockIdx.y,
+                             counter + 2 * (size_t)blockIdx.y, fresh, budget ? budget + (size_t)blockIdx.y * budget_stride : nullptr);
+}
+
 
 
 __device__ __forceinline__ float wave_incl_scan_add(float v, uint32_t lane) {
@@ -696,12 +774,12 @@
     for (uint32_t i = tid; i < ob.rows * 3u; i += stride) ob.g_col[i] = c_col * (ob.col_s[i] - ob.col_t[i]);
 }
 
-template <bool EPI, bool OBJ = false>
-__global__ void __launch_bounds__(kBlock) k_composite_fwd_wave(const float *__restrict__ sigmas, const float *__restrict__ rgbs,
-                                                               const float *__restrict__ deltas, const int32_t *__restrict__ rays,
-                                                               uint32_t M, uint32_t N, float *__restrict__ weights_sum,
-                                                               float *__restrict__ depth, float *__restrict__ image, CompositeEpilogue ep,
-                                                               CompositeObjective ob = CompositeObjective{}) {
+template <bool EPI, bool OBJ>
+__device__ __forceinline__ void composite_fwd_wave_body(const float *__restrict__ sigmas, const float *__restrict__ rgbs,
+                                                        const float *__restrict__ deltas, const int32_t *__restrict__ rays,
+                                                        uint32_t M, uint32_t N, float *__restrict__ weights_sum,
+                                                        float *__restrict__ depth, float *__restrict__ image, const CompositeEpilogue &ep,
+                                                        const CompositeObjective &ob) {
     __shared__ float obj_sh[kBlock / kWave];
     if (OBJ && blockIdx.x >= ob.ray_blocks) {
         if (ob.rates_decay && blockIdx.x == ob.ray_blocks && threadIdx.x == 0) ob.rates_decay[1] *= ob.fea_decay;
@@ -767,6 +845,29 @@
 }
 
 template <bool EPI, bool OBJ = false>
+__global__ void __launch_bounds__(kBlock) k_composite_fwd_wave(const float *__restrict__ sigmas, const float *__restrict__ rgbs,
+                                                               const float *__restrict__ deltas, const int32_t *__restrict__ rays,
+                                                               uint32_t M, uint32_t N, float *__restrict__ weights_sum,
+                                                               float *__restrict__ depth, float *__restrict__ image, CompositeEpilogue ep,
+                                                               CompositeObjective ob = CompositeObjective{}) {
+    composite_fwd_wave_body<EPI, OBJ>(sigmas, rgbs, deltas, rays, M, N, weights_sum, depth, image, ep, ob);
+}
+
+__global__ void __launch_bounds__(kBlock) k_composite_fwd_wave_group(const float *__restrict__ sigmas, const float *__restrict__ rgbs,
+                                                                     const float *__restrict__ deltas, const int32_t *__restrict__ rays,
+                                                                     uint32_t M, uint32_t N, float *__restrict__ weights_sum,
+                                                                     float *__restrict__ depth, float *__restrict__ image, CompositeEpilogue ep,
+                                                                     uint32_t budget_stride) {
+    const size_t base = (size_t)blockIdx.y * N, sbase = (size_t)blockIdx.y * M;
+    if (ep.bg) ep.bg += 3 * base;
+    ep.nears += base;
+    ep.fars += base;
+    if (ep.budget) ep.budget += (size_t)blockIdx.y * budget_stride;
+    composite_fwd_wave_body<true, false>(sigmas + sbase, rgbs + 3 * sbase, deltas + 2 * sbase, rays + 3 * base, M, N, weights_sum + base,
+                                         depth + base, image + 3 * base, ep, CompositeObjective{});
+}
+
+template <bool EPI, bool OBJ = false>
 __global__ void __launch_bounds__(kBlock) k_composite_bwd_wave(const float *__restrict__ grad_ws, const float *__restrict__ grad_image,
                                                                const float *__restrict__ sigmas, const float *__restrict__ rgbs,
                                                                const float *__restrict__ deltas, const int32_t *__restrict__ rays,
@@ -1201,6 +1302,62 @@
     return check_launch();
 }
 
+constexpr uint32_t kMaxGroup = 65535;
+
+int pvd_make_ray_batch_group(const float *poses, uint32_t P, int64_t *state, uint64_t seed, float fx, float fy, float cx, float cy, uint32_t H,
+                             uint32_t W, uint32_t N, uint32_t G, const float *aabb, float min_near, int64_t *inds, float *rays_o, float *rays_d,
+                             float *bg, float *nears, float *fars, pvd_stream_t stream) {
+    if (N == 0 || G == 0) return PVD_OK;
+    PVD_REQUIRE(poses && P > 0 && state && aabb && rays_o && rays_d && nears && fars && H > 0 && W > 0 && G <= kMaxGroup);
+    PVD_REQUIRE((uint64_t)H * W < (1ull << 32));
+    hipLaunchKernelGGL(k_make_ray_batch_group, dim3(div_up(N, kBlock), G), dim3(kBlock), 0, (hipStream_t)stream, poses, P, (long long *)state,
+                       seed, fx, fy, cx, cy, H, W, N, aabb, min_near, inds, rays_o, rays_d, bg, nears, fars);
+    return check_launch();
+}
+
+size_t pvd_march_group_workspace_bytes(uint32_t N, uint32_t G) { return (size_t)G * pvd_march_workspace_bytes(N); }
+
+int pvd_march_rays_train_group(const float *rays_o, const float *rays_d, const uint8_t *grid, float bound, float dt_gamma, uint32_t max_steps,
+                               uint32_t N, uint32_t G, uint32_t C, uint32_t H, uint32_t M, const float *nears, const float *fars, float *xyzs,
+                               float *dirs, float *deltas, int32_t *rays, int32_t *counter, uint32_t perturb, void *workspace,
+                               size_t workspace_bytes, uint32_t flags, const int32_t *budget_dev, uint32_t budget_stride,
+                               const uint8_t *coarse_mask, pvd_stream_t stream) {
+    hipStream_t s = (hipStream_t)stream;
+    const bool fresh = (flags & PVD_MARCH_FRESH) != 0;
+    if (G == 0) return PVD_OK;
+    PVD_REQUIRE(G <= kMaxGroup);
+    if (N == 0) {
+        if (fresh && M && xyzs && dirs && deltas && counter) {
+            (void)hipMemsetAsync(xyzs, 0, 3 * (size_t)G * M * sizeof(float), s); (void)hipMemsetAsync(dirs, 0, 3 * (size_t)G * M * sizeof(float), s);
+            (void)hipMemsetAsync(deltas, 0, 2 * (size_t)G * M * sizeof(float), s); (void)hipMemsetAsync(counter, 0, 2 * (size_t)G * sizeof(int32_t), s);
+        }
+        return PVD_OK;
+    }
+    PVD_REQUIRE(rays_o && rays_d && grid && nears && fars && xyzs && dirs && deltas && rays && counter);
+    PVD_REQUIRE(C >= 1 && C <= 16 && H >= 1 && H <= 1024 && max_steps >= 1);
+    PVD_REQUIRE(workspace && workspace_bytes >= pvd_march_group_workspace_bytes(N, G) && N <= kMarchFusedScanMaxRays);
+    MarchRayRecords *records = (MarchRayRecords *)workspace;
+    const dim3 g(div_up(N, kRaysPerBlock), G), b(kBlock);
+    if ((H & (H - 1u)) || H < PVD_COARSE_BLOCK) coarse_mask = nullptr;
+    hipLaunchKernelGGL(k_march_count_wave_group, g, b, 0, s, rays_o, rays_d, grid, bound, dt_gamma, max_steps, N, C, H, nears, fars, rays,
+                       perturb, records, counter, fresh ? 1u : 0u, coarse_mask);
+    hipLaunchKernelGGL(k_march_write_records_group, g, b, 0, s, rays_o, rays_d, grid, bound, dt_gamma, max_steps, N, C, H, M, nears, fars, xyzs,
+                       dirs, deltas, rays, perturb, records, counter, fresh ? 1u : 0u, budget_dev, budget_stride);
+    return check_launch();
+}
+
+int pvd_composite_rays_train_bg_forward_group(const float *sigmas, const float *rgbs, const float *deltas, const int32_t *rays, uint32_t M,
+                                              uint32_t N, uint32_t G, const float *bg, float bg_scalar, const float *nears, const float *fars,
+                                              float depth_eps, float *weights_sum, float *depth, float *image, const int32_t *budget_dev,
+                                              uint32_t budget_stride, pvd_stream_t stream) {
+    if (N == 0 || G == 0) return PVD_OK;
+    PVD_REQUIRE(sigmas && rgbs && deltas && rays && nears && fars && weights_sum && depth && image && G <= kMaxGroup);
+    const CompositeEpilogue ep{bg, bg_scalar, nears, fars, depth_eps, 0u, budget_dev};
+    hipLaunchKernelGGL(k_composite_fwd_wave_group, dim3(div_up(N, kBlock / kWave), G), dim3(kBlock), 0, (hipStream_t)stream, sigmas, rgbs,
+                       deltas, rays, M, N, weights_sum, depth, image, ep, budget_stride);
+    return check_launch();
+}
+
 int pvd_composite_rays_train_forward(const float *sigmas, const float *rgbs, const float *deltas, const int32_t *rays,
                                      uint32_t M, uint32_t N, float *weights_sum, float *depth, float *image,
                                      pvd_stream_t stream) {
diff --git a/aaai2023-pvd_amd/pvd/knobs.py b/aaai2023-pvd_amd/pvd/knobs.py
--- a/aaai2023-pvd_amd/pvd/knobs.py
+++ b/aaai2023-pvd_amd/pvd/knobs.py
@@ -9,6 +9,9 @@
                                 "(the reference's arithmetic for this gradient; 21 MB) or widened into the fp32 bucket first (42 MB; rounds 1-5)"),
     "PVD_DP_WIRE": ("f32", "f32 | f16 | bf16: width of the gradient on the wire (classic form only; measured -0.3 dB PSNR: opt-in)"),
     "PVD_STEPS_PER_GRAPH": ("", "bench.py: steps recorded per hipGraph launch (default: the largest of 20/10/5/4/2 dividing --steps)"),
+    "PVD_PREFIX_GROUP": ("20", "G: the student-independent prefix (batch, march, frozen teacher's forward and compositing) of G consecutive steps of a "
+                               "back-to-back multi-step recording as ONE launch per stage (include/pvd_hip_prefix.h); the largest divisor of the steps "
+                               "per graph up to G is used; 1 = per step; the forked recording and ray-DP keep 1 (pvd/trainer.py: capture_step)"),
     "PVD_HW_QUEUES": ("", "keep = do not set GPU_MAX_HW_QUEUES=2 at import (an integrator who owns that variable); the forked schedule is then refused "
                           "unless the caller exported 2 itself"),
 }
diff --git a/aaai2023-pvd_amd/pvd/ops.py b/aaai2023-pvd_amd/pvd/ops.py
--- a/aaai2023-pvd_amd/pvd/ops.py
+++ b/aaai2023-pvd_amd/pvd/ops.py
@@ -54,8 +54,16 @@
         pvd_hip.make_ray_batch(poses, state, seed, fx, fy, cx, cy, H, W, N, aabb, min_near, None, rays_o, rays_d, bg, nears, fars)
         return rays_o, rays_d, bg, (nears, fars)
 
+    def make_batch_group(poses, state, seed, intrinsics, H, W, N, G, aabb, min_near):
+        dev = poses.device
+        f = lambda *s: torch.empty(*s, dtype=torch.float32, device=dev)
+        rays_o, rays_d, bg, nears, fars = f(G, N, 3), f(G, N, 3), f(G, N, 3), f(G, N), f(G, N)
+        fx, fy, cx, cy = intrinsics
+        pvd_hip.make_ray_batch_group(poses, state, seed, fx, fy, cx, cy, H, W, N, G, aabb, min_near, None, rays_o, rays_d, bg, nears, fars)
+        return rays_o, rays_d, bg, (nears, fars)
+
     def freq_encode(x, bands, include_input=True, out_dtype=torch.float32, row_stride=None):
         return pvd_hip.freq_encode(x, bands, include_input, out_dtype, row_stride)
 
-    return types.SimpleNamespace(freq_encode=freq_encode, make_batch=make_batch, occupancy=pvd_hip.occupancy_backend, raymarching=raymarching, GridEncoder=gridencoder.GridEncoder, SHEncoder=shencoder.SHEncoder,
+    return types.SimpleNamespace(freq_encode=freq_encode, make_batch=make_batch, make_batch_group=make_batch_group, occupancy=pvd_hip.occupancy_backend, raymarching=raymarching, GridEncoder=gridencoder.GridEncoder, SHEncoder=shencoder.SHEncoder,
                                  vm_encode=vmencoder.vm_encode, vm_encode_infer=vmencoder.vm_encode_infer, plenoxel=plenoxel, get_rays=get_rays_fused, fused_head=fusedhead, distill_loss=_distill_loss(), mse_loss=_mse_loss(), flat_adamw=_flat_adamw(), device_type="cuda", name="hip")
diff --git a/aaai2023-pvd_amd/pvd/renderer.py b/aaai2023-pvd_amd/pvd/renderer.py
--- a/aaai2023-pvd_amd/pvd/renderer.py
+++ b/aaai2023-pvd_amd/pvd/renderer.py
@@ -351,6 +351,33 @@
         xyzs, dirs, deltas, rays = self._march_train(rays_o, rays_d, nears, fars, counter, perturb, force_all_rays, dt_gamma, max_steps, budget)
         return [xyzs, dirs, deltas, rays], (nears, fars)
 
+    def march_group(self, rays_o, rays_d, nears_fars, dt_gamma=0, perturb=False, max_steps=1024):
+        import pvd_hip
+        G, N = rays_o.shape[0], rays_o.shape[1]
+        assert self.mean_count > 0 and rays_o.is_cuda, "a group is marched into fixed rows: needs a measured mean_count"
+        nears, fars = nears_fars
+        budget = self._budget()
+        M = self.mean_count + (128 - self.mean_count % 128)
+        budget_dev = None
+        if budget is not None:
+            M, budget_dev = int(budget[0]), budget[1]
+        dev = rays_o.device
+        f = lambda *s: torch.empty(*s, dtype=torch.float32, device=dev)
+        xyzs, dirs, deltas = f(G * M, 3), f(G * M, 3), f(G * M, 2)
+        rays = torch.empty(G, N, 3, dtype=torch.int32, device=dev)
+        counter = torch.empty(G, 2, dtype=torch.int32, device=dev)
+        pvd_hip.march_rays_train_group(rays_o.float().contiguous(), rays_d.float().contiguous(), self.density_bitfield, self.bound, dt_gamma,
+                                       max_steps, N, G, self.cascade, self.grid_size, M, nears.contiguous(), fars.contiguous(), xyzs, dirs,
+                                       deltas, rays, counter, perturb, fresh=True, budget_dev=budget_dev, coarse_mask=self.coarse_mask())
+        j = max(G - 16, 0)
+        while j < G:
+            slot = (self.local_step + j) % 16
+            run = min(G - j, 16 - slot)
+            self.step_counter[slot:slot + run].copy_(counter[j:j + run])
+            j += run
+        self.local_step += G
+        return xyzs, dirs, deltas, rays, M
+
     def _march_train(self, rays_o, rays_d, nears, fars, counter, perturb, force_all_rays, dt_gamma, max_steps, budget):
         coarse = self.coarse_mask()
         extra = () if budget is None and coarse is None else (budget,) if coarse is None else (budget, coarse)
diff --git a/aaai2023-pvd_amd/pvd/trainer.py b/aaai2023-pvd_amd/pvd/trainer.py
--- a/aaai2023-pvd_amd/pvd/trainer.py
+++ b/aaai2023-pvd_amd/pvd/trainer.py
@@ -250,7 +250,7 @@
 
     steps_per_replay = 1
 
-    def capture(self, body, warmup=3, steps_per_graph=1):
+    def capture(self, body, warmup=3, steps_per_graph=1, record_body=None):
         assert self.device_type == "cuda"
         side = torch.cuda.Stream()
         side.wait_stream(torch.cuda.current_stream())
@@ -277,7 +277,7 @@
             with cap:
                 for k_rec in range(max(1, int(steps_per_graph))):
                     self._zero_grads(first_in_recording=k_rec == 0)
-                    self._static_out = body()
+                    self._static_out = (record_body or body)()
                     if os.environ.get("PVD_TEST_FAIL_IN_CAPTURE") == "1":
                         raise RuntimeError("forced failure inside the capture (PVD_TEST_FAIL_IN_CAPTURE)")
                     self._backward(self._static_out[0])
@@ -379,6 +379,46 @@
         tea = self.model_tea
         attrs = {k: getattr(tea, k, None) for k in ("feature_sigma_color", "sigma_l", "color_l")}
         return dict(part, out_tea=out_tea, tea_attrs={k: v for k, v in attrs.items() if torch.is_tensor(v)})
+
+    def prefetch_group(self, batch_group_fn, G):
+        stu, tea = self.model_stu, self.model_tea
+        rm = stu.rm
+        rays_o, rays_d, bg, nf = batch_group_fn(G)
+        N = rays_o.shape[1]
+        amp = self.fp16 and self.device_type == "cuda"
+        kw = self.render_kwargs()
+        xyzs, dirs, deltas, rays, M = stu.march_group(rays_o, rays_d, nf, dt_gamma=kw["dt_gamma"], perturb=True, max_steps=kw["max_steps"])
+        with torch.autocast(self.device_type, dtype=torch.float16, enabled=amp), torch.no_grad():
+            sigmas, rgbs = tea(xyzs, dirs)
+            attrs = {k: getattr(tea, k, None) for k in ("feature_sigma_color", "sigma_l", "color_l")}
+            if tea.density_scale != 1:
+                sigmas = tea.density_scale * sigmas
+        import pvd_hip
+        sigmas, rgbs = sigmas.float().contiguous(), rgbs.float().contiguous()
+        ws = torch.empty(G, N, dtype=torch.float32, device=sigmas.device)
+        depth, image = torch.empty_like(ws), torch.empty(G, N, 3, dtype=torch.float32, device=sigmas.device)
+        pvd_hip.composite_rays_train_bg_forward_group(sigmas, rgbs, deltas, rays, M, N, G, bg.contiguous(), 0.0, nf[0], nf[1], 1e-6, ws, depth, image)
+        pres = []
+        for j in range(G):
+            sl = slice(j * M, (j + 1) * M)
+            out_tea = {"depth": depth[j].view(1, N), "image": image[j].view(1, N, 3), "inherited_params": None, "sigmas": sigmas[sl], "rays": rays[j],
+                       "nears_fars": (nf[0][j], nf[1][j])}
+            pres.append(dict(rays_o=rays_o[j:j + 1], rays_d=rays_d[j:j + 1], bg=bg[j:j + 1], inh=[xyzs[sl], dirs[sl], deltas[sl], rays[j]],
+                             nf=(nf[0][j], nf[1][j]), out_tea=out_tea, tea_attrs={k: v[sl] for k, v in attrs.items() if torch.is_tensor(v)}))
+        return pres
+
+    def _prefix_group(self, steps_per_graph, batch_group_fn):
+        try:
+            G = int(os.environ.get("PVD_PREFIX_GROUP", "20") or 20)
+        except ValueError:
+            G = 1
+        tea, stu = self.model_tea, self.model_stu
+        if (G <= 1 or batch_group_fn is None or self.device_type != "cuda" or tea.bg_radius > 0 or stu.bg_radius > 0 or not stu.cuda_ray
+                or stu.mean_count <= 0 or getattr(tea, "teacher_variant", False)):
+            return 1
+        while steps_per_graph % G:
+            G -= 1
+        return G
 
     def compute_loss(self, rays_o, rays_d, bg_color, nears_fars=None, pre=None):
         o, stu, tea = self.opt, self.model_stu, self.model_tea
@@ -509,7 +549,7 @@
         self._backward_and_step(loss)
         return loss.detach(), info, pred_stu, pred_tea
 
-    def capture_step(self, batch_fn, steps_per_graph=1):
+    def capture_step(self, batch_fn, steps_per_graph=1, batch_group_fn=None):
         def body():
             rays_o, rays_d, bg, *rest = batch_fn()
             with torch.autocast(self.device_type, dtype=torch.float16, enabled=self.fp16):
@@ -520,6 +560,7 @@
             self.sync_sharded_state()
         self._replay_owes_part_a = None
         self.fused_spans = None
+        self.prefix_group = 1
         stage = self._stage_of(self.global_step)
         assert self._stage_of(self.global_step + warm) == stage, \
             "capture_step: the %d warm-up steps cross a stage boundary (global_step %d); step eagerly past it first" % (warm, self.global_step)
@@ -546,6 +587,19 @@
                 self.pipelined_ingraph = False
                 self.capture_fallback = "back-to-back"
                 out = self.capture(body, warmup=0, steps_per_graph=steps_per_graph)
+        elif not self.dp.enabled and stage == 3 and stu_marches and self._prefix_group(steps_per_graph, batch_group_fn) > 1:
+            G = self._prefix_group(steps_per_graph, batch_group_fn)
+            group = {"k": 0, "pres": None}
+
+            def body_grouped():
+                if group["k"] % G == 0:
+                    group["pres"] = self.prefetch_group(batch_group_fn, G)
+                pre = group["pres"][group["k"] % G]
+                group["k"] += 1
+                with torch.autocast(self.device_type, dtype=torch.float16, enabled=self.fp16):
+                    return self.compute_loss(None, None, None, pre=pre)
+            out = self.capture(body, steps_per_graph=steps_per_graph, record_body=body_grouped)
+            self.prefix_group = G
         else:
             out = self.capture(body, steps_per_graph=steps_per_graph)
         self._captured_stage = self._stage_of(self.global_step)
diff --git a/aaai2023-pvd_amd/pvd/workload.py b/aaai2023-pvd_amd/pvd/workload.py
--- a/aaai2023-pvd_amd/pvd/workload.py
+++ b/aaai2023-pvd_amd/pvd/workload.py
@@ -124,14 +124,17 @@
         bg = torch.rand(1, opt.num_rays, 3, device=self.device, generator=self.gen)
         return r["rays_o"], r["rays_d"], bg
 
+    def _init_batch_state(self):
+        if not hasattr(self, "_batch_state"):
+            self._batch_state = torch.zeros(3, dtype=torch.int64, device=self.device)
+            self._poses_c = self.poses.float().contiguous()
+            self._batch_seed = 0x5eed + 1000003 * int(torch.cuda.initial_seed() % (2 ** 31)) + 0x9E3779B1 * self.dp_rank
+
     def device_batch(self):
         opt = self.opt
         mk = getattr(self.ops, "make_batch", None)
         if mk is not None:
-            if not hasattr(self, "_batch_state"):
-                self._batch_state = torch.zeros(3, dtype=torch.int64, device=self.device)
-                self._poses_c = self.poses.float().contiguous()
-                self._batch_seed = 0x5eed + 1000003 * int(torch.cuda.initial_seed() % (2 ** 31)) + 0x9E3779B1 * self.dp_rank
+            self._init_batch_state()
             return mk(self._poses_c, self._batch_state, self._batch_seed, BLENDER_INTRINSICS, 800, 800, opt.num_rays,
                       self.stu.aabb_train, self.stu.min_near)
         if not hasattr(self, "_pose_idx"):
@@ -143,9 +146,15 @@
         bg = torch.rand(1, opt.num_rays, 3, device=self.device)
         return r["rays_o"], r["rays_d"], bg
 
+    def device_batch_group(self, G):
+        self._init_batch_state()
+        return self.ops.make_batch_group(self._poses_c, self._batch_state, self._batch_seed, BLENDER_INTRINSICS, 800, 800, self.opt.num_rays, G,
+                                         self.stu.aabb_train, self.stu.min_near)
+
     def enable_graph(self, steps_per_graph=1):
         assert not self.opt.update_stu_extra, "update_stu_extra rewrites the occupancy grid between steps: run eagerly"
-        self.trainer.capture_step(self.device_batch, steps_per_graph=steps_per_graph)
+        group_fn = self.device_batch_group if getattr(self.ops, "make_batch_group", None) is not None else None
+        self.trainer.capture_step(self.device_batch, steps_per_graph=steps_per_graph, batch_group_fn=group_fn)
         self._graph = True
 
     @property
diff --git a/aaai2023-pvd_amd/pvd_hip/__init__.py b/aaai2023-pvd_amd/pvd_hip/__init__.py
--- a/aaai2023-pvd_amd/pvd_hip/__init__.py
+++ b/aaai2023-pvd_amd/pvd_hip/__init__.py
@@ -75,11 +75,18 @@
 ENTRY_POINTS_MESH_SIMPLIFY = ("pvd_mesh_simplify_workspace_bytes", "pvd_mesh_simplify_count", "pvd_mesh_simplify_emit")
 ENTRY_POINTS_MESH_RAY = ("pvd_mesh_ray_workspace_bytes", "pvd_mesh_ray_count", "pvd_mesh_ray_build", "pvd_mesh_ray_cast")
 ENTRY_POINTS_MESH_SMOOTH = ("pvd_mesh_smooth_workspace_bytes", "pvd_mesh_smooth_build", "pvd_mesh_smooth_run")
+ENTRY_POINTS_PREFIX = ("pvd_make_ray_batch_group", "pvd_march_group_workspace_bytes", "pvd_march_rays_train_group",
+                       "pvd_composite_rays_train_bg_forward_group")
 for _name in (ENTRY_POINTS + ENTRY_POINTS_MLP + ENTRY_POINTS_METRICS + ENTRY_POINTS_DATA + ENTRY_POINTS_MARCH + ENTRY_POINTS_MESH
               + ENTRY_POINTS_COMPONENTS + ENTRY_POINTS_MESH_ATTR + ENTRY_POINTS_MESH_DIST + ENTRY_POINTS_MESH_SIMPLIFY + ENTRY_POINTS_MESH_RAY
               + ENTRY_POINTS_MESH_SMOOTH):
     if _name not in ("pvd_status_string", "pvd_last_hip_error"):
         getattr(_lib, _name).restype = ctypes.c_int
+HAS_PREFIX_GROUP = all(hasattr(_lib, _name) for _name in ENTRY_POINTS_PREFIX)
+if HAS_PREFIX_GROUP:
+    for _name in ENTRY_POINTS_PREFIX:
+        getattr(_lib, _name).restype = ctypes.c_int
+    _lib.pvd_march_group_workspace_bytes.restype = ctypes.c_size_t
 _lib.pvd_march_workspace_bytes.restype = ctypes.c_size_t
 _lib.pvd_mesh_workspace_bytes.restype = ctypes.c_size_t
 _lib.pvd_mesh_dist_workspace_bytes.restype = ctypes.c_size_t
@@ -962,6 +969,76 @@
           _p(weights_sum), _p(image), _u32(M), _u32(N), _p(bg), _f32(bg_scalar), _p(grad_sigmas), _p(grad_rgbs), _u32(1 if fresh else 0),
           _p(budget_dev))
 
+
+
+def make_ray_batch_group(poses, state, seed, fx, fy, cx, cy, H, W, N, G, aabb, min_near, inds, rays_o, rays_d, bg, nears, fars):
+    dev = _dev(poses, state, aabb, inds, rays_o, rays_d, bg, nears, fars)
+    _f32_all(poses=poses, aabb=aabb, rays_o=rays_o, rays_d=rays_d, nears=nears, fars=fars)
+    _want(state, torch.int64, "state")
+    if inds is not None:
+        _want(inds, torch.int64, "inds")
+    if bg is not None:
+        _want(bg, torch.float32, "bg")
+    if state.numel() < 3:
+        raise PvdHipError("state must hold 3 int64 values")
+    for name, t, per in (("inds", inds, 1), ("rays_o", rays_o, 3), ("rays_d", rays_d, 3), ("bg", bg, 3), ("nears", nears, 1), ("fars", fars, 1)):
+        if t is not None and t.numel() != G * N * per:
+            raise PvdHipError("%s must hold G * N * %d elements" % (name, per))
+    _call("pvd_make_ray_batch_group", dev, _p(poses), _u32(poses.shape[0]), _p(state), ctypes.c_uint64(int(seed) & (2 ** 64 - 1)), _f32(fx),
+          _f32(fy), _f32(cx), _f32(cy), _u32(H), _u32(W), _u32(N), _u32(G), _p(aabb), _f32(min_near), _p(inds), _p(rays_o), _p(rays_d), _p(bg),
+          _p(nears), _p(fars))
+
+
+def _march_group_workspace(dev, N, G):
+    key = (dev, torch.cuda.current_stream(dev).cuda_stream, N, G)
+    ws = _march_ws.get(key)
+    if ws is None:
+        ws = torch.empty(int(_lib.pvd_march_group_workspace_bytes(_u32(N), _u32(G))), dtype=torch.uint8, device=dev)
+        _march_ws[key] = ws
+    return ws
+
+
+def march_rays_train_group(rays_o, rays_d, grid, bound, dt_gamma, max_steps, N, G, C, H, M, nears, fars, xyzs, dirs, deltas, rays, counter,
+                           perturb, fresh=False, budget_dev=None, coarse_mask=None):
+    dev = _dev(rays_o, rays_d, grid, nears, fars, xyzs, dirs, deltas, rays, counter, budget_dev, coarse_mask)
+    if coarse_mask is not None:
+        _want(coarse_mask, torch.uint8, "coarse_mask")
+        if coarse_mask.numel() != coarse_mask_bytes(C, H):
+            raise PvdHipError("coarse_mask must hold C * (H/8)^3 bytes")
+    stride = 0
+    if budget_dev is not None:
+        _want(budget_dev, torch.int32, "budget_dev")
+        if budget_dev.numel() not in (1, G):
+            raise PvdHipError("budget_dev must hold 1 or G values")
+        stride = 1 if (budget_dev.numel() == G and G > 1) else 0
+    _f32_all(rays_o=rays_o, rays_d=rays_d, nears=nears, fars=fars, xyzs=xyzs, dirs=dirs, deltas=deltas)
+    _want(grid, torch.uint8, "grid"), _want(rays, torch.int32, "rays"), _want(counter, torch.int32, "counter")
+    if (rays_o.numel() != 3 * G * N or rays_d.numel() != 3 * G * N or nears.numel() != G * N or fars.numel() != G * N or rays.numel() != 3 * G * N
+            or counter.numel() != 2 * G or xyzs.numel() != 3 * G * M or dirs.numel() != 3 * G * M or deltas.numel() != 2 * G * M):
+        raise PvdHipError("group buffers must be [G][N ...] / [G][M ...]")
+    if N > 16384:
+        raise PvdHipError("a segment holds at most 16384 rays")
+    ws = _march_group_workspace(dev, N, G)
+    _call("pvd_march_rays_train_group", dev, _p(rays_o), _p(rays_d), _p(grid), _f32(bound), _f32(dt_gamma), _u32(max_steps), _u32(N), _u32(G),
+          _u32(C), _u32(H), _u32(M), _p(nears), _p(fars), _p(xyzs), _p(dirs), _p(deltas), _p(rays), _p(counter), _u32(int(perturb)), _p(ws),
+          ctypes.c_size_t(ws.numel()), _u32(1 if fresh else 0), _p(budget_dev), _u32(stride), _p(coarse_mask))
+
+
+def composite_rays_train_bg_forward_group(sigmas, rgbs, deltas, rays, M, N, G, bg, bg_scalar, nears, fars, depth_eps, weights_sum, depth, image,
+                                          budget_dev=None):
+    dev = _dev(sigmas, rgbs, deltas, rays, bg, nears, fars, weights_sum, depth, image, budget_dev)
+    _f32_all(sigmas=sigmas, rgbs=rgbs, deltas=deltas, nears=nears, fars=fars, weights_sum=weights_sum, depth=depth, image=image)
+    _want(rays, torch.int32, "rays")
+    if (sigmas.numel() != G * M or rgbs.numel() != 3 * G * M or deltas.numel() != 2 * G * M or rays.numel() != 3 * G * N or nears.numel() != G * N
+            or fars.numel() != G * N or weights_sum.numel() != G * N or depth.numel() != G * N or image.numel() != 3 * G * N
+            or (bg is not None and bg.numel() != 3 * G * N)):
+        raise PvdHipError("group buffers must be [G][N ...] / [G][M ...]")
+    stride = 0
+    if budget_dev is not None:
+        _want(budget_dev, torch.int32, "budget_dev")
+        stride = 1 if (budget_dev.numel() == G and G > 1) else 0
+    _call("pvd_composite_rays_train_bg_forward_group", dev, _p(sigmas), _p(rgbs), _p(deltas), _p(rays), _u32(M), _u32(N), _u32(G), _p(bg),
+          _f32(bg_scalar), _p(nears), _p(fars), _f32(depth_eps), _p(weights_sum), _p(depth), _p(image), _p(budget_dev), _u32(stride))
 
 
 def composite_objective_blocks(N, rows, fixed=False):
diff --git a/include/pvd_hip_prefix.h b/include/pvd_hip_prefix.h
--- /dev/null
+++ b/include/pvd_hip_prefix.h
@@ -0,0 +1,33 @@
+#ifndef PVD_HIP_PREFIX_H
+#define PVD_HIP_PREFIX_H
+
+#include "pvd_hip_march.h"
+
+#ifdef __cplusplus
+extern "C" {
+#endif
+
+int pvd_make_ray_batch_group(const float *poses, uint32_t P, int64_t *state, uint64_t seed, float fx, float fy, float cx,
+                             float cy, uint32_t H, uint32_t W, uint32_t N, uint32_t G, const float *aabb, float min_near,
+                             int64_t *inds, float *rays_o, float *rays_d, float *bg, float *nears, float *fars,
+                             pvd_stream_t stream);
+
+size_t pvd_march_group_workspace_bytes(uint32_t N, uint32_t G);
+
+int pvd_march_rays_train_group(const float *rays_o, const float *rays_d, const uint8_t *grid, float bound, float dt_gamma,
+                               uint32_t max_steps, uint32_t N, uint32_t G, uint32_t C, uint32_t H, uint32_t M, const float *nears,
+                               const float *fars, float *xyzs, float *dirs, float *deltas, int32_t *rays, int32_t *counter,
+                               uint32_t perturb, void *workspace, size_t workspace_bytes, uint32_t flags,
+                               const int32_t *budget_dev, uint32_t budget_stride, const uint8_t *coarse_mask, pvd_stream_t stream);
+
+int pvd_composite_rays_train_bg_forward_group(const float *sigmas, const float *rgbs, const float *deltas, const int32_t *rays,
+                                              uint32_t M, uint32_t N, uint32_t G, const float *bg, float bg_scalar,
+                                              const float *nears, const float *fars, float depth_eps, float *weights_sum,
+                                              float *depth, float *image, const int32_t *budget_dev, uint32_t budget_stride,
+                                              pvd_stream_t stream);
+
+#ifdef __cplusplus
+}
+#endif
+
+#endif
```

Result: faster. 12.97 million rays/s (median of 6 runs) (+11.3%).
